# vymv/PupilOptixLab

Hardware: AMD Instinct MI355X
Metric: Mrays/sec + ms/frame, 1M-tri scene @1920x1080 8spp; 1/2/4/8-GPU scaling (higher is better)
Workload: dtype f32; 1 GPU; config4: 1,000,014-primitive sphere field (1,000,014 tris), 1920x1080, 8 spp, max_depth 4; rays_traced_plain_process=18645769168, parallelism=tiles32x1, area_emitters=2, accel=flat, emitter_select=guide, bvh_nodes=213019

## Files before the change

### include/pupil_pt.h

```cpp
#pragma once
#include <stddef.h>
#include <stdint.h>

#ifdef __cplusplus
extern "C" {
#endif

#define PUPIL_OK 0
#define PUPIL_ERR_INVALID -1
#define PUPIL_ERR_HIP -2
#define PUPIL_ERR_OOM -3
#define PUPIL_ERR_IO -4
#define PUPIL_ERR_UNSUPPORTED -5

#define PUPIL_TEX_RGB 0u
#define PUPIL_TEX_BITMAP 1u
#define PUPIL_TEX_CHECKERBOARD 2u

#define PUPIL_MAT_UNKNOWN 0u
#define PUPIL_MAT_DIFFUSE 1u
#define PUPIL_MAT_DIELECTRIC 2u
#define PUPIL_MAT_ROUGH_DIELECTRIC 3u
#define PUPIL_MAT_CONDUCTOR 4u
#define PUPIL_MAT_ROUGH_CONDUCTOR 5u
#define PUPIL_MAT_PLASTIC 6u
#define PUPIL_MAT_ROUGH_PLASTIC 7u
#define PUPIL_MAT_COUNT 8u

#define PUPIL_EMITTER_NONE 0u
#define PUPIL_EMITTER_TRI_AREA 1u
#define PUPIL_EMITTER_SPHERE 2u
#define PUPIL_EMITTER_CONST_ENV 3u
#define PUPIL_EMITTER_ENV_MAP 4u
#define PUPIL_EMITTER_POINT 5u
#define PUPIL_EMITTER_SPOT 6u
#define PUPIL_EMITTER_DIRECTIONAL 7u

#define PUPIL_SHAPE_MESH 0u
#define PUPIL_SHAPE_SPHERE 1u

typedef struct pupil_texture {
    uint32_t type;
    float c0[3];
    float c1[3];
    float transform[16];
    uint32_t width, height;
    uint32_t filter;
    uint32_t pad;
    const float *rgba;
} pupil_texture;

typedef struct pupil_material {
    uint32_t type;
    uint32_t twosided;
    float int_ior, ext_ior;
    uint32_t nonlinear;
    pupil_texture tex[4];
} pupil_material;

typedef struct pupil_shape {
    uint32_t kind;
    uint32_t num_vertices, num_faces;
    const float *positions;
    const float *normals;
    const float *texcoords;
    const uint32_t *indices;
} pupil_shape;

typedef struct pupil_instance {
    uint32_t shape;
    uint32_t material;
    float to_world[12];
    float to_object[12];
    uint32_t flip_normals;
    uint32_t flip_tex_coords;
    int32_t emitter_offset;
    uint32_t pad;
} pupil_instance;

typedef struct pupil_emitter {
    uint32_t type;
    float weight;
    float select_probability;
    float area;
    pupil_texture radiance;
    float pos[3][3];
    float nrm[3][3];
    float tex[3][2];
    float center[3];
    float radius;
    float color[3];
    float to_world[9];
    float to_local[9];
    float scale;
} pupil_emitter;

typedef struct pupil_scene_desc {
    uint32_t width, height;
    uint32_t max_depth;
    uint32_t pad0;
    float sample_to_camera[16];
    float camera_to_world[16];
    uint32_t num_shapes;
    uint32_t num_materials;
    uint32_t num_instances;
    uint32_t num_area_emitters;
    const pupil_shape *shapes;
    const pupil_material *materials;
    const pupil_instance *instances;
    const pupil_emitter *area_emitters;
    const pupil_emitter *env;
} pupil_scene_desc;

typedef struct pupil_pt_frame {
    void *accum;
    void *frame;
    void *albedo;
    void *normal;
    void *test;
    uint32_t compact;
    uint32_t pad;
} pupil_pt_frame;

typedef struct pupil_pt_launch {
    uint32_t random_seed;
    uint32_t sample_cnt;
    uint32_t spp;
    uint32_t max_depth;
    uint32_t accumulate;
    uint32_t tile_size;
    uint32_t tile_rank;
    uint32_t tile_world;
    uint32_t collect_stats;
    uint32_t hints;
} pupil_pt_launch;

#define PUPIL_STATS_COUNTERS 1u
#define PUPIL_STATS_TIMING 2u
#define PUPIL_STATS_TRACE_TIMING 4u
#define PUPIL_HINT_CONTINUE 1u

typedef struct pupil_pt_counters {
    uint64_t primary_rays;
    uint64_t extension_rays;
    uint64_t shadow_rays;
    uint64_t path_samples;
    uint64_t node_visits;
    uint64_t prim_tests;
    uint64_t bvh_nodes;
    uint64_t bvh_prims;
    double build_ms;
    double last_render_ms;
    double trace_ms;
    double trace_bytes;
    uint64_t trace_launches;
    double extend_ms;
    uint64_t extend_launches;
    uint64_t extend_node_visits;
    uint64_t extend_prim_tests;
    double extend_bytes;
    double shade_ms;
    uint64_t two_level;
    uint64_t shadow_rays_reference;
    uint64_t bvh_depth;
    uint64_t unique_node_fetches;
    uint64_t rays_traced_total;
    uint64_t frames_in_flight;
    uint64_t pipeline_slots;
    uint64_t tlas_sah_splits;
    uint64_t queue_handed;
    uint64_t queue_activated;
    uint64_t queue_retired;
    uint64_t queue_listed;
    uint64_t ring_bytes;
    uint64_t ring_budget_bytes;
    uint64_t accel_refits;
    float node_bound[3];
    uint32_t pad_counters;
    uint64_t node_loop_iters;
    uint64_t node_loop_lanes;
    uint64_t leaf_loop_iters;
    uint64_t leaf_loop_lanes;
    uint64_t refills;
    uint64_t refill_lanes;
    uint64_t frame_launches;
    double frame_ms;
    uint64_t terminal_rays_culled;
    uint64_t coop_slots;
    uint64_t hidden_instances;
} pupil_pt_counters;

typedef struct pupil_pt pupil_pt;

const char *pupil_last_error(void);
int pupil_abi_version(void);

int pupil_pt_create(const pupil_scene_desc *scene, int device, pupil_pt **out);
int pupil_pt_set_camera(pupil_pt *pt, const float sample_to_camera[16], const float camera_to_world[16]);
int pupil_pt_update_instance(pupil_pt *pt, uint32_t instance, const float to_world[12], const float to_object[12]);
int pupil_pt_update_instances(pupil_pt *pt, uint32_t n, const uint32_t *ids, const float *to_world,
                              const float *to_object);
int pupil_pt_update_instances_masked(pupil_pt *pt, uint32_t n, const uint32_t *ids,
                                     const float *to_world, const float *to_object,
                                     const uint32_t *visibility_mask);
int pupil_pt_update_instances_device(pupil_pt *pt, uint32_t n, const uint32_t *ids_device,
                                     const void *to_world_device, const void *to_object_device, void *hip_stream);
int pupil_pt_get_instance_transforms(pupil_pt *pt, uint32_t first, uint32_t n, float *to_world, float *to_object);
int pupil_pt_instances_device_info(pupil_pt *pt, uint64_t *updates, uint64_t *instances, uint64_t *skipped,
                                   uint32_t *last_launches, uint32_t *last_syncs, double *last_ms);
int pupil_debug_invert3x4(const float m[12], float out[12]);
int pupil_debug_update_counts(pupil_pt *pt, uint32_t *launches, uint32_t *syncs);
#define PUPIL_VERTS_DEVICE 1u
#define PUPIL_VERTS_REBUILD 2u
int pupil_pt_update_shape_vertices(pupil_pt *pt, uint32_t shape, const float *positions, const float *normals,
                                   uint32_t flags, void *hip_stream);
int pupil_pt_snapshot_shape_vertices(pupil_pt *pt, uint32_t shape);
int pupil_pt_clear_vertex_snapshots(pupil_pt *pt);
int pupil_pt_update_emitters(pupil_pt *pt, const pupil_scene_desc *scene);
int pupil_pt_enable_device_emitters(pupil_pt *pt, const pupil_scene_desc *scene);
int pupil_pt_refresh_emitters(pupil_pt *pt);
int pupil_pt_device_emitters_info(pupil_pt *pt, uint32_t *enabled, uint64_t *refreshes, double *last_ms);
int pupil_pt_update_materials(pupil_pt *pt, uint32_t n, const uint32_t *ids, const pupil_material *materials);
int pupil_pt_update_texture_device(pupil_pt *pt, uint32_t material, uint32_t slot, const void *rgba_device,
                                   uint32_t width, uint32_t height, void *hip_stream);
int pupil_pt_material_info(pupil_pt *pt, uint64_t *updates, double *last_ms);
int pupil_pt_update_env_device(pupil_pt *pt, const void *rgba_device, uint32_t width, uint32_t height,
                               void *hip_stream);
int pupil_pt_update_env_params(pupil_pt *pt, float scale, const float to_world[9], const float to_local[9]);
int pupil_pt_env_info(pupil_pt *pt, uint64_t *updates, double *last_ms);
int pupil_pt_render(pupil_pt *pt, const pupil_pt_frame *out, const pupil_pt_launch *launch, void *hip_stream);
int pupil_pt_stats(pupil_pt *pt, pupil_pt_counters *out);
int pupil_pt_local_pixels(uint32_t width, uint32_t height, uint32_t tile_size, uint32_t tile_rank,
                          uint32_t tile_world, uint32_t *out_pixels, uint32_t *inout_count);
void pupil_pt_destroy(pupil_pt *pt);
int pupil_pt_motion_vectors(pupil_pt *pt, const float prev_sample_to_camera[16],
                            const float prev_camera_to_world[16], const float *prev_to_world,
                            void *out_flow , uint32_t compact,
                            uint32_t tile_size, uint32_t tile_rank, uint32_t tile_world,
                            void *hip_stream);

typedef struct pupil_ray_hits {
    void *hit;
    void *instance;
    void *primitive;
    void *material;
    void *position;
    void *normal;
    void *texcoord;
} pupil_ray_hits;
enum { PUPIL_QUERY_ANY_HIT = 1 };
int pupil_pt_query_rays(pupil_pt *pt, uint32_t n, const void *rays_device , uint32_t flags,
                        const pupil_ray_hits *out, void *hip_stream);
int pupil_pt_query_camera(pupil_pt *pt, float jitter_x, float jitter_y, uint32_t compact, uint32_t tile_size,
                          uint32_t tile_rank, uint32_t tile_world, void *rays_out_device, const pupil_ray_hits *out,
                          void *hip_stream);
int pupil_pt_query_info(pupil_pt *pt, uint64_t *queries, uint64_t *rays, uint64_t *scratch_grows, double *last_ms);

typedef struct pupil_ray_radiance {
    void *radiance;
    void *albedo;
    void *normal;
} pupil_ray_radiance;
int pupil_pt_radiance_rays(pupil_pt *pt, uint32_t n, const void *rays_device ,
                           const uint32_t *stream_ids_device ,
                           const pupil_pt_launch *launch, const pupil_ray_radiance *out, void *hip_stream);
int pupil_pt_radiance_info(pupil_pt *pt, uint64_t *calls, uint64_t *rays, uint64_t *extension_rays,
                           uint64_t *shadow_rays, uint64_t *scratch_grows, double *last_ms);

int pupil_pt_trace_rays(pupil_pt *pt, uint32_t n, const float *rays, float *out, int any_hit);
int pupil_pt_export_bvh4(pupil_pt *pt, uint32_t *num_nodes, void *nodes, uint32_t *num_records, float *records,
                         int32_t *root_link);
int pupil_debug_math(int device, uint32_t n, const float *x, const float *y2, float *out);
int pupil_debug_select_emitter(pupil_pt *pt, uint32_t n, const float *p, int32_t *out);
int pupil_debug_read_emitters(pupil_pt *pt, uint32_t first, uint32_t n, float *out);
int pupil_debug_emitter_sample(pupil_pt *pt, uint32_t emitter, uint32_t n, const float *xi, const float *pos_nrm,
                               float *out);
int pupil_debug_read_emitter_guide(pupil_pt *pt, uint32_t *bits, uint32_t *guide, uint32_t *inout_count);
int pupil_debug_env(pupil_pt *pt, uint32_t n, const float *xi_or_dir, const float *pos_nrm, uint32_t mode, float *out);
int pupil_debug_read_env_tables(pupil_pt *pt, uint32_t *width, uint32_t *height, float *col_cdf, float *row_cdf,
                                float *row_weight, float *normalization);
int pupil_debug_tex_sample(pupil_pt *pt, uint32_t material, uint32_t slot, uint32_t n, const float *uv, float *out);
int pupil_debug_read_material(pupil_pt *pt, uint32_t material, uint32_t *type, float out[3]);
int pupil_debug_fill_tlas_reserve(pupil_pt *pt, float value);
int pupil_debug_bvh_reinsert(int device, uint32_t n, const float *boxes, uint32_t rounds, double *cost,
                             uint32_t *kept, uint32_t *rejected);
int pupil_debug_partition(int device, uint32_t n, uint32_t capacity, const uint8_t *keys, uint32_t nbins,
                          uint32_t mode, uint32_t shift_or_tag, uint32_t bin_mask, const uint64_t *cum_in,
                          uint32_t *out, uint32_t *counts, uint32_t *starts, uint32_t *total, uint32_t *log,
                          uint64_t *cum_out, uint64_t *snap, uint32_t *info);

enum { PUPIL_IMAGE_AUTO = 0, PUPIL_IMAGE_EXR = 1, PUPIL_IMAGE_HDR = 2, PUPIL_IMAGE_PFM = 3 };
int pupil_image_save(const char *path, uint32_t width, uint32_t height, const float *rgba, uint32_t format);

int pupil_image_load(const char *path, uint32_t *width, uint32_t *height, float *rgba);

enum {
    PUPIL_DENOISE_USE_ALBEDO = 1,
    PUPIL_DENOISE_USE_NORMAL = 1 << 1,
    PUPIL_DENOISE_APPLY_TO_AOV = 1 << 2,
    PUPIL_DENOISE_USE_TEMPORAL = 1 << 3,
    PUPIL_DENOISE_USE_UPSCALE_2X = 1 << 4,
    PUPIL_DENOISE_TILED = 1 << 5
};
typedef struct pupil_denoise_data {
    const void *input;
    void *output;
    const void *prev_output;
    const void *albedo;
    const void *normal;
    const void *motion_vector;
} pupil_denoise_data;
typedef struct pupil_denoiser pupil_denoiser;
int pupil_denoiser_create(int device, uint32_t mode, pupil_denoiser **out);
int pupil_denoiser_setup(pupil_denoiser *d, uint32_t mode, uint32_t width, uint32_t height, float sigma_color);
int pupil_denoiser_execute(pupil_denoiser *d, const pupil_denoise_data *data, void *hip_stream);
int pupil_denoiser_reset_history(pupil_denoiser *d);
void pupil_denoiser_destroy(pupil_denoiser *d);

typedef struct pupil_world pupil_world;

int pupil_world_create(pupil_world **out);
int pupil_world_load_xml(pupil_world *w, const char *path);
int pupil_world_set_film(pupil_world *w, uint32_t width, uint32_t height, uint32_t max_depth);
int pupil_world_set_sensor(pupil_world *w, float fov, char fov_axis, float near_clip, float far_clip,
                           const float to_world[16]);
int pupil_world_add_mesh(pupil_world *w, uint32_t num_vertices, uint32_t num_faces, const float *positions,
                         const float *normals, const float *texcoords, const uint32_t *indices, uint32_t *out_shape);
int pupil_world_add_builtin_shape(pupil_world *w, const char *name , uint32_t *out_shape);
int pupil_world_add_material(pupil_world *w, const pupil_material *m, uint32_t *out_material);
int pupil_world_add_instance(pupil_world *w, uint32_t shape, uint32_t material, const float to_world[16],
                             uint32_t flip_normals, uint32_t flip_tex_coords, uint32_t is_emitter,
                             const pupil_texture *radiance, uint32_t *out_instance);
int pupil_world_add_const_env(pupil_world *w, const float radiance[3]);
int pupil_world_add_delta_emitter(pupil_world *w, const pupil_emitter *e, uint32_t *out_light);
int pupil_world_set_delta_emitter(pupil_world *w, uint32_t light, const pupil_emitter *e);
int pupil_world_get_delta_emitter(pupil_world *w, uint32_t light, pupil_emitter *out);
int pupil_world_invert3x3(const float m[9], float out[9]);
int pupil_world_set_instance_transform(pupil_world *w, uint32_t instance, const float to_world[16]);
int pupil_world_set_instance_visibility(pupil_world *w, uint32_t instance, uint32_t visibility_mask);
int pupil_world_get_instance_visibility(pupil_world *w, uint32_t instance, uint32_t *visibility_mask);
int pupil_world_set_mesh_vertices(pupil_world *w, uint32_t shape, const float *positions, const float *normals);
int pupil_world_set_material(pupil_world *w, uint32_t material, const pupil_material *m);
int pupil_world_get_desc(pupil_world *w, pupil_scene_desc *desc);
void pupil_world_destroy(pupil_world *w);

#ifdef __cplusplus
}
#endif
```

### pupiloptixlab_amd/abi.py

```python
from __future__ import annotations

import ctypes as C
import os

TEX_RGB, TEX_BITMAP, TEX_CHECKERBOARD = 0, 1, 2
MAT_UNKNOWN, MAT_DIFFUSE, MAT_DIELECTRIC, MAT_ROUGH_DIELECTRIC = 0, 1, 2, 3
MAT_CONDUCTOR, MAT_ROUGH_CONDUCTOR, MAT_PLASTIC, MAT_ROUGH_PLASTIC = 4, 5, 6, 7
EMITTER_NONE, EMITTER_TRI_AREA, EMITTER_SPHERE, EMITTER_CONST_ENV, EMITTER_ENV_MAP = 0, 1, 2, 3, 4
EMITTER_POINT, EMITTER_SPOT, EMITTER_DIRECTIONAL = 5, 6, 7
SHAPE_MESH, SHAPE_SPHERE = 0, 1

PUPIL_OK = OK = 0
ERR_INVALID, ERR_HIP, ERR_OOM, ERR_IO, ERR_UNSUPPORTED = -1, -2, -3, -4, -5
VERTS_DEVICE, VERTS_REBUILD = 1, 2
IMAGE_AUTO, IMAGE_EXR, IMAGE_HDR, IMAGE_PFM = 0, 1, 2, 3
ERR_NAMES = {-1: "PUPIL_ERR_INVALID", -2: "PUPIL_ERR_HIP", -3: "PUPIL_ERR_OOM", -4: "PUPIL_ERR_IO",
             -5: "PUPIL_ERR_UNSUPPORTED"}

f32p = C.POINTER(C.c_float)
u32p = C.POINTER(C.c_uint32)


class Texture(C.Structure):
    _fields_ = [("type", C.c_uint32), ("c0", C.c_float * 3), ("c1", C.c_float * 3),
                ("transform", C.c_float * 16), ("width", C.c_uint32), ("height", C.c_uint32),
                ("filter", C.c_uint32), ("pad", C.c_uint32), ("rgba", f32p)]


class Material(C.Structure):
    _fields_ = [("type", C.c_uint32), ("twosided", C.c_uint32), ("int_ior", C.c_float),
                ("ext_ior", C.c_float), ("nonlinear", C.c_uint32), ("tex", Texture * 4)]


class Shape(C.Structure):
    _fields_ = [("kind", C.c_uint32), ("num_vertices", C.c_uint32), ("num_faces", C.c_uint32),
                ("positions", f32p), ("normals", f32p), ("texcoords", f32p), ("indices", u32p)]


class Instance(C.Structure):
    _fields_ = [("shape", C.c_uint32), ("material", C.c_uint32), ("to_world", C.c_float * 12),
                ("to_object", C.c_float * 12), ("flip_normals", C.c_uint32),
                ("flip_tex_coords", C.c_uint32), ("emitter_offset", C.c_int32), ("pad", C.c_uint32)]


class Emitter(C.Structure):
    _fields_ = [("type", C.c_uint32), ("weight", C.c_float), ("select_probability", C.c_float),
                ("area", C.c_float), ("radiance", Texture), ("pos", (C.c_float * 3) * 3),
                ("nrm", (C.c_float * 3) * 3), ("tex", (C.c_float * 2) * 3), ("center", C.c_float * 3),
                ("radius", C.c_float), ("color", C.c_float * 3), ("to_world", C.c_float * 9),
                ("to_local", C.c_float * 9), ("scale", C.c_float)]


class SceneDesc(C.Structure):
    _fields_ = [("width", C.c_uint32), ("height", C.c_uint32), ("max_depth", C.c_uint32),
                ("pad0", C.c_uint32), ("sample_to_camera", C.c_float * 16),
                ("camera_to_world", C.c_float * 16), ("num_shapes", C.c_uint32),
                ("num_materials", C.c_uint32), ("num_instances", C.c_uint32),
                ("num_area_emitters", C.c_uint32), ("shapes", C.POINTER(Shape)),
                ("materials", C.POINTER(Material)), ("instances", C.POINTER(Instance)),
                ("area_emitters", C.POINTER(Emitter)), ("env", C.POINTER(Emitter))]


class Frame(C.Structure):
    _fields_ = [("accum", C.c_void_p), ("frame", C.c_void_p), ("albedo", C.c_void_p),
                ("normal", C.c_void_p), ("test", C.c_void_p), ("compact", C.c_uint32),
                ("pad", C.c_uint32)]


class Launch(C.Structure):
    _fields_ = [("random_seed", C.c_uint32), ("sample_cnt", C.c_uint32), ("spp", C.c_uint32),
                ("max_depth", C.c_uint32), ("accumulate", C.c_uint32), ("tile_size", C.c_uint32),
                ("tile_rank", C.c_uint32), ("tile_world", C.c_uint32), ("collect_stats", C.c_uint32),
                ("hints", C.c_uint32)]


class Counters(C.Structure):
    _fields_ = [("primary_rays", C.c_uint64), ("extension_rays", C.c_uint64),
                ("shadow_rays", C.c_uint64), ("path_samples", C.c_uint64),
                ("node_visits", C.c_uint64), ("prim_tests", C.c_uint64), ("bvh_nodes", C.c_uint64),
                ("bvh_prims", C.c_uint64), ("build_ms", C.c_double), ("last_render_ms", C.c_double),
                ("trace_ms", C.c_double), ("trace_bytes", C.c_double), ("trace_launches", C.c_uint64),
                ("extend_ms", C.c_double), ("extend_launches", C.c_uint64), ("extend_node_visits", C.c_uint64),
                ("extend_prim_tests", C.c_uint64), ("extend_bytes", C.c_double), ("shade_ms", C.c_double),
                ("two_level", C.c_uint64), ("shadow_rays_reference", C.c_uint64),
                ("bvh_depth", C.c_uint64), ("unique_node_fetches", C.c_uint64),
                ("rays_traced_total", C.c_uint64), ("frames_in_flight", C.c_uint64),
                ("pipeline_slots", C.c_uint64), ("tlas_sah_splits", C.c_uint64),
                ("queue_handed", C.c_uint64), ("queue_activated", C.c_uint64), ("queue_retired", C.c_uint64),
                ("queue_listed", C.c_uint64), ("ring_bytes", C.c_uint64), ("ring_budget_bytes", C.c_uint64),
                ("accel_refits", C.c_uint64), ("node_bound", C.c_float * 3), ("pad_counters", C.c_uint32),
                ("node_loop_iters", C.c_uint64), ("node_loop_lanes", C.c_uint64), ("leaf_loop_iters", C.c_uint64),
                ("leaf_loop_lanes", C.c_uint64), ("refills", C.c_uint64), ("refill_lanes", C.c_uint64),
                ("frame_launches", C.c_uint64),
                ("frame_ms", C.c_double),
                ("terminal_rays_culled", C.c_uint64), ("coop_slots", C.c_uint64),
                ("hidden_instances", C.c_uint64)]

    def as_dict(self):
        d = {name: getattr(self, name) for name, _ in self._fields_ if name != "pad_counters"}
        d["node_bound"] = [float(x) for x in self.node_bound]
        return d


DENOISE_USE_ALBEDO, DENOISE_USE_NORMAL, DENOISE_APPLY_TO_AOV = 1, 2, 4
DENOISE_USE_TEMPORAL, DENOISE_USE_UPSCALE_2X, DENOISE_TILED = 8, 16, 32


class DenoiseData(C.Structure):
    _fields_ = [("input", C.c_void_p), ("output", C.c_void_p), ("prev_output", C.c_void_p),
                ("albedo", C.c_void_p), ("normal", C.c_void_p), ("motion_vector", C.c_void_p)]


QUERY_ANY_HIT = 1


class RayHits(C.Structure):
    _fields_ = [("hit", C.c_void_p), ("instance", C.c_void_p), ("primitive", C.c_void_p),
                ("material", C.c_void_p), ("position", C.c_void_p), ("normal", C.c_void_p),
                ("texcoord", C.c_void_p)]


class RayRadiance(C.Structure):
    _fields_ = [("radiance", C.c_void_p), ("albedo", C.c_void_p), ("normal", C.c_void_p)]


SIGNATURES = {
    "pupil_last_error": (C.c_char_p, []),
    "pupil_abi_version": (C.c_int, []),
    "pupil_pt_create": (C.c_int, [C.POINTER(SceneDesc), C.c_int, C.POINTER(C.c_void_p)]),
    "pupil_pt_set_camera": (C.c_int, [C.c_void_p, f32p, f32p]),
    "pupil_pt_update_instance": (C.c_int, [C.c_void_p, C.c_uint32, f32p, f32p]),
    "pupil_pt_update_instances": (C.c_int, [C.c_void_p, C.c_uint32, u32p, f32p, f32p]),
    "pupil_pt_update_instances_masked": (C.c_int, [C.c_void_p, C.c_uint32, u32p, f32p, f32p, u32p]),
    "pupil_pt_update_instances_device": (C.c_int, [C.c_void_p, C.c_uint32, C.c_void_p, C.c_void_p, C.c_void_p,
                                                    C.c_void_p]),
    "pupil_pt_get_instance_transforms": (C.c_int, [C.c_void_p, C.c_uint32, C.c_uint32, f32p, f32p]),
    "pupil_pt_instances_device_info": (C.c_int, [C.c_void_p, C.POINTER(C.c_uint64), C.POINTER(C.c_uint64),
                                                  C.POINTER(C.c_uint64), u32p, u32p, C.POINTER(C.c_double)]),
    "pupil_debug_invert3x4": (C.c_int, [f32p, f32p]),
    "pupil_debug_update_counts": (C.c_int, [C.c_void_p, u32p, u32p]),
    "pupil_pt_update_shape_vertices": (C.c_int, [C.c_void_p, C.c_uint32, C.c_void_p, C.c_void_p, C.c_uint32,
                                                  C.c_void_p]),
    "pupil_pt_snapshot_shape_vertices": (C.c_int, [C.c_void_p, C.c_uint32]),
    "pupil_pt_clear_vertex_snapshots": (C.c_int, [C.c_void_p]),
    "pupil_pt_update_emitters": (C.c_int, [C.c_void_p, C.POINTER(SceneDesc)]),
    "pupil_pt_enable_device_emitters": (C.c_int, [C.c_void_p, C.POINTER(SceneDesc)]),
    "pupil_pt_refresh_emitters": (C.c_int, [C.c_void_p]),
    "pupil_pt_device_emitters_info": (C.c_int, [C.c_void_p, u32p, C.POINTER(C.c_uint64), C.POINTER(C.c_double)]),
    "pupil_pt_update_materials": (C.c_int, [C.c_void_p, C.c_uint32, u32p, C.POINTER(Material)]),
    "pupil_pt_update_texture_device": (C.c_int, [C.c_void_p, C.c_uint32, C.c_uint32, C.c_void_p, C.c_uint32,
                                                  C.c_uint32, C.c_void_p]),
    "pupil_pt_material_info": (C.c_int, [C.c_void_p, C.POINTER(C.c_uint64), C.POINTER(C.c_double)]),
    "pupil_pt_update_env_device": (C.c_int, [C.c_void_p, C.c_void_p, C.c_uint32, C.c_uint32, C.c_void_p]),
    "pupil_pt_update_env_params": (C.c_int, [C.c_void_p, C.c_float, f32p, f32p]),
    "pupil_pt_env_info": (C.c_int, [C.c_void_p, C.POINTER(C.c_uint64), C.POINTER(C.c_double)]),
    "pupil_debug_read_env_tables": (C.c_int, [C.c_void_p, u32p, u32p, f32p, f32p, f32p, f32p]),
    "pupil_world_invert3x3": (C.c_int, [f32p, f32p]),
    "pupil_debug_read_material": (C.c_int, [C.c_void_p, C.c_uint32, u32p, f32p]),
    "pupil_debug_read_emitters": (C.c_int, [C.c_void_p, C.c_uint32, C.c_uint32, f32p]),
    "pupil_debug_read_emitter_guide": (C.c_int, [C.c_void_p, u32p, u32p, u32p]),
    "pupil_debug_fill_tlas_reserve": (C.c_int, [C.c_void_p, C.c_float]),
    "pupil_pt_render": (C.c_int, [C.c_void_p, C.POINTER(Frame), C.POINTER(Launch), C.c_void_p]),
    "pupil_pt_stats": (C.c_int, [C.c_void_p, C.POINTER(Counters)]),
    "pupil_pt_local_pixels": (C.c_int, [C.c_uint32, C.c_uint32, C.c_uint32, C.c_uint32, C.c_uint32,
                                         u32p, u32p]),
    "pupil_pt_destroy": (None, [C.c_void_p]),
    "pupil_pt_motion_vectors": (C.c_int, [C.c_void_p, f32p, f32p, f32p, C.c_void_p, C.c_uint32, C.c_uint32,
                                           C.c_uint32, C.c_uint32, C.c_void_p]),
    "pupil_pt_query_rays": (C.c_int, [C.c_void_p, C.c_uint32, C.c_void_p, C.c_uint32, C.POINTER(RayHits), C.c_void_p]),
    "pupil_pt_query_camera": (C.c_int, [C.c_void_p, C.c_float, C.c_float, C.c_uint32, C.c_uint32, C.c_uint32,
                                         C.c_uint32, C.c_void_p, C.POINTER(RayHits), C.c_void_p]),
    "pupil_pt_query_info": (C.c_int, [C.c_void_p, C.POINTER(C.c_uint64), C.POINTER(C.c_uint64),
                                       C.POINTER(C.c_uint64), C.POINTER(C.c_double)]),
    "pupil_pt_radiance_rays": (C.c_int, [C.c_void_p, C.c_uint32, C.c_void_p, C.c_void_p, C.POINTER(Launch),
                                          C.POINTER(RayRadiance), C.c_void_p]),
    "pupil_pt_radiance_info": (C.c_int, [C.c_void_p, C.POINTER(C.c_uint64), C.POINTER(C.c_uint64),
                                          C.POINTER(C.c_uint64), C.POINTER(C.c_uint64), C.POINTER(C.c_uint64),
                                          C.POINTER(C.c_double)]),
    "pupil_pt_trace_rays": (C.c_int, [C.c_void_p, C.c_uint32, f32p, f32p, C.c_int]),
    "pupil_pt_export_bvh4": (C.c_int, [C.c_void_p, u32p, C.c_void_p, u32p, f32p, C.POINTER(C.c_int32)]),
    "pupil_debug_math": (C.c_int, [C.c_int, C.c_uint32, f32p, f32p, f32p]),
    "pupil_debug_bvh_reinsert": (C.c_int, [C.c_int, C.c_uint32, f32p, C.c_uint32, C.POINTER(C.c_double), u32p, u32p]),
    "pupil_debug_partition": (C.c_int, [C.c_int, C.c_uint32, C.c_uint32, C.POINTER(C.c_uint8), C.c_uint32, C.c_uint32,
                                         C.c_uint32, C.c_uint32, C.POINTER(C.c_uint64), u32p, u32p, u32p, u32p, u32p,
                                         C.POINTER(C.c_uint64), C.POINTER(C.c_uint64), u32p]),
    "pupil_image_save": (C.c_int, [C.c_char_p, C.c_uint32, C.c_uint32, f32p, C.c_uint32]),
    "pupil_debug_select_emitter": (C.c_int, [C.c_void_p, C.c_uint32, f32p, C.POINTER(C.c_int32)]),
    "pupil_debug_env": (C.c_int, [C.c_void_p, C.c_uint32, f32p, f32p, C.c_uint32, f32p]),
    "pupil_debug_emitter_sample": (C.c_int, [C.c_void_p, C.c_uint32, C.c_uint32, f32p, f32p, f32p]),
    "pupil_debug_tex_sample": (C.c_int, [C.c_void_p, C.c_uint32, C.c_uint32, C.c_uint32, f32p, f32p]),
    "pupil_image_load": (C.c_int, [C.c_char_p, C.POINTER(C.c_uint32), C.POINTER(C.c_uint32), f32p]),
    "pupil_world_create": (C.c_int, [C.POINTER(C.c_void_p)]),
    "pupil_world_load_xml": (C.c_int, [C.c_void_p, C.c_char_p]),
    "pupil_world_set_film": (C.c_int, [C.c_void_p, C.c_uint32, C.c_uint32, C.c_uint32]),
    "pupil_world_set_sensor": (C.c_int, [C.c_void_p, C.c_float, C.c_char, C.c_float, C.c_float, f32p]),
    "pupil_world_add_mesh": (C.c_int, [C.c_void_p, C.c_uint32, C.c_uint32, f32p, f32p, f32p, u32p, u32p]),
    "pupil_world_add_builtin_shape": (C.c_int, [C.c_void_p, C.c_char_p, u32p]),
    "pupil_world_add_material": (C.c_int, [C.c_void_p, C.POINTER(Material), u32p]),
    "pupil_world_add_instance": (C.c_int, [C.c_void_p, C.c_uint32, C.c_uint32, f32p, C.c_uint32,
                                           C.c_uint32, C.c_uint32, C.POINTER(Texture), u32p]),
    "pupil_world_add_const_env": (C.c_int, [C.c_void_p, f32p]),
    "pupil_world_add_delta_emitter": (C.c_int, [C.c_void_p, C.POINTER(Emitter), u32p]),
    "pupil_world_set_delta_emitter": (C.c_int, [C.c_void_p, C.c_uint32, C.POINTER(Emitter)]),
    "pupil_world_get_delta_emitter": (C.c_int, [C.c_void_p, C.c_uint32, C.POINTER(Emitter)]),
    "pupil_world_set_instance_transform": (C.c_int, [C.c_void_p, C.c_uint32, f32p]),
    "pupil_world_set_instance_visibility": (C.c_int, [C.c_void_p, C.c_uint32, C.c_uint32]),
    "pupil_world_get_instance_visibility": (C.c_int, [C.c_void_p, C.c_uint32, u32p]),
    "pupil_world_set_mesh_vertices": (C.c_int, [C.c_void_p, C.c_uint32, f32p, f32p]),
    "pupil_world_set_material": (C.c_int, [C.c_void_p, C.c_uint32, C.POINTER(Material)]),
    "pupil_world_get_desc": (C.c_int, [C.c_void_p, C.POINTER(SceneDesc)]),
    "pupil_world_destroy": (None, [C.c_void_p]),
    "pupil_denoiser_create": (C.c_int, [C.c_int, C.c_uint32, C.POINTER(C.c_void_p)]),
    "pupil_denoiser_setup": (C.c_int, [C.c_void_p, C.c_uint32, C.c_uint32, C.c_uint32, C.c_float]),
    "pupil_denoiser_execute": (C.c_int, [C.c_void_p, C.POINTER(DenoiseData), C.c_void_p]),
    "pupil_denoiser_reset_history": (C.c_int, [C.c_void_p]),
    "pupil_denoiser_destroy": (None, [C.c_void_p]),
}

LIB_DIR = os.path.join(os.path.dirname(os.path.abspath(__file__)), "lib")
LIB_PATH = os.path.join(LIB_DIR, "libpupil_pt.so")


class PupilError(RuntimeError):
    def __init__(self, code: int, message: str):
        super().__init__(f"{ERR_NAMES.get(code, code)}: {message}")
        self.code = code


_LIB = None


def load_library(path: str | None = None):
    global _LIB
    if _LIB is not None and path is None:
        return _LIB
    try:
        import torch
    except Exception:
        pass
    p = path or os.environ.get("PUPIL_LIB") or LIB_PATH
    if not os.path.exists(p):
        raise FileNotFoundError(f"{p} not built: run `python -c 'import __graft_entry__ as g; g.build()'`")
    lib = C.CDLL(p)
    for name, (res, args) in SIGNATURES.items():
        if p != LIB_PATH and not hasattr(lib, name):
            continue
        fn = getattr(lib, name)
        fn.restype = res
        fn.argtypes = args
    if path is None:
        _LIB = lib
    return lib


def check(code: int, lib=None):
    if code != PUPIL_OK:
        lib = lib or load_library()
        msg = lib.pupil_last_error()
        raise PupilError(code, msg.decode() if msg else "")
    return code
```

### pupiloptixlab_amd/csrc/engine.hip

```cpp
#include <hip/hip_runtime.h>

#include <algorithm>
#include <chrono>
#include <cmath>
#include <cstddef>
#include <cstdio>
#include <cstdlib>
#include <cstring>
#include <string>
#include <vector>

#include "host/emitter_weight.h"
#include "host/pipe_schedule.h"
#include "host/scoped_buffer.h"
#include "pt_accel.h"

namespace {

thread_local std::string g_last_error;

constexpr uint32_t kMaxPairs = 4096;

using namespace pupil;

// ... 525 lines not shown
    bool trace_only = false;
    uint32_t pair = 0;
    bool open = false;
    const TraceStats *tsp() const { return stats ? &ts_dev : nullptr; }
    uint32_t pair_cap = 0;
    void ev0(uint8_t kind) {
        open = timing && !(trace_only && kind == 2) && pair < pair_cap;
        if (!open) return;
        pt->pair_kind[pair] = kind;
        (void)hipEventRecord(pt->trace_events[2 * pair], s);
    }
    void ev1() {
        if (!open) return;
        (void)hipEventRecord(pt->trace_events[2 * pair + 1], s);
        pair++;
        open = false;
    }
    void tail_slot() {
        if (tail && pt->tail_launches < kMaxDepth + 1)
            ts_dev.wave_times = pt->tail_buf + (size_t)pt->tail_launches++ * pt->tail_waves * 4;
        else
            ts_dev.wave_times = nullptr;
    }
    PathState view(uint32_t h, size_t paths, size_t extra = 0) const {
        PathState v = pt->ps;
        const size_t o = (size_t)h * paths + extra;
        v.ray_o += o, v.ray_d += o, v.hit += o, v.thr += o, v.rad += o, v.misc += o;
        v.sh_d += o, v.sh_c += o, v.mbin += o, v.sflags += o;
        return v;
    }
};

int render_pipelined(RenderCtx &cx, const FrameParams &fp, const pupil_pt_launch *launch) {
    pupil_pt *pt = cx.pt;
    hipStream_t s = cx.s;
    PipeState &st = pt->pipe;
    const PipeKnobs &kn = pt->knobs;
    const uint32_t nl = fp.num_local;
    const PipeRender r{fp.spp, launch->random_seed, fp.max_depth, (launch->hints & PUPIL_HINT_CONTINUE) != 0, cx.stats,
                       fp.num_paths, nl, {cx.key[0], cx.key[1], cx.key[2], cx.key[3], cx.key[4]}};
    PipePlan plan = st.plan(kn, r);
    bool grew = false;
    if (plan.ring_paths() > pt->cap) {
        grew = true;
        int rc = ensure_state(pt, plan.ring_paths());
        while (rc == PUPIL_ERR_OOM && plan.shrink()) rc = ensure_state(pt, plan.ring_paths());
        if (rc) return rc;
    }
    if (plan.aov_floats() > pt->aov_cap) {
        grew = true;
        if (pt->aov_scratch) (void)hipFree(pt->aov_scratch);
        pt->aov_scratch = nullptr;
        pt->aov_cap = 0;
        HIP_TRY(hipMalloc((void **)&pt->aov_scratch, sizeof(float) * plan.aov_floats()));
        pt->aov_cap = plan.aov_floats();
    }
    const PathState ring = pt->ps;
    const PipeCommit commit = st.commit(plan, grew);
    for (const PipeRange &d : commit.dropped) {
        if (d.off + d.len > pt->cap) continue;
        HIP_TRY(hipMemsetAsync(ring.sflags + d.off, 0, d.len, s));
        if (!pt->shade_list) HIP_TRY(hipMemsetAsync(ring.mbin + d.off, 0xFF, d.len, s));
    }
    if (commit.reset && pt->ring_fresh) {
        HIP_TRY(hipMemsetAsync(ring.sflags, 0, pt->cap, s));
        if (!pt->shade_list) HIP_TRY(hipMemsetAsync(ring.mbin, 0xFF, pt->cap, s));
        pt->ring_fresh = false;
    }
    Queues &q = pt->q;
    const uint32_t interleave0 = pt->primary_interleave;
    if (st.one_launch_frame(kn) && frame_kernel_supported(pt->sc)) {
        HIP_TRY(hipMemcpyAsync(pt->ray_cum + 2, pt->ray_cum, 2 * sizeof(unsigned long long), hipMemcpyDeviceToDevice, s));
        pt->snap_taken = true;
        FrameParams fs = fp;
        fs.group = 1;
        cx.ev0(3);
        launch_frame(pt->sc, fs, ring, pt->q.work + kWorkFrame, pt->ray_cum, pt->ovf, pt->ovf_threads,
                     interleave0 && fp.spp > 1 ? fp.spp : 0u, s);
        cx.ev1();
        launch_accumulate(fp, ring, nullptr, true, s);
        st.one_launch_frame_done();
        pt->last_iters = fp.max_depth;
        pt->last_primary = st.started;
        pt->primary_cum += st.started;
        pt->frame_launches++;
        return PUPIL_OK;
    }
    auto scratch = [&](uint32_t index) { return pt->aov_scratch + (size_t)index * 7 * nl; };
    pt->snap_taken = false;
    auto trace = [&](const PipeTrace &t) -> int {
        const uint32_t interleave = interleave0 && t.samples > 1 ? t.samples : 0u;
        if (t.inject) {
            FrameParams fg = fp;
            fg.seed0 = t.nf.seed;
            fg.num_paths = t.nfp;
            launch_generate(pt->sc, fg, cx.view(t.nf.slot, st.cap), s, !pt->fresh());
        }
        if (t.had) {
            launch_partition(ring.sflags, t.ring_extent, 2, kPartFlags, t.read_tag, q.nxsh, q.hist, q.counts + kCntNext,
                             q.counts + kStartNext, nullptr, nullptr, s, pt->ray_cum,
                             pt->snap_taken ? nullptr : pt->ray_cum + 2);
            pt->snap_taken = true;
            if (t.check_exit) {
                uint32_t c[2] = {1, 1};
                HIP_TRY(hipMemcpyAsync(c, q.counts + kCntNext, sizeof(c), hipMemcpyDeviceToHost, s));
                HIP_TRY(hipStreamSynchronize(s));
                if (c[0] == 0 && c[1] == 0) return 1;
            }
            cx.ev0(1);
            cx.tail_slot();
            if (t.inject)
                launch_trace_mixed(pt->sc, ring, q, pt->ovf, pt->ovf_threads, cx.tsp(), s, t.nfp, 0u, t.base, interleave, nl);
            else
                launch_trace_mixed(pt->sc, ring, q, pt->ovf, pt->ovf_threads, cx.tsp(), s);
            cx.ev1();
        } else {
            cx.ev0(0);
            cx.tail_slot();
            launch_extend(pt->sc, cx.view(t.nf.slot, st.cap), q, nullptr, nullptr, t.nfp, pt->ovf, pt->ovf_threads,
                          cx.tsp(), s, interleave, nl);
            cx.ev1();
        }
        return 0;
    };
    auto shade = [&](const PipeShade &h) -> int {
        if (!pt->shade_list)
            launch_partition(ring.mbin, h.ring_extent, kPartMaxBins, kPartExclusive, 0u, q.bins, q.hist, q.counts,
                             q.counts + kStartBins, q.counts + kScratch, nullptr, s, nullptr, nullptr, pt->bin_mask);
        FrameParams fs = fp;
        fs.group = st.G;
        if (h.aov_scratch) {
            fs.albedo = scratch(h.aov_index);
            fs.normal = fs.albedo + 3 * (size_t)nl;
            fs.test = fs.albedo + 6 * (size_t)nl;
            fs.aov_local = 1;
            fs.aov_frame_stride = (uint32_t)(7 * nl);
        }
        if (h.clear_flags) HIP_TRY(hipMemsetAsync(ring.sflags, 0, h.ring_extent, s));
        constexpr ShadeList kLists[] = {kShadeAll, kShadeNext, kShadeNextRange};
        const ShadeList list = pt->shade_list ? kLists[(int)h.list] : kShadeBins;
        cx.ev0(2);
        launch_shade(pt->sc, fs, ring, q, h.write_tag, s, list, h.range_base, h.range_n, h.max_count, pt->fresh(),
                     h.range_seed);
        cx.ev1();
        return 0;
    };
    if (st.half_pending)
        if (const int rc = shade(st.shade_half())) return rc;
    const uint32_t L = st.iterations();
    for (uint32_t it = 0; it < L; it++) {
        const int rc = trace(st.trace_half(kn, it, L));
        if (rc == 1) break;
        if (rc) return rc;
        if (const int rs = shade(st.shade_half())) return rs;
    }
    const PipeFinish fin = st.finish(kn, L);
    launch_accumulate(fp, cx.view(fin.slot, st.cap, fin.offset), fin.aov_scratch ? scratch(fin.aov_index) : nullptr, true, s);
    if (fin.trace_ahead) {
        const int rc = trace(st.trace_ahead(kn));
        if (rc < 0) return rc;
        st.half_ran(rc == 0);
    }
    pt->last_iters = L;
    pt->last_primary = st.started;
    pt->primary_cum += st.started;
    return PUPIL_OK;
}


int upload_shapes(pupil_pt *pt, const pupil_scene_desc *scene) {
    std::vector<ShapeDev> &shapes = pt->shapes;
    shapes.assign(scene->num_shapes, ShapeDev{});
    for (uint32_t s = 0; s < scene->num_shapes; s++) {
        const pupil_shape &sh = scene->shapes[s];
        shapes[s].kind = sh.kind;
        shapes[s].num_vertices = sh.num_vertices;
        shapes[s].num_faces = sh.num_faces;
        if (sh.kind == PUPIL_SHAPE_MESH) {
            if (!sh.positions || !sh.indices || sh.num_faces == 0)
                return fail(PUPIL_ERR_INVALID, "mesh without positions/indices");
            for (size_t i = 0; i < 3 * (size_t)sh.num_faces; i++)
                if (sh.indices[i] >= sh.num_vertices) return fail(PUPIL_ERR_INVALID, "index out of range");
            if (pt->upload(&shapes[s].pos, sh.positions, 3 * (size_t)sh.num_vertices) ||
                (sh.normals && pt->upload(&shapes[s].nrm, sh.normals, 3 * (size_t)sh.num_vertices)) ||
                (sh.texcoords && pt->upload(&shapes[s].tex, sh.texcoords, 2 * (size_t)sh.num_vertices)) ||
                pt->upload(&shapes[s].idx, sh.indices, 3 * (size_t)sh.num_faces))
                return fail(PUPIL_ERR_OOM, "mesh upload failed");
        } else if (sh.kind != PUPIL_SHAPE_SPHERE) {
            return fail(PUPIL_ERR_INVALID, "unknown shape kind");
        }
    }
    return PUPIL_OK;
}

int convert_material(const pupil_material &src, DevMaterial &d) {
    std::memset(&d, 0, sizeof(d));
    d.type = src.type <= 7u ? src.type : 0u;
    d.twosided = src.twosided;
    d.nonlinear = src.nonlinear;
    if (d.type == PUPIL_MAT_DIELECTRIC || d.type == PUPIL_MAT_ROUGH_DIELECTRIC || d.type == PUPIL_MAT_PLASTIC ||
        d.type == PUPIL_MAT_ROUGH_PLASTIC)
        d.eta = src.int_ior / src.ext_ior;
    for (int k = 0; k < 4; k++)
        if (const int rc = texture_desc(src.tex[k], d.tex[k])) return rc;
    if (d.type == PUPIL_MAT_PLASTIC || d.type == PUPIL_MAT_ROUGH_PLASTIC) {
        const pupil_texture &dt = d.type == PUPIL_MAT_PLASTIC ? src.tex[0] : src.tex[1];
        const pupil_texture &stx = d.type == PUPIL_MAT_PLASTIC ? src.tex[1] : src.tex[2];
        d.specular_sampling_weight = specular_sampling_weight(pixel_average(dt), pixel_average(stx));
        d.int_fdr = diffuse_reflectance(1.f / d.eta);
    }
    return PUPIL_OK;
}

int convert_materials(pupil_pt *pt, const pupil_scene_desc *scene, std::vector<DevMaterial> &mats) {
    mats.resize(scene->num_materials);
    for (uint32_t m = 0; m < scene->num_materials; m++) {
        const pupil_material &src = scene->materials[m];
        DevMaterial &d = mats[m];
        if (const int rc = convert_material(src, d)) return rc;
        for (int k = 0; k < 4; k++)
            if (src.tex[k].type == PUPIL_TEX_BITMAP) {
                float4 *texels = nullptr;
                HIP_TRY(pt->upload(&texels, reinterpret_cast<const float4 *>(src.tex[k].rgba),
                                   (size_t)src.tex[k].width * src.tex[k].height));
                d.tex[k].data = texels;
            }
    }
    if (mats.empty()) {
        DevMaterial d;
        std::memset(&d, 0, sizeof(d));
        mats.push_back(d);
    }
    return PUPIL_OK;
}

int upload_tables(pupil_pt *pt, const pupil_scene_desc *scene, const std::vector<DevMaterial> &mats) {
    std::vector<DevInstance> &insts = pt->h_insts;
    insts.resize(scene->num_instances);
    std::vector<uint32_t> prim_inst;
    uint32_t true_areas = 0;
    if (scene->area_emitters)
        for (uint32_t e = 0; e < scene->num_area_emitters; e++) {
            const uint32_t t = scene->area_emitters[e].type;
            true_areas += t >= PUPIL_EMITTER_POINT && t <= PUPIL_EMITTER_DIRECTIONAL ? 0u : 1u;
        }
    for (uint32_t i = 0; i < scene->num_instances; i++) {
        const pupil_instance &src = scene->instances[i];
        if (src.shape >= scene->num_shapes) return fail(PUPIL_ERR_INVALID, "instance shape out of range");
        if (src.material >= mats.size()) return fail(PUPIL_ERR_INVALID, "instance material out of range");
        const pupil_shape &sh = scene->shapes[src.shape];
        DevInstance &d = insts[i];
        std::memset(&d, 0, sizeof(d));
        std::memcpy(d.to_world, src.to_world, sizeof(d.to_world));
        std::memcpy(d.to_object, src.to_object, sizeof(d.to_object));
        d.kind = sh.kind;
        d.material = src.material;
        d.prim_offset = (uint32_t)prim_inst.size();
        d.emitter_offset = src.emitter_offset;
        d.flip_normals = src.flip_normals;
        d.flip_tex_coords = src.flip_tex_coords;
        d.bin = material_bin(mats[src.material].type);
        d.blas_root = kTraverseDone;
        d.positions = pt->shapes[src.shape].pos;
        d.normals = pt->shapes[src.shape].nrm;
        d.texcoords = pt->shapes[src.shape].tex;
        d.indices = pt->shapes[src.shape].idx;
        const uint32_t nprim = sh.kind == PUPIL_SHAPE_SPHERE ? 1u : sh.num_faces;
        if (src.emitter_offset >= 0 && (size_t)src.emitter_offset + nprim > true_areas)
            return fail(PUPIL_ERR_INVALID, "emitter offset out of range");
        prim_inst.insert(prim_inst.end(), nprim, i);
    }
    pt->num_prims = (uint32_t)prim_inst.size();
    if (prim_inst.size() >= (1ull << 31)) return fail(PUPIL_ERR_UNSUPPORTED, "more than 2^31 primitives");
    std::vector<uint32_t> inst_first(insts.size() + 1);
    for (size_t i = 0; i < insts.size(); i++) inst_first[i] = insts[i].prim_offset;
    inst_first[insts.size()] = (uint32_t)prim_inst.size();
    uint32_t guide_shift = 0;
    while ((prim_inst.size() >> guide_shift) > 8192u) guide_shift++;
    std::vector<uint32_t> inst_guide;
    if (!prim_inst.empty()) {
        const size_t nb = ((prim_inst.size() - 1) >> guide_shift) + 1;
        inst_guide.resize(nb + 1);
        for (size_t k = 0; k <= nb; k++)
            inst_guide[k] = prim_inst[std::min(k << guide_shift, prim_inst.size() - 1)];
    } else {
        inst_guide.assign(2, 0u);
    }
    uint32_t *d_inst_first = nullptr, *d_inst_guide = nullptr;
    if (pt->upload(&pt->d_insts, insts.data(), insts.size()) || pt->upload(&pt->d_mats, mats.data(), mats.size()) ||
        pt->upload(&pt->d_prim_inst, prim_inst.data(), prim_inst.size()) ||
        pt->upload(&d_inst_first, inst_first.data(), inst_first.size()) ||
        pt->upload(&d_inst_guide, inst_guide.data(), inst_guide.size()))
        return fail(PUPIL_ERR_OOM, "scene upload failed");
    pt->num_mats = (uint32_t)mats.size();
    pt->h_mats = mats;
    DeviceScene &sc = pt->sc;
    sc.num_prims = pt->num_prims;
    sc.prim_inst = pt->d_prim_inst;
    sc.inst_first = d_inst_first;
    sc.inst_guide = d_inst_guide;
    sc.inst_guide_shift = guide_shift;
    sc.instances = pt->d_insts;
    sc.materials = pt->d_mats;
    return PUPIL_OK;
}

void derive_bins(pupil_pt *pt) {
    DeviceScene &sc = pt->sc;
    const bool was_list = pt->shade_list;
    const uint32_t was_single = sc.single_bin;
    uint32_t bins = 0;
    for (const DevInstance &d : pt->h_insts) bins |= 1u << d.bin;
    pt->shade_list = (bins & (bins - 1u)) == 0u;
    if (const char *sl = std::getenv("PUPIL_SHADE_LIST")) {
        if (std::strcmp(sl, "bins") == 0) pt->shade_list = false;
        if (std::strcmp(sl, "list") == 0) pt->shade_list = true;
    }
    sc.single_bin = pt->shade_list && bins && (bins & (bins - 1u)) == 0u ? (uint32_t)__builtin_ctz(bins) : 0u;
    pt->bin_mask = bins | 1u;
    if (pt->shade_list != was_list || sc.single_bin != was_single) pt->ring_fresh = true;
}

void read_knobs(pupil_pt *pt) {
    DeviceScene &sc = pt->sc;
    int cus = 256;
    (void)hipDeviceGetAttribute(&cus, hipDeviceAttributeMultiprocessorCount, pt->device);
    sc.num_cus = (uint32_t)std::max(1, cus);
    sc.trace_refill = 16;
    if (const char *r = std::getenv("PUPIL_REFILL")) sc.trace_refill = (uint32_t)std::min(64, std::max(1, std::atoi(r)));
    if (const char *po = std::getenv("PUPIL_PRIMARY_ORDER")) pt->primary_interleave = std::strcmp(po, "path") != 0;
    derive_bins(pt);
    if (const char *fr = std::getenv("PUPIL_FRESH_SHADE")) pt->fresh_shade = std::atoi(fr) != 0;
    if (const char *tc = std::getenv("PUPIL_TERMINAL_CULL")) pt->cull_on = std::atoi(tc) != 0;
    if (const char *tk = std::getenv("PUPIL_TERMINAL_CULL_K"))
        pt->cull_k = (uint32_t)std::min((int)kCullSetMax, std::max(1, std::atoi(tk)));
    if (const char *a = std::getenv("PUPIL_AHEAD")) pt->knobs.ahead_mode = std::min(2, std::max(0, std::atoi(a)));
    if (const char *k = std::getenv("PUPIL_PIPE")) pt->knobs.limit = (uint32_t)std::min(63, std::max(0, std::atoi(k)));
    {
        size_t free_b = 0, total_b = 0;
        if (hipMemGetInfo(&free_b, &total_b) != hipSuccess) free_b = 0;
        pt->knobs.budget = 0.25 * (double)free_b;
    }
    if (const char *g = std::getenv("PUPIL_PIPE_GB")) pt->knobs.budget = std::max(0.0, std::atof(g)) * 1e9;
    if (const char *g = std::getenv("PUPIL_PIPE_PATHS")) pt->knobs.paths = std::max(1.0, std::atof(g));
    if (const char *g = std::getenv("PUPIL_PIPE_GROUP_PATHS")) pt->knobs.group_paths = std::max(1.0, std::atof(g));
    if (const char *g = std::getenv("PUPIL_PIPE_GROUP_MAX")) pt->knobs.group_max = (uint32_t)std::min(64, std::max(1, std::atoi(g)));
    if (const char *g = std::getenv("PUPIL_PIPE_GROUP_ALL")) pt->knobs.group_all = std::atoi(g) != 0;
    if (const char *g = std::getenv("PUPIL_PIPE_SPLIT")) pt->knobs.split = std::atoi(g) != 0;
    if (const char *g = std::getenv("PUPIL_PIPE_RAMP")) pt->knobs.ramp = (uint32_t)std::max(0, std::atoi(g));
    if (const char *g = std::getenv("PUPIL_FRAME_PATHS")) pt->knobs.frame_paths = std::max(0.0, std::atof(g));
    if (const char *g = std::getenv("PUPIL_RADIANCE_CHUNK"))
        pt->rad_chunk = (size_t)std::min(2147483647.0, std::max(64.0, std::atof(g)));
    sc.trace_node_min = 8;
    if (const char *r = std::getenv("PUPIL_NODE_MIN")) sc.trace_node_min = (uint32_t)std::min(64, std::max(1, std::atoi(r)));
}

int alloc_workspace(pupil_pt *pt) {
    pt->ovf_threads = trace_grid_blocks() * (uint32_t)kTraceBlock;
    if (pt->alloc(&pt->ovf, (size_t)pt->ovf_threads * kStackOvf) || pt->alloc(&pt->trace_counters, 32) ||
        pt->alloc(&pt->ray_cum, 4) || pt->alloc(&pt->q.counts, kCountSlots) || pt->alloc(&pt->q.work, kWorkSlots) ||
        pt->alloc(&pt->d_cull, 1 + kCullSetMax) || pt->alloc(&pt->cull_cum, 2 * kCullShards * kCullStride) ||
        pt->alloc(&pt->rad_cum, pupil_pt::kRadTotals + 2))
        return fail(PUPIL_ERR_OOM, "workspace allocation failed");
    if (hipMemset(pt->q.work, 0, kWorkSlots * sizeof(uint32_t)) != hipSuccess ||
        hipMemset(pt->rad_cum, 0, (pupil_pt::kRadTotals + 2) * sizeof(unsigned long long)) != hipSuccess ||
        hipMemset(pt->cull_cum, 0, 2 * kCullShards * kCullStride * sizeof(unsigned long long)) != hipSuccess ||
        hipMemset(pt->ray_cum, 0, 4 * sizeof(unsigned long long)) != hipSuccess)
        return fail(PUPIL_ERR_HIP, "workspace clear failed");
    if (hipEventCreate(&pt->ev_begin) != hipSuccess || hipEventCreate(&pt->ev_end) != hipSuccess ||
        hipEventCreateWithFlags(&pt->ev_sync, hipEventDisableTiming) != hipSuccess ||
        hipEventCreateWithFlags(&pt->ev_verts, hipEventDisableTiming) != hipSuccess)
        return fail(PUPIL_ERR_HIP, "event creation failed");
    return PUPIL_OK;
}

int derive_cull_set(pupil_pt *pt, bool records_changed = true) {
    DeviceScene &sc = pt->sc;
    sc.cull_set = pt->d_cull + 1;
    sc.cull_n = 0;
    if (records_changed) pt->cull_scanned = 0;
    if (records_changed) pt->query_slot_valid = false;
    if (!pt->cull_on || sc.has_env || !sc.prims || (sc.two_level && !sc.tl_world)) return PUPIL_OK;
    uint64_t emissive = 0;
    for (size_t i = 0; i < pt->h_insts.size(); i++) {
        const DevInstance &d = pt->h_insts[i];
        if (d.emitter_offset < 0) continue;
        emissive += d.kind == PUPIL_SHAPE_MESH ? pt->shapes[pt->accel.inst_shape[i]].num_faces : 1u;
    }
    if (emissive == 0 || emissive > pt->cull_k) return PUPIL_OK;
    if (pt->cull_scanned == emissive) {
        sc.cull_n = pt->cull_scanned;
        return PUPIL_OK;
    }
    uint32_t found[1 + kCullSetMax] = {};
    HIP_TRY(hipMemsetAsync(pt->d_cull, 0, sizeof(found), pt->own_stream));
    launch_cull_scan(sc.prims, pt->accel.world_record_slots(), pt->d_insts, (uint32_t)pt->h_insts.size(), pt->d_cull,
                     kCullSetMax, pt->own_stream);
    HIP_TRY(hipGetLastError());
    HIP_TRY(hipMemcpyAsync(found, pt->d_cull, sizeof(found), hipMemcpyDeviceToHost, pt->own_stream));
    HIP_TRY(hipStreamSynchronize(pt->own_stream));
    pt->accel.counts.launches++, pt->accel.counts.syncs++;
    if (found[0] != emissive) return PUPIL_OK;
    std::sort(found + 1, found + 1 + found[0]);
    HIP_TRY(hipMemcpyAsync(pt->d_cull, found, sizeof(found), hipMemcpyHostToDevice, pt->own_stream));
    HIP_TRY(hipStreamSynchronize(pt->own_stream));
    pt->accel.counts.syncs++;
    sc.cull_n = pt->cull_scanned = found[0];
    return PUPIL_OK;
}

int device_emitter_tables(const pupil_pt *pt, const pupil_scene_desc *scene, std::vector<uint32_t> &emit_inst,
                          std::vector<float> &inst_weight) {
    const uint32_t ni = (uint32_t)pt->h_insts.size(), ne = pt->num_true_areas;
    if (scene->num_instances != ni) return fail(PUPIL_ERR_INVALID, "the scene's instance count is not the engine's");
    if (scene->num_area_emitters != pt->sc.num_areas)
        return fail(PUPIL_ERR_INVALID, "the scene's area emitter count is not the engine's");
    if ((ni && !scene->instances) || (pt->sc.num_areas && !scene->area_emitters))
        return fail(PUPIL_ERR_INVALID, "missing scene array");
    for (uint32_t e = 0; e < pt->sc.num_areas; e++) {
        const uint32_t t = scene->area_emitters[e].type;
        const bool delta = t >= PUPIL_EMITTER_POINT && t <= PUPIL_EMITTER_DIRECTIONAL;
        if (delta != (e >= ne) || (delta && t != pt->emit_types[e]))
            return fail(PUPIL_ERR_INVALID, "the scene's delta lights are not the engine's");
    }
    emit_inst.assign(ne, 0u);
    inst_weight.assign(ni, 0.f);
    uint32_t next = 0;
    for (uint32_t i = 0; i < ni; i++) {
        const DevInstance &d = pt->h_insts[i];
        if (scene->instances[i].emitter_offset != d.emitter_offset)
            return fail(PUPIL_ERR_INVALID, "an instance's emitter_offset is not the engine's");
        if (d.emitter_offset < 0) continue;
        const uint32_t range = d.kind == PUPIL_SHAPE_MESH ? pt->shapes[pt->accel.inst_shape[i]].num_faces : 1u;
        if ((uint32_t)d.emitter_offset != next || range > ne - next)
            return fail(PUPIL_ERR_INVALID, "an emissive instance's emitter range is not its face count");
        inst_weight[i] = Pupil::world::GetWeight(scene->area_emitters[next].radiance);
        for (uint32_t k = 0; k < range; k++) emit_inst[next + k] = i;
        next += range;
    }
    if (next != ne) return fail(PUPIL_ERR_INVALID, "the emitter ranges do not cover the emitter table");
    return PUPIL_OK;
}

int device_emitter_setup(pupil_pt *pt, const pupil_scene_desc *scene) {
    std::vector<uint32_t> emit_inst;
    std::vector<float> inst_weight;
    if (const int rc = device_emitter_tables(pt, scene, emit_inst, inst_weight)) return rc;
    const uint32_t ne = pt->sc.num_areas;
    if (!pt->d_emit_inst || pt->dev_emit_count != ne) {
        for (void *p : {(void *)pt->d_emit_inst, (void *)pt->d_emit_weight, (void *)pt->d_emit_select}) pt->release(p);
        pt->d_emit_inst = nullptr;
        pt->d_emit_weight = pt->d_emit_select = nullptr;
        if (pt->alloc(&pt->d_emit_inst, ne) || pt->alloc(&pt->d_emit_weight, ne) || pt->alloc(&pt->d_emit_select, ne))
            return fail(PUPIL_ERR_OOM, "emitter bookkeeping allocation failed");
        pt->dev_emit_count = ne;
    }
    if (!pt->d_inst_weight && (pt->alloc(&pt->d_inst_weight, inst_weight.size()) || pt->alloc(&pt->d_emit_sum, 1)))
        return fail(PUPIL_ERR_OOM, "emitter bookkeeping allocation failed");
    if (!emit_inst.empty())
        HIP_TRY(hipMemcpy(pt->d_emit_inst, emit_inst.data(), sizeof(uint32_t) * emit_inst.size(), hipMemcpyHostToDevice));
    HIP_TRY(hipMemcpy(pt->d_inst_weight, inst_weight.data(), sizeof(float) * inst_weight.size(), hipMemcpyHostToDevice));
    return PUPIL_OK;
}

int rebuild_emitters(pupil_pt *pt) {
    const auto t0 = std::chrono::steady_clock::now();
    EmitterJob job{};
    job.areas = pt->d_areas;
    job.cdf = pt->d_cdf;
    job.guide = pt->d_guide;
    job.guide_bits = pt->sc.guide_bits;
    job.count = pt->num_true_areas;
    job.total = pt->sc.num_areas;
    job.emitter_num = pt->sc.num_areas + (pt->sc.has_env ? 1u : 0u);
    job.instances = pt->d_insts;
    job.emit_inst = pt->d_emit_inst;
    job.inst_weight = pt->d_inst_weight;
    job.weight = pt->d_emit_weight;
    job.select = pt->d_emit_select;
    job.sum = pt->d_emit_sum;
    launch_emitter_rebuild(job, pt->own_stream);
    HIP_TRY(hipGetLastError());
    HIP_TRY(hipStreamSynchronize(pt->own_stream));
    pt->accel.counts.launches += job.count ? (job.guide ? 5u : 4u) : 0u;
    pt->accel.counts.syncs++;
    pt->emit_refreshes++;
    pt->emit_ms = std::chrono::duration<double, std::milli>(std::chrono::steady_clock::now() - t0).count();
    return derive_cull_set(pt, false);
}

int keep_device_emitters(pupil_pt *pt, const pupil_scene_desc *scene) {
    if (!pt->dev_emit) return PUPIL_OK;
    if (device_emitter_setup(pt, scene) != PUPIL_OK) {
        pt->dev_emit = false;
        g_last_error = "device-side emitter table switched off: " + g_last_error;
    }
    return PUPIL_OK;
}

}

extern "C" {

const char *pupil_last_error(void) { return g_last_error.c_str(); }
int pupil_abi_version(void) { return 7; }

int pupil_pt_local_pixels(uint32_t width, uint32_t height, uint32_t tile_size, uint32_t tile_rank, uint32_t tile_world,
                          uint32_t *out_pixels, uint32_t *inout_count) {
    if (!inout_count || width == 0 || height == 0) return fail(PUPIL_ERR_INVALID, "bad arguments");
    if (tile_world > 1 && (tile_size == 0 || tile_rank >= tile_world)) return fail(PUPIL_ERR_INVALID, "bad tiling");
    const uint32_t n = local_pixels(width, height, tile_size, tile_rank, tile_world, nullptr);
    if (out_pixels) {
        if (*inout_count < n) return fail(PUPIL_ERR_INVALID, "output too small");
        local_pixels(width, height, tile_size, tile_rank, tile_world, out_pixels);
    }
    *inout_count = n;
    return PUPIL_OK;
}

int pupil_pt_create(const pupil_scene_desc *scene, int device, pupil_pt **out) {
    if (!scene || !out) return fail(PUPIL_ERR_INVALID, "null argument");
    *out = nullptr;
    if (scene->width == 0 || scene->height == 0) return fail(PUPIL_ERR_INVALID, "empty film");
    if (scene->num_instances == 0) return fail(PUPIL_ERR_INVALID, "scene has no instances");
    if (scene->env && scene->env->type == PUPIL_EMITTER_ENV_MAP &&
        !env_map_size_ok(scene->env->radiance.width, scene->env->radiance.height))
        return fail(PUPIL_ERR_INVALID, "env map smaller than 2 x 2 texels");
    int ndev = 0;
    if (hipGetDeviceCount(&ndev) != hipSuccess || ndev == 0) return fail(PUPIL_ERR_HIP, "no HIP device");
    if (device < 0 || device >= ndev) return fail(PUPIL_ERR_INVALID, "bad device index");
    HIP_TRY(hipSetDevice(device));
    auto pt = new pupil_pt();
    pt->device = device;
    pt->width = scene->width;
    pt->height = scene->height;
    pt->max_depth = scene->max_depth ? scene->max_depth : 1;
    std::memcpy(pt->sc.camera.s2c, scene->sample_to_camera, sizeof(pt->sc.camera.s2c));
    std::memcpy(pt->sc.camera.c2w, scene->camera_to_world, sizeof(pt->sc.camera.c2w));
    std::vector<DevMaterial> mats;
    int rc = hipStreamCreateWithFlags(&pt->own_stream, hipStreamNonBlocking) == hipSuccess
                 ? PUPIL_OK
                 : fail(PUPIL_ERR_HIP, "stream creation failed");
    if (!rc) rc = upload_shapes(pt, scene);
    if (!rc) rc = convert_materials(pt, scene, mats);
    if (!rc) rc = upload_tables(pt, scene, mats);
    if (!rc) rc = upload_emitters(pt, scene);
    if (!rc)
        rc = pt->accel.build({pt->own_stream, pt->num_prims, pt->d_prim_inst, pt->d_insts, pt->d_mats, &pt->h_insts,
                              &pt->sc, &pt->totals},
                             scene, pt->shapes);
    if (!rc) read_knobs(pt);
    if (!rc) rc = alloc_workspace(pt);
    if (!rc) rc = pt->accel.publish();
    if (!rc) rc = derive_cull_set(pt);
    if (rc) {
        delete pt;
        return rc;
    }
    pt->totals.bvh_prims = pt->num_prims;
    pt->totals.build_ms = pt->accel.ms;
    *out = pt;
    return PUPIL_OK;
}

int pupil_pt_set_camera(pupil_pt *pt, const float sample_to_camera[16], const float camera_to_world[16]) {
    if (!pt || !sample_to_camera || !camera_to_world) return fail(PUPIL_ERR_INVALID, "null argument");
    if (std::memcmp(pt->sc.camera.s2c, sample_to_camera, sizeof(pt->sc.camera.s2c)) != 0 ||
        std::memcmp(pt->sc.camera.c2w, camera_to_world, sizeof(pt->sc.camera.c2w)) != 0)
        pt->pipe.invalidate();
    std::memcpy(pt->sc.camera.s2c, sample_to_camera, sizeof(pt->sc.camera.s2c));
    std::memcpy(pt->sc.camera.c2w, camera_to_world, sizeof(pt->sc.camera.c2w));
    return PUPIL_OK;
}

int pupil_pt_update_instances_masked(pupil_pt *pt, uint32_t n, const uint32_t *ids, const float *to_world,
                                     const float *to_object, const uint32_t *visibility_mask) {
    if (!pt || (n && (!ids || (!to_world && !visibility_mask) || !to_world != !to_object)))
        return fail(PUPIL_ERR_INVALID, "null argument");
    for (uint32_t k = 0; k < n; k++)
        if (ids[k] >= pt->h_insts.size()) return fail(PUPIL_ERR_INVALID, "instance index out of range");
    if (n == 0) return PUPIL_OK;
    HIP_TRY(hipSetDevice(pt->device));
    HIP_TRY(order_after_renders(pt));
    pt->pipe.invalidate();
    pt->accel.counts = SceneAccel::Counts{};
    std::vector<uint32_t> changed;
    bool emitters_moved = false;
    for (uint32_t k = 0; k < n; k++) {
        const uint32_t id = ids[k];
        DevInstance &d = pt->h_insts[id];
        if (to_world) {
            emitters_moved = emitters_moved || d.emitter_offset >= 0;
            std::memcpy(d.to_world, to_world + 12 * (size_t)k, sizeof(d.to_world));
            std::memcpy(d.to_object, to_object + 12 * (size_t)k, sizeof(d.to_object));
            if (pt->accel.two_level) refresh_instance_margins(d);
        }
        if (visibility_mask) d.hidden = (visibility_mask[k] & 0xFFu) == 0u ? 1u : 0u;
        if (std::find(changed.begin(), changed.end(), id) == changed.end()) changed.push_back(id);
    }
    std::vector<DevInstance> staged;
    staged.reserve(changed.size());
    for (uint32_t id : changed) {
        staged.push_back(device_instance(pt->h_insts[id]));
        HIP_TRY(hipMemcpyAsync(pt->d_insts + id, &staged.back(), sizeof(DevInstance), hipMemcpyHostToDevice,
                               pt->own_stream));
    }
    pt->accel.refits++;
    if (const int rc = pt->accel.update_instances(changed)) return rc;
    pt->totals.build_ms = pt->accel.ms;
    if (const int rc = derive_cull_set(pt)) return rc;
    if (pt->dev_emit && emitters_moved) return rebuild_emitters(pt);
    return PUPIL_OK;
}

int pupil_pt_update_shape_vertices(pupil_pt *pt, uint32_t shape, const float *positions, const float *normals,
                                   uint32_t flags, void *hip_stream) {
    if (!pt || !positions) return fail(PUPIL_ERR_INVALID, "null argument");
    if (shape >= pt->shapes.size()) return fail(PUPIL_ERR_INVALID, "shape index out of range");
    const ShapeDev &sd = pt->shapes[shape];
    if (sd.kind != PUPIL_SHAPE_MESH) return fail(PUPIL_ERR_INVALID, "shape is not a mesh");
    if (normals && !sd.nrm) return fail(PUPIL_ERR_INVALID, "the shape was created without normals");
    if (flags & ~(PUPIL_VERTS_DEVICE | PUPIL_VERTS_REBUILD)) return fail(PUPIL_ERR_INVALID, "unknown flags");
    const bool device = (flags & PUPIL_VERTS_DEVICE) != 0u, rebuild = (flags & PUPIL_VERTS_REBUILD) != 0u;
    std::vector<uint32_t> changed;
    bool emissive = false;
    for (uint32_t i = 0; i < (uint32_t)pt->h_insts.size(); i++)
        if (pt->accel.inst_shape[i] == shape && pt->h_insts[i].kind == PUPIL_SHAPE_MESH) {
            changed.push_back(i);
            emissive = emissive || pt->h_insts[i].emitter_offset >= 0;
        }
    if (device && emissive && !pt->dev_emit)
        return fail(PUPIL_ERR_UNSUPPORTED, "device vertices of an emissive shape: the emitter table needs the host path");
    HIP_TRY(hipSetDevice(pt->device));
    const auto t0 = std::chrono::steady_clock::now();
    HIP_TRY(order_after_renders(pt));
    pt->pipe.invalidate();
    const size_t bytes = sizeof(float) * 3 * (size_t)sd.num_vertices;
    if (device) {
        HIP_TRY(hipEventRecord(pt->ev_verts, (hipStream_t)hip_stream));
        HIP_TRY(hipStreamWaitEvent(pt->own_stream, pt->ev_verts, 0));
    }
    const hipMemcpyKind kind = device ? hipMemcpyDeviceToDevice : hipMemcpyHostToDevice;
    HIP_TRY(hipMemcpyAsync(sd.pos, positions, bytes, kind, pt->own_stream));
    if (normals) HIP_TRY(hipMemcpyAsync(sd.nrm, normals, bytes, kind, pt->own_stream));
    if (changed.empty()) {
        HIP_TRY(hipStreamSynchronize(pt->own_stream));
    } else {
        if (const int rc = pt->accel.update_shape(shape, changed, rebuild)) return rc;
        pt->totals.build_ms = std::chrono::duration<double, std::milli>(std::chrono::steady_clock::now() - t0).count();
    }
    pt->accel.refits++;
    if (const int rc = derive_cull_set(pt)) return rc;
    if (pt->dev_emit && emissive) return rebuild_emitters(pt);
    return PUPIL_OK;
}
// ... 870 lines not shown
        const uint32_t rec_slots = slots ? pt->accel.world_record_slots() : 1u;
        if (slots && !pt->query_slot_valid) {
            launch_query_prim_slots(pt->sc.prims, rec_slots, pt->num_prims, pt->query_slot, s);
            pt->query_slot_valid = true;
        }
        const QueryJob job{rays,
                           hits,
                           n,
                           rec_slots,
                           slots ? pt->query_slot : nullptr,
                           (int32_t *)out->instance,
                           (int32_t *)out->primitive,
                           (int32_t *)out->material,
                           (float *)out->position,
                           (float *)out->normal,
                           (float2 *)out->texcoord,
                           scatter,
                           scatter ? (float4 *)out->hit : nullptr};
        launch_query_resolve(pt->sc, job, s);
    }
    HIP_TRY(hipEventRecord(pt->ev_q1, s));
    HIP_TRY(hipGetLastError());
    pt->queries++;
    pt->query_rays += n;
    pt->last_stream = s;
    pt->rendered = true;
    return PUPIL_OK;
}

}
}

int pupil_pt_query_rays(pupil_pt *pt, uint32_t n, const void *rays_device, uint32_t flags, const pupil_ray_hits *out,
                        void *hip_stream) {
    if (!pt) return fail(PUPIL_ERR_INVALID, "null argument");
    if (const int rc = check_query_outputs(out, flags)) return rc;
    if (n >= (1u << 31)) return fail(PUPIL_ERR_INVALID, "too many rays in one query");
    if (n == 0) return PUPIL_OK;
    if (!rays_device) return fail(PUPIL_ERR_INVALID, "null argument");
    if ((uintptr_t)rays_device & 15u) return fail(PUPIL_ERR_INVALID, "misaligned ray list (16 B)");
    HIP_TRY(hipSetDevice(pt->device));
    return run_query(pt, n, (const float4 *)rays_device, flags, out, (hipStream_t)hip_stream, nullptr, [] {});
}

int pupil_pt_query_camera(pupil_pt *pt, float jitter_x, float jitter_y, uint32_t compact, uint32_t tile_size,
                          uint32_t tile_rank, uint32_t tile_world, void *rays_out_device, const pupil_ray_hits *out,
                          void *hip_stream) {
    if (!pt) return fail(PUPIL_ERR_INVALID, "null argument");
    if (const int rc = check_query_outputs(out, 0u)) return rc;
    if ((uintptr_t)rays_out_device & 15u) return fail(PUPIL_ERR_INVALID, "misaligned ray list (16 B)");
    const uint32_t world = tile_world ? tile_world : 1u;
    const uint32_t ts = tile_size ? tile_size : 32u;
    if (tile_rank >= world) return fail(PUPIL_ERR_INVALID, "tile_rank >= tile_world");
    HIP_TRY(hipSetDevice(pt->device));
    hipStream_t s = (hipStream_t)hip_stream;
    const uint32_t key[5] = {pt->width, pt->height, ts, tile_rank, world};
    const uint32_t *map = nullptr;
    uint32_t num_local = 0;
    if (const int rc = local_pixel_map(pt, key, &map, &num_local)) return rc;
    if (num_local == 0) return PUPIL_OK;
    const uint32_t *scatter = compact ? nullptr : map;
    float4 *rays = (float4 *)rays_out_device;
    if (!rays) {
        if (!pt->flow_rays) HIP_TRY(pt->alloc(&pt->flow_rays, 2 * (size_t)pt->width * pt->height));
        rays = pt->flow_rays;
    }
    return run_query(pt, num_local, rays, 0u, out, s, scatter, [&] {
        launch_flow_rays(pt->sc, pt->width, pt->height, map, num_local, jitter_x, jitter_y, rays, s);
    });
}

int pupil_pt_query_info(pupil_pt *pt, uint64_t *queries, uint64_t *rays, uint64_t *scratch_grows, double *last_ms) {
    if (!pt) return fail(PUPIL_ERR_INVALID, "null argument");
    if (queries) *queries = pt->queries;
    if (rays) *rays = pt->query_rays;
    if (scratch_grows) *scratch_grows = pt->query_grows;
    if (last_ms) {
        *last_ms = 0.0;
        if (pt->queries) {
            HIP_TRY(hipSetDevice(pt->device));
            HIP_TRY(hipEventSynchronize(pt->ev_q1));
            float ms = 0.f;
            HIP_TRY(hipEventElapsedTime(&ms, pt->ev_q0, pt->ev_q1));
            *last_ms = ms;
        }
    }
    return PUPIL_OK;
}

extern "C++" {
namespace {

int ensure_radiance_state(pupil_pt *pt, size_t need, hipStream_t s) {
    if (need <= pt->rad_cap) return PUPIL_OK;
    if (pt->rad_block && pt->rendered) HIP_TRY(hipStreamSynchronize(pt->last_stream));
    const size_t cap = std::min(pt->rad_chunk, std::max(need, 2 * pt->rad_cap));
    auto up = [](size_t bytes) { return (bytes + 255u) & ~(size_t)255u; };
    const size_t rec = up(16 * cap), byte = up(cap);
    const size_t hist = up(sizeof(uint32_t) * partition_hist_entries((uint32_t)cap));
    const size_t total = 8 * rec + 2 * byte + up(4 * cap) + up(8 * cap) + up(4 * cap) + hist + up(4 * kCountSlots);
    if (pt->rad_block) (void)hipFree(pt->rad_block);
    pt->rad_block = nullptr;
    pt->rad_cap = 0;
    HIP_TRY(hipMalloc(&pt->rad_block, total));
    char *b = (char *)pt->rad_block;
    auto take = [&b](size_t bytes) {
        char *p = b;
        b += bytes;
        return (void *)p;
    };
    PathState &ps = pt->rad_ps;
    ps.ray_o = (float4 *)take(rec);
    ps.ray_d = (float4 *)take(rec);
    ps.hit = (float4 *)take(rec);
    ps.thr = (float4 *)take(rec);
    ps.rad = (float4 *)take(rec);
    ps.misc = (uint4 *)take(rec);
    ps.sh_d = (float4 *)take(rec);
    ps.sh_c = (float4 *)take(rec);
    ps.mbin = (uint8_t *)take(byte);
    ps.sflags = (uint8_t *)take(byte);
    Queues &q = pt->rad_q;
    q.bins = (uint32_t *)take(up(4 * cap));
    q.nxsh = (uint32_t *)take(up(8 * cap));
    pt->rad_ids = (uint32_t *)take(up(4 * cap));
    q.hist = (uint32_t *)take(hist);
    q.counts = (uint32_t *)take(up(4 * kCountSlots));
    q.work = pt->q.work + kWorkRadiance;
    q.capacity = (uint32_t)cap;
    pt->rad_cap = cap;
    pt->rad_grows++;
    launch_identity_ids(pt->rad_ids, (uint32_t)cap, s);
    return PUPIL_OK;
}

int radiance_chunk(pupil_pt *pt, hipStream_t s, const float4 *rays, const uint32_t *stream_ids,
                   const pupil_pt_launch *launch, const pupil_ray_radiance *out, uint32_t depth, uint32_t r0,
                   uint32_t nr, uint32_t s0, uint32_t ns) {
    const PathState &ps = pt->rad_ps;
    const Queues &q = pt->rad_q;
    const uint32_t np = nr * ns;
    HIP_TRY(hipMemsetAsync(ps.sflags, 0, np, s));
    if (!pt->shade_list) HIP_TRY(hipMemsetAsync(ps.mbin, 0xFF, np, s));
    launch_generate_rays(RayGenJob{rays, stream_ids, r0, nr, np, launch->random_seed + s0}, ps, s);
    FrameParams fp{};
    fp.num_local = nr;
    fp.num_paths = np;
    fp.spp = ns;
    fp.seed0 = launch->random_seed + s0;
    fp.cnt0 = launch->sample_cnt + (launch->accumulate ? s0 : 0u);
    fp.accumulate = launch->accumulate;
    fp.max_depth = depth;
    fp.compact = 1;
    fp.aov_local = 1;
    fp.group = 1;
    fp.accum = (float4 *)out->radiance + r0;
    fp.albedo = out->albedo ? (float *)out->albedo + 3 * (size_t)r0 : nullptr;
    fp.normal = out->normal ? (float *)out->normal + 3 * (size_t)r0 : nullptr;
    fp.cull_cum = pt->sc.cull_n ? pt->rad_cum : nullptr;
    for (uint32_t b = 0; b < depth; b++) {
        if (b == 0) {
            launch_extend(pt->sc, ps, q, pt->rad_ids, nullptr, np, pt->ovf, pt->ovf_threads, nullptr, s);
        } else {
            launch_partition(ps.sflags, np, 2, kPartFlags, sflag_tag(depth, b - 1), q.nxsh, q.hist, q.counts + kCntNext,
                             q.counts + kStartNext, nullptr, nullptr, s, pt->rad_cum + pupil_pt::kRadTotals, nullptr);
            if (depth > 64 && b % 16 == 0) {
                uint32_t c[2] = {1, 1};
                HIP_TRY(hipMemcpyAsync(c, q.counts + kCntNext, sizeof(c), hipMemcpyDeviceToHost, s));
                HIP_TRY(hipStreamSynchronize(s));
                if (c[0] == 0 && c[1] == 0) break;
            }
            launch_trace_mixed(pt->sc, ps, q, pt->ovf, pt->ovf_threads, nullptr, s);
        }
        if (!pt->shade_list)
            launch_partition(ps.mbin, np, kPartMaxBins, kPartExclusive, 0u, q.bins, q.hist, q.counts,
                             q.counts + kStartBins, q.counts + kScratch, nullptr, s, nullptr, nullptr, pt->bin_mask);
        if (depth > 63) HIP_TRY(hipMemsetAsync(ps.sflags, 0, np, s));
        const ShadeList list = !pt->shade_list ? kShadeBins : (b == 0 ? kShadeAll : kShadeNext);
        launch_shade(pt->sc, fp, ps, q, sflag_tag(depth, b), s, list, 0u, b == 0 ? np : 0u, np);
    }
    launch_accumulate(fp, ps, nullptr, false, s);
    return PUPIL_OK;
}

}
}

int pupil_pt_radiance_rays(pupil_pt *pt, uint32_t n, const void *rays_device, const uint32_t *stream_ids_device,
                           const pupil_pt_launch *launch, const pupil_ray_radiance *out, void *hip_stream) {
    if (!pt || !launch || !out || !out->radiance) return fail(PUPIL_ERR_INVALID, "null argument");
    if (launch->spp == 0) return fail(PUPIL_ERR_INVALID, "spp = 0");
    if (n >= (1u << 31)) return fail(PUPIL_ERR_INVALID, "too many rays in one call");
    if (((uintptr_t)rays_device & 15u) || ((uintptr_t)out->radiance & 15u) || ((uintptr_t)stream_ids_device & 3u) ||
        ((uintptr_t)out->albedo & 3u) || ((uintptr_t)out->normal & 3u))
        return fail(PUPIL_ERR_INVALID, "misaligned pointer (rays, radiance: 16 B, the others: 4 B)");
    if (n == 0) return PUPIL_OK;
    if (!rays_device) return fail(PUPIL_ERR_INVALID, "null argument");
    HIP_TRY(hipSetDevice(pt->device));
    hipStream_t s = (hipStream_t)hip_stream;
    const uint32_t depth = std::max(1u, launch->max_depth ? launch->max_depth : pt->max_depth);
    const uint32_t sb = (uint32_t)std::min<size_t>(launch->spp, pt->rad_chunk);
    const uint32_t per = (uint32_t)std::min<size_t>(n, pt->rad_chunk / sb);
    if (!pt->ev_r0) {
        HIP_TRY(hipEventCreate(&pt->ev_r0));
        HIP_TRY(hipEventCreate(&pt->ev_r1));
    }
    if (const int rc = ensure_radiance_state(pt, (size_t)sb * per, s)) return rc;
    if (pt->rendered && s != pt->last_stream) {
        HIP_TRY(hipEventRecord(pt->ev_sync, pt->last_stream));
        HIP_TRY(hipStreamWaitEvent(s, pt->ev_sync, 0));
    }
    HIP_TRY(hipEventRecord(pt->ev_r0, s));
    pt->last_stream = s;
    pt->rendered = true;
    for (uint32_t s0 = 0; s0 < launch->spp; s0 += sb)
        for (uint32_t r0 = 0; r0 < n; r0 += per)
            if (const int rc = radiance_chunk(pt, s, (const float4 *)rays_device, stream_ids_device, launch, out, depth,
                                              r0, std::min(per, n - r0), s0, std::min(sb, launch->spp - s0)))
                return rc;
    HIP_TRY(hipEventRecord(pt->ev_r1, s));
    HIP_TRY(hipGetLastError());
    pt->rad_calls++;
    pt->rad_rays += n;
    return PUPIL_OK;
}

int pupil_pt_radiance_info(pupil_pt *pt, uint64_t *calls, uint64_t *rays, uint64_t *extension_rays,
                           uint64_t *shadow_rays, uint64_t *scratch_grows, double *last_ms) {
    if (!pt) return fail(PUPIL_ERR_INVALID, "null argument");
    if (calls) *calls = pt->rad_calls;
    if (rays) *rays = pt->rad_rays;
    if (scratch_grows) *scratch_grows = pt->rad_grows;
    if (extension_rays) *extension_rays = 0;
    if (shadow_rays) *shadow_rays = 0;
    if (last_ms) *last_ms = 0.0;
    if (!pt->rad_calls || !(extension_rays || shadow_rays || last_ms)) return PUPIL_OK;
    HIP_TRY(hipSetDevice(pt->device));
    HIP_TRY(hipEventSynchronize(pt->ev_r1));
    if (extension_rays || shadow_rays) {
        std::vector<unsigned long long> cum(pupil_pt::kRadTotals + 2);
        HIP_TRY(hipMemcpy(cum.data(), pt->rad_cum, sizeof(unsigned long long) * cum.size(), hipMemcpyDeviceToHost));
        unsigned long long culled = 0;
        for (uint32_t k = 0; k < kCullShards; k++) culled += cum[k * kCullStride];
        if (extension_rays) *extension_rays = cum[pupil_pt::kRadTotals] + culled;
        if (shadow_rays) *shadow_rays = cum[pupil_pt::kRadTotals + 1];
    }
    if (last_ms) {
        float ms = 0.f;
        HIP_TRY(hipEventElapsedTime(&ms, pt->ev_r0, pt->ev_r1));
        *last_ms = ms;
    }
    return PUPIL_OK;
}

int pupil_debug_select_emitter(pupil_pt *pt, uint32_t n, const float *p, int32_t *out) {
    if (!pt || !p || !out) return fail(PUPIL_ERR_INVALID, "null argument");
    if (n == 0) return PUPIL_OK;
    HIP_TRY(hipSetDevice(pt->device));
    HIP_TRY(hipDeviceSynchronize());
    float *dp = nullptr;
    int *dout = nullptr;
    HIP_TRY(hipMalloc((void **)&dp, sizeof(float) * n));
    hipError_t err = hipMalloc((void **)&dout, sizeof(int) * n);
    if (err == hipSuccess) err = hipMemcpy(dp, p, sizeof(float) * n, hipMemcpyHostToDevice);
    if (err == hipSuccess) {
        launch_debug_select(pt->sc, dp, dout, n, pt->own_stream);
        err = hipStreamSynchronize(pt->own_stream);
    }
    if (err == hipSuccess) err = hipMemcpy(out, dout, sizeof(int) * n, hipMemcpyDeviceToHost);
    (void)hipFree(dp);
    if (dout) (void)hipFree(dout);
    HIP_TRY(err);
    return PUPIL_OK;
}

int pupil_debug_read_emitters(pupil_pt *pt, uint32_t first, uint32_t n, float *out) {
    if (!pt || (n && !out)) return fail(PUPIL_ERR_INVALID, "null argument");
    if (first > pt->sc.num_areas || n > pt->sc.num_areas - first) return fail(PUPIL_ERR_INVALID, "emitter range out of bounds");
    if (n == 0) return PUPIL_OK;
    HIP_TRY(hipSetDevice(pt->device));
    HIP_TRY(order_after_renders(pt));
    HIP_TRY(hipStreamSynchronize(pt->own_stream));
    std::vector<DevEmitter> areas(n);
    std::vector<float> cdf(n);
    HIP_TRY(hipMemcpy(areas.data(), pt->d_areas + first, sizeof(DevEmitter) * n, hipMemcpyDeviceToHost));
    HIP_TRY(hipMemcpy(cdf.data(), pt->d_cdf + first, sizeof(float) * n, hipMemcpyDeviceToHost));
    for (uint32_t e = 0; e < n; e++) {
        const DevEmitter &d = areas[e];
        float *o = out + 24 * (size_t)e;
        o[0] = d.select_probability;
        o[1] = d.area;
        o[2] = cdf[e];
        std::memcpy(o + 3, &d.type, sizeof(float));
        for (int v = 0; v < 3; v++) {
            o[4 + 3 * v] = d.pos[v].x, o[5 + 3 * v] = d.pos[v].y, o[6 + 3 * v] = d.pos[v].z;
            o[13 + 3 * v] = d.nrm[v].x, o[14 + 3 * v] = d.nrm[v].y, o[15 + 3 * v] = d.nrm[v].z;
        }
        if (d.type >= PUPIL_EMITTER_POINT) {
            o[4] = d.center.x, o[5] = d.center.y, o[6] = d.center.z;
            o[7] = d.color.x, o[8] = d.color.y, o[9] = d.color.z;
            o[10] = d.pos[0].x, o[11] = d.pos[0].y, o[12] = 0.f;
        }
        o[22] = o[23] = 0.f;
    }
    return PUPIL_OK;
}

int pupil_debug_read_emitter_guide(pupil_pt *pt, uint32_t *bits, uint32_t *guide, uint32_t *inout_count) {
    if (!pt || !inout_count) return fail(PUPIL_ERR_INVALID, "null argument");
    const uint32_t count = pt->d_guide ? (1u << pt->sc.guide_bits) + 1u : 0u;
    if (bits) *bits = pt->sc.guide_bits;
    if (guide && count) {
        if (*inout_count < count) return fail(PUPIL_ERR_INVALID, "output too small");
        HIP_TRY(hipSetDevice(pt->device));
        HIP_TRY(order_after_renders(pt));
        HIP_TRY(hipStreamSynchronize(pt->own_stream));
        HIP_TRY(hipMemcpy(guide, pt->d_guide, sizeof(uint32_t) * count, hipMemcpyDeviceToHost));
    }
    *inout_count = count;
    return PUPIL_OK;
}

extern "C++" {
namespace {
template <typename Launch>
int debug_probe(pupil_pt *pt, uint32_t n, const float *in, uint32_t in_w, float *out, uint32_t out_w, Launch launch) {
    HIP_TRY(hipSetDevice(pt->device));
    HIP_TRY(order_after_renders(pt));
    float *din = nullptr, *dout = nullptr;
    HIP_TRY(hipMalloc((void **)&din, sizeof(float) * in_w * n));
    hipError_t err = hipMalloc((void **)&dout, sizeof(float) * out_w * n);
    if (err == hipSuccess) err = hipMemcpy(din, in, sizeof(float) * in_w * n, hipMemcpyHostToDevice);
    if (err == hipSuccess) {
        launch(din, dout);
        err = hipGetLastError();
        if (err == hipSuccess) err = hipStreamSynchronize(pt->own_stream);
    }
    if (err == hipSuccess) err = hipMemcpy(out, dout, sizeof(float) * out_w * n, hipMemcpyDeviceToHost);
    (void)hipFree(din);
    if (dout) (void)hipFree(dout);
    HIP_TRY(err);
    return PUPIL_OK;
}
}
}

int pupil_debug_env(pupil_pt *pt, uint32_t n, const float *xi_or_dir, const float *pos_nrm, uint32_t mode, float *out) {
    if (!pt || !xi_or_dir || !pos_nrm || !out) return fail(PUPIL_ERR_INVALID, "null argument");
    if (mode > 1u) return fail(PUPIL_ERR_INVALID, "unknown mode");
    if (!pt->sc.has_env || !pt->d_env) return fail(PUPIL_ERR_INVALID, "the scene has no env emitter");
    if (n == 0) return PUPIL_OK;
    if (mode == 0u)
        for (uint32_t i = 0; i < n; i++)
            if (!(xi_or_dir[3 * i] >= 0.f && xi_or_dir[3 * i] <= 1.f && xi_or_dir[3 * i + 1] >= 0.f && xi_or_dir[3 * i + 1] <= 1.f))
                return fail(PUPIL_ERR_INVALID, "xi outside [0, 1]");
    return debug_probe(pt, n, xi_or_dir, 3, out, 8, [&](const float *din, float *dout) {
        launch_debug_env(pt->sc, din, pos_nrm, mode, dout, n, pt->own_stream);
    });
}

int pupil_debug_emitter_sample(pupil_pt *pt, uint32_t emitter, uint32_t n, const float *xi, const float *pos_nrm,
                               float *out) {
    if (!pt || !xi || !pos_nrm || !out) return fail(PUPIL_ERR_INVALID, "null argument");
    if (emitter > pt->sc.num_areas) return fail(PUPIL_ERR_INVALID, "emitter index beyond the env's");
    const bool env = emitter == pt->sc.num_areas;
    if (env && (!pt->sc.has_env || !pt->d_env)) return fail(PUPIL_ERR_INVALID, "the scene has no env emitter");
    if (n == 0) return PUPIL_OK;
    for (uint32_t i = 0; i < n; i++)
        if (!(xi[3 * i] >= 0.f && xi[3 * i] <= 1.f && xi[3 * i + 1] >= 0.f && xi[3 * i + 1] <= 1.f))
            return fail(PUPIL_ERR_INVALID, "xi outside [0, 1]");
    const DevEmitter *e = env ? pt->d_env : pt->d_areas + emitter;
    return debug_probe(pt, n, xi, 3, out, 8, [&](const float *din, float *dout) {
        launch_debug_emitter_sample(e, din, pos_nrm, dout, n, pt->own_stream);
    });
}

int pupil_debug_read_env_tables(pupil_pt *pt, uint32_t *width, uint32_t *height, float *col_cdf, float *row_cdf,
                                float *row_weight, float *normalization) {
    if (!pt || !width || !height) return fail(PUPIL_ERR_INVALID, "null argument");
    if (const int rc = env_map_held(pt)) return rc;
    const DevEmitter &e = pt->h_env;
    const size_t w = e.map_w, h = e.map_h;
    *width = e.map_w;
    *height = e.map_h;
    if (!col_cdf && !row_cdf && !row_weight && !normalization) return PUPIL_OK;
    HIP_TRY(hipSetDevice(pt->device));
    HIP_TRY(order_after_renders(pt));
    HIP_TRY(hipStreamSynchronize(pt->own_stream));
    if (col_cdf) HIP_TRY(hipMemcpy(col_cdf, e.col_cdf, sizeof(float) * (w + 1) * h, hipMemcpyDeviceToHost));
    if (row_cdf) HIP_TRY(hipMemcpy(row_cdf, e.row_cdf, sizeof(float) * (h + 1), hipMemcpyDeviceToHost));
    if (row_weight) HIP_TRY(hipMemcpy(row_weight, e.row_weight, sizeof(float) * h, hipMemcpyDeviceToHost));
    if (normalization)
        HIP_TRY(hipMemcpy(normalization, &pt->d_env->normalization, sizeof(float), hipMemcpyDeviceToHost));
    return PUPIL_OK;
}

int pupil_debug_tex_sample(pupil_pt *pt, uint32_t material, uint32_t slot, uint32_t n, const float *uv, float *out) {
    if (!pt || !uv || !out) return fail(PUPIL_ERR_INVALID, "null argument");
    if (material >= pt->num_mats || slot >= 4u) return fail(PUPIL_ERR_INVALID, "no such material texture");
    if (n == 0) return PUPIL_OK;
    return debug_probe(pt, n, uv, 2, out, 3, [&](const float *din, float *dout) {
        launch_debug_tex(pt->sc, material, slot, din, dout, n, pt->own_stream);
    });
}

int pupil_debug_read_material(pupil_pt *pt, uint32_t material, uint32_t *type, float out[3]) {
    if (!pt || !type || !out) return fail(PUPIL_ERR_INVALID, "null argument");
    if (material >= pt->num_mats) return fail(PUPIL_ERR_INVALID, "material index out of range");
    HIP_TRY(hipSetDevice(pt->device));
    HIP_TRY(order_after_renders(pt));
    HIP_TRY(hipStreamSynchronize(pt->own_stream));
    DevMaterial d;
    HIP_TRY(hipMemcpy(&d, pt->d_mats + material, sizeof(d), hipMemcpyDeviceToHost));
    *type = d.type;
    out[0] = d.eta;
    out[1] = d.int_fdr;
    out[2] = d.specular_sampling_weight;
    return PUPIL_OK;
}

int pupil_debug_fill_tlas_reserve(pupil_pt *pt, float value) {
    if (!pt) return fail(PUPIL_ERR_INVALID, "null argument");
    if (!pt->accel.two_level) return fail(PUPIL_ERR_UNSUPPORTED, "the flattened BVH has no TLAS reserve");
    HIP_TRY(hipSetDevice(pt->device));
    HIP_TRY(order_after_renders(pt));
    const uint64_t lo = pt->accel.tl.tlas_nodes, hi = std::min<uint64_t>(pt->accel.tl.tlas_cap, pt->accel.nodes4_count());
    if (hi > lo) {
        std::vector<float> junk((hi - lo) * (sizeof(Bvh4Node) / sizeof(float)), value);
        HIP_TRY(hipMemcpyAsync((void *)(pt->sc.nodes4 + lo), junk.data(), sizeof(float) * junk.size(),
                               hipMemcpyHostToDevice, pt->own_stream));
        HIP_TRY(hipStreamSynchronize(pt->own_stream));
    }
    if (const int rc = pt->accel.publish()) return rc;
    return derive_cull_set(pt);
}

int pupil_debug_bvh_reinsert(int device, uint32_t n, const float *boxes, uint32_t rounds, double *cost,
                             uint32_t *kept, uint32_t *rejected) {
    if (!boxes || !cost) return fail(PUPIL_ERR_INVALID, "null argument");
    if (n < 2 || rounds > 64u) return fail(PUPIL_ERR_INVALID, "needs n >= 2 boxes and at most 64 rounds");
    HIP_TRY(hipSetDevice(device));
    std::vector<Bvh4Node> nodes;
    std::vector<uint32_t> order;
    ReinsertLog log;
    if (build_bvh4_over_boxes(boxes, n, nodes, order, nullptr, nullptr, (int)rounds, &log) != 0)
        return fail(PUPIL_ERR_HIP, "the box BVH build failed");
    if (log.costs.empty()) return fail(PUPIL_ERR_HIP, "out of device memory for the reinsertion pass");
    for (uint32_t r = 0; r <= rounds; r++) cost[r] = log.costs[std::min<size_t>(r, log.costs.size() - 1)];
    if (kept) *kept = (uint32_t)log.kept;
    if (rejected) *rejected = (uint32_t)log.rejected;
    return PUPIL_OK;
}

int pupil_debug_partition(int device, uint32_t n, uint32_t capacity, const uint8_t *keys, uint32_t nbins,
                          uint32_t mode, uint32_t shift_or_tag, uint32_t bin_mask, const uint64_t *cum_in,
                          uint32_t *out, uint32_t *counts, uint32_t *starts, uint32_t *total, uint32_t *log,
                          uint64_t *cum_out, uint64_t *snap, uint32_t *info) {
    if ((!keys && n > 0) || !out || !counts || !starts) return fail(PUPIL_ERR_INVALID, "null argument");
    if (nbins < 1u || nbins > (uint32_t)kPartMaxBins) return fail(PUPIL_ERR_INVALID, "nbins must be in 1..9");
    if (mode > 1u) return fail(PUPIL_ERR_INVALID, "mode must be 0 (exclusive) or 1 (flags)");
    if (mode == 1u && nbins != 2u) return fail(PUPIL_ERR_INVALID, "the flags mode has two bins");
    if (n > capacity) return fail(PUPIL_ERR_INVALID, "n exceeds the capacity");
    if (capacity > (1u << 28)) return fail(PUPIL_ERR_INVALID, "the capacity exceeds 2^28 paths");
    if (!cum_in && (cum_out || snap)) return fail(PUPIL_ERR_INVALID, "cum_out and snap need cum_in");
    HIP_TRY(hipSetDevice(device));
    constexpr uint32_t kFill = 0xA5A5A5A5u, kGuard = 64;
    const size_t per = mode == 1u ? 2 : 1;
    const size_t hist_n = partition_hist_entries(capacity), out_n = per * capacity;
    uint32_t rounds = 0, blocks = 0;
    partition_geometry(n, &rounds, &blocks);
    if ((size_t)nbins * blocks > hist_n) return fail(PUPIL_ERR_INVALID, "the histogram would not fit its scratch");
    constexpr uint32_t kCounts = 0, kStarts = kPartMaxBins, kLog = 2 * kPartMaxBins, kTotal = 3 * kPartMaxBins;
    constexpr uint32_t kSmall = 3 * kPartMaxBins + 1;
    ScratchBuf<uint8_t> d_keys;
    ScratchBuf<uint32_t> d_hist, d_out, d_small;
    ScratchBuf<unsigned long long> d_cum;
    HIP_TRY(d_keys.alloc(n));
    HIP_TRY(d_hist.alloc(hist_n + kGuard));
    HIP_TRY(d_out.alloc(out_n + kGuard));
    HIP_TRY(d_small.alloc(kSmall));
    HIP_TRY(d_cum.alloc(2 * kPartMaxBins));
    HIP_TRY(hipMemsetD32((hipDeviceptr_t)d_hist.get(), (int)kFill, hist_n + kGuard));
    HIP_TRY(hipMemsetD32((hipDeviceptr_t)d_out.get(), (int)kFill, out_n + kGuard));
    HIP_TRY(hipMemsetD32((hipDeviceptr_t)d_small.get(), (int)kFill, kSmall));
    HIP_TRY(hipMemsetD32((hipDeviceptr_t)d_cum.get(), (int)kFill, 2 * 2 * kPartMaxBins));
    if (n) HIP_TRY(hipMemcpy(d_keys.get(), keys, n, hipMemcpyHostToDevice));
    if (cum_in) HIP_TRY(hipMemcpy(d_cum.get(), cum_in, sizeof(uint64_t) * nbins, hipMemcpyHostToDevice));
    HIP_TRY(hipDeviceSynchronize());
    launch_partition(d_keys.get(), n, nbins, mode == 1u ? kPartFlags : kPartExclusive, shift_or_tag, d_out.get(),
                     d_hist.get(), d_small.get() + kCounts, d_small.get() + kStarts, d_small.get() + kTotal,
                     d_small.get() + kLog, nullptr, cum_in ? d_cum.get() : nullptr,
                     cum_in && snap ? d_cum.get() + kPartMaxBins : nullptr, bin_mask);
    HIP_TRY(hipGetLastError());
    HIP_TRY(hipDeviceSynchronize());
    std::vector<uint32_t> h_hist(hist_n + kGuard), h_out(out_n + kGuard);
    uint32_t h_small[kSmall];
    HIP_TRY(hipMemcpy(h_hist.data(), d_hist.get(), sizeof(uint32_t) * h_hist.size(), hipMemcpyDeviceToHost));
    HIP_TRY(hipMemcpy(h_out.data(), d_out.get(), sizeof(uint32_t) * h_out.size(), hipMemcpyDeviceToHost));
    HIP_TRY(hipMemcpy(h_small, d_small.get(), sizeof(h_small), hipMemcpyDeviceToHost));
    if (cum_out) HIP_TRY(hipMemcpy(cum_out, d_cum.get(), sizeof(uint64_t) * nbins, hipMemcpyDeviceToHost));
    if (snap) HIP_TRY(hipMemcpy(snap, d_cum.get() + kPartMaxBins, sizeof(uint64_t) * nbins, hipMemcpyDeviceToHost));
    std::copy(h_out.begin(), h_out.begin() + per * n, out);
    std::copy(h_small + kCounts, h_small + kCounts + nbins, counts);
    std::copy(h_small + kStarts, h_small + kStarts + nbins, starts);
    if (log) std::copy(h_small + kLog, h_small + kLog + nbins, log);
    if (total) *total = h_small[kTotal];
    if (info) {
        const auto untouched = [](const std::vector<uint32_t> &v, size_t from) {
            return std::all_of(v.begin() + from, v.end(), [](uint32_t w) { return w == kFill; });
        };
        info[0] = rounds;
        info[1] = blocks;
        info[2] = (uint32_t)hist_n;
        info[3] = untouched(h_hist, (size_t)nbins * blocks) && untouched(h_out, per * n) ? 1u : 0u;
    }
    return PUPIL_OK;
}

int pupil_debug_math(int device, uint32_t n, const float *x, const float *y2, float *out) {
    if (!x || !y2 || !out) return fail(PUPIL_ERR_INVALID, "null argument");
    HIP_TRY(hipSetDevice(device));
    float *dx = nullptr, *dy = nullptr, *dout = nullptr;
    HIP_TRY(hipMalloc((void **)&dx, sizeof(float) * (n ? n : 1)));
    HIP_TRY(hipMalloc((void **)&dy, sizeof(float) * (n ? n : 1)));
    HIP_TRY(hipMalloc((void **)&dout, sizeof(float) * 6 * (n ? n : 1)));
    HIP_TRY(hipMemcpy(dx, x, sizeof(float) * n, hipMemcpyHostToDevice));
    HIP_TRY(hipMemcpy(dy, y2, sizeof(float) * n, hipMemcpyHostToDevice));
    launch_debug_math(dx, dy, dout, n, nullptr);
    HIP_TRY(hipDeviceSynchronize());
    HIP_TRY(hipMemcpy(out, dout, sizeof(float) * 6 * n, hipMemcpyDeviceToHost));
    (void)hipFree(dx);
    (void)hipFree(dy);
    (void)hipFree(dout);
    return PUPIL_OK;
}

}
```

### pupiloptixlab_amd/csrc/pt_kernels.h

```cpp
#pragma once

#include <vector>

#include <hip/hip_runtime.h>

#include "pt_scene.h"

namespace pupil {

constexpr int kTraceBlock = 128;
constexpr int kTraceWavesPerSimd = 7;
constexpr int kTraceWavesPerSimdTL = 5;
constexpr int kStackOvf = 160;
constexpr int kRing = 16;
constexpr int kTraceStackEntries = kRing + kStackOvf;
constexpr int kShadeBlock = 256;
constexpr uint32_t kMaxDepth = 128;
constexpr uint32_t kNumQueues = 9;
constexpr uint32_t kMissIndex = 0xFFFFFFFFu;

struct PathState {
    float4 *ray_o;
    float4 *ray_d;
    float4 *hit;
    float4 *thr;
    float4 *rad;
    uint4 *misc;
    float4 *sh_d;
    float4 *sh_c;
    uint8_t *mbin;
    uint8_t *sflags;
};

__host__ __device__ inline uint32_t sflag_tag(uint32_t max_depth, uint32_t bounce) {
    return max_depth <= 63u ? bounce % 63u + 1u : 0u;
}

constexpr int kPartMaxBins = 9;
constexpr uint32_t kCntNext = 9, kCntShadow = 10;
constexpr uint32_t kWorkShards = 8, kWorkStride = 32, kWorkKind = (2 * kWorkShards + 1) * kWorkStride;
constexpr uint32_t kWorkExtend = 0, kWorkRays = 2 * kWorkKind, kWorkFrame = 3 * kWorkKind;
constexpr uint32_t kWorkFlow = 4 * kWorkKind;
constexpr uint32_t kWorkQuery = 5 * kWorkKind;
constexpr uint32_t kWorkRadiance = 6 * kWorkKind;
constexpr uint32_t kWorkSlots = 7 * kWorkKind;
constexpr uint32_t kStartBins = 16;
constexpr uint32_t kStartNext = 25, kStartShadow = 26;
constexpr uint32_t kScratch = 27;
constexpr uint32_t kCountSlots = 32;

constexpr uint32_t kCullSetMax = 32;
constexpr uint32_t kCullShards = 64, kCullStride = 16;

struct Queues {
    uint32_t *bins;
    uint32_t *nxsh;
    uint32_t *counts;
    uint32_t *hist;
    uint32_t *work;
    uint32_t capacity;
};

enum PartMode : int {
    kPartExclusive = 0,
    kPartFlags = 1,
};

struct FrameParams {
    uint32_t width, height;
    uint32_t num_local;
    uint32_t num_paths;
    uint32_t spp;
    uint32_t seed0;
    uint32_t cnt0;
    uint32_t accumulate;
    uint32_t max_depth;
    uint32_t compact;
    const uint32_t *pixel_map;
    float4 *accum;
    float4 *frame;
    float *albedo;
    float *normal;
    float *test;
    unsigned long long *nee_count;
    unsigned long long *cull_cum;
    uint32_t aov_local;
    uint32_t group;
    uint32_t aov_frame_stride;
};

__device__ __forceinline__ float4 ld_ps(const float4 *a) {
    typedef float v4f __attribute__((ext_vector_type(4)));
    const v4f v = __builtin_nontemporal_load(reinterpret_cast<const v4f *>(a));
    return make_float4(v.x, v.y, v.z, v.w);
}
__device__ __forceinline__ uint4 ld_ps(const uint4 *a) {
    typedef unsigned v4u __attribute__((ext_vector_type(4)));
    const v4u v = __builtin_nontemporal_load(reinterpret_cast<const v4u *>(a));
    return make_uint4(v.x, v.y, v.z, v.w);
}
__device__ __forceinline__ void st_ps(float4 *a, float4 v) {
    typedef float v4f __attribute__((ext_vector_type(4)));
    v4f w = {v.x, v.y, v.z, v.w};
    __builtin_nontemporal_store(w, reinterpret_cast<v4f *>(a));
}
__device__ __forceinline__ void st_ps(uint4 *a, uint4 v) {
    typedef unsigned v4u __attribute__((ext_vector_type(4)));
    v4u w = {v.x, v.y, v.z, v.w};
    __builtin_nontemporal_store(w, reinterpret_cast<v4u *>(a));
}

#ifndef PUPIL_INST_GUIDE
#define PUPIL_INST_GUIDE 1
#endif
__device__ __forceinline__ uint32_t inst_of_prim(const DeviceScene &sc, uint32_t idx) {
    if (!PUPIL_INST_GUIDE) return sc.prim_inst[idx];
    const uint32_t k = idx >> sc.inst_guide_shift;
    uint32_t lo = sc.inst_guide[k], hi = sc.inst_guide[k + 1];
    while (lo < hi) {
        const uint32_t mid = (lo + hi + 1u) >> 1;
        if (sc.inst_first[mid] <= idx) lo = mid;
        else hi = mid - 1u;
    }
    return lo;
}

struct TraceStats {
    unsigned long long *counters;
    unsigned long long *wave_times = nullptr;
};

void launch_generate(const DeviceScene &sc, const FrameParams &fp, const PathState &ps, hipStream_t s, bool full);
void launch_extend(const DeviceScene &sc, const PathState &ps, const Queues &q, const uint32_t *queue,
                   const uint32_t *queue_count, uint32_t static_count, int *ovf, uint32_t ovf_threads,
                   const TraceStats *stats, hipStream_t s, uint32_t interleave_spp = 0, uint32_t num_local = 0);
enum ShadeList : int { kShadeBins = 0, kShadeAll = 1, kShadeNext = 2, kShadeNextRange = 3 };
void launch_shade(const DeviceScene &sc, const FrameParams &fp, const PathState &ps, const Queues &q, uint32_t tag,
                  hipStream_t s, ShadeList list, uint32_t range_base, uint32_t range_n, uint32_t max_count,
                  bool fresh_range = false, uint32_t fresh_seed0 = 0);
void launch_trace_mixed(const DeviceScene &sc, const PathState &ps, const Queues &q, int *ovf, uint32_t ovf_threads,
                        const TraceStats *stats, hipStream_t s, uint32_t ahead_count = 0, uint32_t list_base = 0,
                        uint32_t ahead_base = 0, uint32_t ahead_spp = 0, uint32_t ahead_local = 0);
bool frame_kernel_supported(const DeviceScene &sc);
void launch_frame(const DeviceScene &sc, const FrameParams &fp, const PathState &ps, uint32_t *work,
                  unsigned long long *ray_cum, int *ovf, uint32_t ovf_threads, uint32_t interleave_spp, hipStream_t s);
void launch_node_bound(const Bvh4Node *nodes, uint64_t n, uint32_t *out, hipStream_t s, bool clear = true);
void launch_accumulate(const FrameParams &fp, const PathState &ps, const float *aov_src, bool clear_flags,
                       hipStream_t s);
uint32_t trace_grid_blocks();
void launch_trace_debug(const DeviceScene &sc, const float *rays, float *out, uint32_t n, int any, int *ovf,
                        uint32_t ovf_threads, uint32_t *work, hipStream_t s, const TraceStats *stats = nullptr);
struct FlowJob {
    float world_to_sample[16];
    const float *prev_to_world;
    const uint32_t *pixel_map;
    uint32_t width, height;
    uint32_t n;
    uint32_t compact;
};
void launch_flow_rays(const DeviceScene &sc, uint32_t width, uint32_t height, const uint32_t *pixel_map, uint32_t n,
                      float jitter_x, float jitter_y, float4 *rays, hipStream_t s);
void launch_flow_project(const DeviceScene &sc, const FlowJob &job, const float4 *rays, const float4 *hits,
                         float2 *flow, hipStream_t s, const float *const *prev_verts = nullptr);
struct QueryJob {
    const float4 *rays;
    const float4 *hits;
    uint32_t n;
    uint32_t slots;
    const uint32_t *prim_slot;
    int32_t *instance, *primitive, *material;
    float *position, *normal;
    float2 *texcoord;
    const uint32_t *out_index;
    float4 *hit_out;
};
void launch_query_prim_slots(const float4 *recs, uint32_t slots, uint32_t num_prims, uint32_t *prim_slot,
                             hipStream_t s);
void launch_query_resolve(const DeviceScene &sc, const QueryJob &job, hipStream_t s);
struct RayGenJob {
    const float4 *rays;
    const uint32_t *stream_ids;
    uint32_t ray_base;
    uint32_t num_local;
    uint32_t num_paths;
    uint32_t seed0;
};
void launch_generate_rays(const RayGenJob &job, const PathState &ps, hipStream_t s);
void launch_identity_ids(uint32_t *ids, uint32_t n, hipStream_t s);
struct EmitterJob {
    DevEmitter *areas;
    float *cdf;
    uint32_t *guide;
    uint32_t guide_bits;
    uint32_t count;
    uint32_t total;
    uint32_t emitter_num;
    const DevInstance *instances;
    const uint32_t *emit_inst;
    const float *inst_weight;
    float *weight, *select;
    float *sum;
};
void launch_emitter_rebuild(const EmitterJob &job, hipStream_t s);
void launch_cull_scan(const float4 *recs, uint32_t slots, const DevInstance *instances, uint32_t num_instances,
                      uint32_t *out, uint32_t cap, hipStream_t s);
PT_HD vec3 texture_const_average(uint32_t type, const float *c0, const float *c1) {
    if (type == PUPIL_TEX_RGB) return v3(c0[0], c0[1], c0[2]);
    if (type == PUPIL_TEX_CHECKERBOARD) {
        const float r = c0[0] + c1[0];
        const float g = c0[1] + c1[1];
        const float b = c0[2] + c1[2];
        return v3(r, g, b) * 0.5f;
    }
    return v3(0.f);
}
PT_HD vec3 bitmap_average(vec3 sum, uint32_t width, uint32_t height) {
    return sum / (1.f * (float)height * (float)width);
}
PT_HD float specular_sampling_weight(vec3 diffuse_average, vec3 specular_average) {
    const float diffuse_luminance = luminance(diffuse_average);
    const float specular_luminance = luminance(specular_average);
    return specular_luminance / (specular_luminance + diffuse_luminance);
}
void launch_specular_weight(DevMaterial *mat, hipStream_t s);
void launch_record_bins(float4 *recs, uint32_t slots, const DevInstance *instances, uint32_t num_instances,
                        hipStream_t s);
constexpr uint32_t kEnvStage = 1024;
struct EnvTablesJob {
    const float4 *texels;
    uint32_t w, h;
    float *col_cdf, *row_cdf;
    const float *row_weight;
    float *col_sum;
    DevEmitter *env;
};
void launch_env_tables(const EnvTablesJob &job, hipStream_t s);
constexpr uint32_t kMoveStageFloats = 32;
constexpr uint32_t kMoveStageBox = 26;
struct MoveInstancesJob {
    DevInstance *instances;
    uint32_t num_instances, n;
    const uint32_t *ids;
    const float *to_world, *to_object;
    uint32_t margins, fallback;
    float *stage;
    uint32_t *list;
    uint8_t *moved;
    uint32_t *skipped;
};
void launch_move_instances(const MoveInstancesJob &job, hipStream_t s);
void launch_debug_math(const float *x, const float *y2, float *out, uint32_t n, hipStream_t s);
void launch_debug_select(const DeviceScene &sc, const float *p, int *out, uint32_t n, hipStream_t s);
void launch_debug_env(const DeviceScene &sc, const float *in, const float *pos_nrm, uint32_t mode, float *out, uint32_t n,
                      hipStream_t s);
void launch_debug_emitter_sample(const DevEmitter *e, const float *in, const float *pos_nrm, float *out, uint32_t n,
                                 hipStream_t s);
void launch_debug_tex(const DeviceScene &sc, uint32_t material, uint32_t slot, const float *uv, float *out, uint32_t n,
                      hipStream_t s);

uint32_t partition_hist_entries(uint32_t n);
void partition_geometry(uint32_t n, uint32_t *rounds, uint32_t *blocks);
void launch_partition(const uint8_t *keys, uint32_t n, uint32_t nbins, PartMode mode, uint32_t shift, uint32_t *out,
                      uint32_t *hist, uint32_t *counts_out, uint32_t *starts_out, uint32_t *total_out, uint32_t *log_out,
                      hipStream_t s, unsigned long long *cum_out = nullptr, unsigned long long *snap_out = nullptr,
                      uint32_t bin_mask = 0u);

struct BvhBuildInput {
    uint32_t num_prims;
    const uint32_t *prim_inst;
    const DevInstance *instances;
    const DevMaterial *materials;
    uint32_t object_space;
};
struct BvhBuildOutput {
    Bvh4Node *nodes4;
    float4 *prims;
    float4 *attrs;
    uint32_t root_link4;
    uint32_t num_nodes4;
    uint32_t depth4;
    uint32_t num_records = 0;
    std::vector<uint32_t> level_start;
};
int build_lbvh(const BvhBuildInput &in, BvhBuildOutput &out, uint32_t leaf_size, hipStream_t s, double *build_ms,
               bool force_lbvh = false);
int build_bvh_bounded(const BvhBuildInput &in, BvhBuildOutput &out, uint32_t leaf_size, hipStream_t s,
                      double *build_ms, uint32_t reserve);
void free_lbvh(BvhBuildOutput &out);
int refit_bvh4(const BvhBuildInput &in, BvhBuildOutput &out, const uint8_t *moved, float *nbox, hipStream_t s,
               double *ms, bool records_only = false);
void launch_refit_levels(Bvh4Node *nodes, const std::vector<uint32_t> &level_start, uint32_t node_base,
                         const float4 *recs, float *nbox, hipStream_t s);
void launch_refresh_attrs(const BvhBuildInput &in, const BvhBuildOutput &out, const uint8_t *moved, hipStream_t s);
void launch_refresh_attrs_shape(float4 *attrs, uint32_t n, const float *positions, const float *normals,
                                const uint32_t *indices, hipStream_t s);
struct ReinsertLog {
    std::vector<double> costs;
    int kept = 0;
    int rejected = 0;
};
int build_bvh4_over_boxes(const float *h_boxes, uint32_t n, std::vector<Bvh4Node> &nodes,
                          std::vector<uint32_t> &order, uint32_t *depth, hipStream_t s, int rounds = -1,
                          ReinsertLog *log = nullptr);

}
```

### pupiloptixlab_amd/csrc/pt_kernels.hip

```cpp
#include "pt_kernels.h"
#include "pt_shade.h"
#include "pt_shading.h"
#include "pt_trace.h"
#include "pt_traverse.h"

#include <cstdlib>
#include <algorithm>

namespace pupil {

namespace {

using namespace tr;

__global__ __launch_bounds__(kShadeBlock) void k_generate(DeviceScene sc, FrameParams fp, PathState ps, uint32_t full) {
    const uint32_t p = blockIdx.x * blockDim.x + threadIdx.x;
    if (p >= fp.num_paths) return;
    vec3 dir;
    const uint32_t rng = fresh_path(sc, fp, p, fp.seed0, dir);
    st_ps(ps.ray_d + p, make_float4(dir.x, dir.y, dir.z, 0.f));
    if (!full) return;
    st_ps(ps.ray_o + p, f4(camera_origin(sc.camera), 0.f));
    st_ps(ps.thr + p, make_float4(1.f, 1.f, 1.f, 0.f));
    st_ps(ps.rad + p, make_float4(0.f, 0.f, 0.f, 0.f));
    st_ps(ps.misc + p, make_uint4(rng, 0u, 0u, 0u));
}

template <int LIST>
__global__ __launch_bounds__(kShadeBlock) __attribute__((amdgpu_waves_per_eu(4))) void k_shade_all(DeviceScene sc, FrameParams fp, PathState ps, Queues q,
                                                           uint32_t tag, uint32_t range_base, uint32_t range_n,
                                                           uint32_t fresh_range, uint32_t fresh_seed0) {
    const uint32_t n_list = LIST == kShadeNext || LIST == kShadeNextRange ? q.counts[kCntNext] : 0u;
    const uint32_t count = LIST == kShadeBins ? q.counts[kScratch]
                                              : n_list + (LIST == kShadeAll || LIST == kShadeNextRange ? range_n : 0u);
    uint32_t start[kPartMaxBins];
#pragma unroll
    for (int b = 0; b < kPartMaxBins; b++) start[b] = LIST == kShadeBins ? q.counts[kStartBins + b] : 0u;
    const uint32_t stride = gridDim.x * blockDim.x;
    for (uint32_t i = blockIdx.x * blockDim.x + threadIdx.x; i < count; i += stride) {
        const uint32_t p = LIST == kShadeBins ? q.bins[i] : (i < n_list ? q.nxsh[i] : range_base + (i - n_list));
        uint32_t bin = 0;
        if (LIST == kShadeBins) {
#pragma unroll
            for (int b = 1; b < kPartMaxBins; b++) bin = i >= start[b] ? (uint32_t)b : bin;
        } else if (sc.single_bin) {
            bin = __float_as_uint(ld_ps(ps.hit + p).w) == kMissIndex ? 0u : sc.single_bin;
        } else {
            bin = ps.mbin[p];
        }
        const bool fresh = LIST != kShadeBins && fresh_range && i >= n_list;
        const uint32_t fresh_p = p - range_base;
        uint32_t flags = 0;
        switch (bin) {
        case 0: shade_miss(sc, fp, ps, p, fresh, fresh_p, fresh_seed0); break;
        case PUPIL_MAT_DIFFUSE: flags = shade_hit<PUPIL_MAT_DIFFUSE>(sc, fp, ps, p, fresh, fresh_p, fresh_seed0); break;
        case PUPIL_MAT_DIELECTRIC: flags = shade_hit<PUPIL_MAT_DIELECTRIC>(sc, fp, ps, p, fresh, fresh_p, fresh_seed0); break;
        case PUPIL_MAT_ROUGH_DIELECTRIC:
            flags = shade_hit<PUPIL_MAT_ROUGH_DIELECTRIC>(sc, fp, ps, p, fresh, fresh_p, fresh_seed0);
            break;
        case PUPIL_MAT_CONDUCTOR: flags = shade_hit<PUPIL_MAT_CONDUCTOR>(sc, fp, ps, p, fresh, fresh_p, fresh_seed0); break;
        case PUPIL_MAT_ROUGH_CONDUCTOR:
            flags = shade_hit<PUPIL_MAT_ROUGH_CONDUCTOR>(sc, fp, ps, p, fresh, fresh_p, fresh_seed0);
            break;
        case PUPIL_MAT_PLASTIC: flags = shade_hit<PUPIL_MAT_PLASTIC>(sc, fp, ps, p, fresh, fresh_p, fresh_seed0); break;
        case PUPIL_MAT_ROUGH_PLASTIC: flags = shade_hit<PUPIL_MAT_ROUGH_PLASTIC>(sc, fp, ps, p, fresh, fresh_p, fresh_seed0); break;
        default: flags = shade_hit<0u>(sc, fp, ps, p, fresh, fresh_p, fresh_seed0); break;
        }
        if (fp.nee_count) {
            const unsigned long long m = __ballot((flags & 4u) != 0u);
            if (m && __lane_id() == __ffsll((unsigned long long)__builtin_amdgcn_read_exec()) - 1)
                atomicAdd(fp.nee_count, (unsigned long long)__popcll(m));
        }
        count_culled(fp, flags);
        ps.sflags[p] = (uint8_t)((flags & 3u) | tag << 2);
        if (LIST == kShadeBins) ps.mbin[p] = 0xFFu;
    }
}

constexpr int shade_one_waves(uint32_t mat) { return mat == PUPIL_MAT_DIFFUSE ? 5 : 4; }
template <int LIST, uint32_t MAT>
__global__ __launch_bounds__(kShadeBlock) __attribute__((amdgpu_waves_per_eu(shade_one_waves(MAT)))) void k_shade_one(
    DeviceScene sc, FrameParams fp, PathState ps, Queues q, uint32_t tag, uint32_t range_base, uint32_t range_n,
    uint32_t fresh_range, uint32_t fresh_seed0) {
    static_assert(LIST != kShadeBins, "single-material shading walks a list");
    const uint32_t n_list = LIST == kShadeNext || LIST == kShadeNextRange ? q.counts[kCntNext] : 0u;
    const uint32_t count = n_list + (LIST == kShadeAll || LIST == kShadeNextRange ? range_n : 0u);
    const uint32_t stride = gridDim.x * blockDim.x;
    for (uint32_t i = blockIdx.x * blockDim.x + threadIdx.x; i < count; i += stride) {
        const uint32_t p = i < n_list ? q.nxsh[i] : range_base + (i - n_list);
        const bool miss = __float_as_uint(ld_ps(ps.hit + p).w) == kMissIndex;
        const bool fresh = fresh_range && i >= n_list;
        const uint32_t fresh_p = p - range_base;
        uint32_t flags = 0;
        if (miss) shade_miss(sc, fp, ps, p, fresh, fresh_p, fresh_seed0);
        else flags = shade_hit<MAT>(sc, fp, ps, p, fresh, fresh_p, fresh_seed0);
        if (fp.nee_count) {
            const unsigned long long m = __ballot((flags & 4u) != 0u);
            if (m && __lane_id() == __ffsll((unsigned long long)__builtin_amdgcn_read_exec()) - 1)
                atomicAdd(fp.nee_count, (unsigned long long)__popcll(m));
        }
        count_culled(fp, flags);
        ps.sflags[p] = (uint8_t)((flags & 3u) | tag << 2);
    }
}

__global__ __launch_bounds__(kShadeBlock) void k_accumulate(FrameParams fp, PathState ps, const float *aov_src,
                                                             uint32_t clear_flags) {
    const uint32_t l = blockIdx.x * blockDim.x + threadIdx.x;
    if (l >= fp.num_local) return;
    const uint32_t out = fp.compact ? l : global_pixel(fp, l);
    if (aov_src) {
        const uint32_t n = fp.num_local;
        if (fp.albedo)
            for (int k = 0; k < 3; k++) fp.albedo[3 * out + k] = aov_src[3 * l + k];
        if (fp.normal)
            for (int k = 0; k < 3; k++) fp.normal[3 * out + k] = aov_src[3 * n + 3 * l + k];
        if (fp.test) fp.test[out] = aov_src[6 * n + l];
    }
    vec3 acc = f3(fp.accum[out]);
    constexpr uint32_t kBatch = 8;
    for (uint32_t s0 = 0; s0 < fp.spp; s0 += kBatch) {
        float4 rad[kBatch];
#pragma unroll
        for (uint32_t j = 0; j < kBatch; j++)
            if (s0 + j < fp.spp) rad[j] = ps.rad[(size_t)(s0 + j) * fp.num_local + l];
#pragma unroll
        for (uint32_t j = 0; j < kBatch; j++) {
            const uint32_t s = s0 + j;
            if (s >= fp.spp) break;
            if (clear_flags) ps.sflags[(size_t)s * fp.num_local + l] = 0u;
            vec3 L = f3(rad[j]);
            const uint32_t cnt = fp.cnt0 + (fp.accumulate ? s : 0u);
            if (fp.accumulate && cnt > 0) {
                const float t = 1.f / ((float)cnt + 1.f);
                L = lerp(acc, L, t);
            }
            acc = L;
        }
    }
    fp.accum[out] = f4(acc, 1.f);
    if (fp.frame) fp.frame[out] = f4(acc, 1.f);
}


__global__ void k_debug_math(const float *x, const float *y2, float *out, uint32_t n) {
    const uint32_t i = blockIdx.x * blockDim.x + threadIdx.x;
    if (i >= n) return;
    const float a = x[i], b = y2[i];
    float s, c;
    dm_sincos(a, s, c);
    out[6 * i + 0] = s;
    out[6 * i + 1] = c;
    out[6 * i + 2] = dm_acos(fminf(fmaxf(a, -1.f), 1.f));
    out[6 * i + 3] = dm_atan2(a, b);
    out[6 * i + 4] = sqrtf(fabs_(a));
    out[6 * i + 5] = 1.0f / a;
}

}


__global__ void k_debug_select(DeviceScene sc, const float *p, int *out, uint32_t n) {
    const uint32_t i = blockIdx.x * blockDim.x + threadIdx.x;
    if (i >= n) return;
    float prob;
    const DevEmitter *e = select_emitter(sc, p[i], prob);
    out[i] = !e ? -2 : (e == sc.env && sc.has_env ? -1 : (int)(e - sc.areas));
}

__global__ void k_debug_env(DeviceScene sc, const float *in, vec3 pos, vec3 nrm, uint32_t mode, float *out, uint32_t n) {
    const uint32_t i = blockIdx.x * blockDim.x + threadIdx.x;
    if (i >= n) return;
    const DevEmitter &e = *sc.env;
    float *o = out + 8 * (size_t)i;
    if (mode == 0u) {
        LocalGeo g;
        g.position = pos;
        g.normal = nrm;
        g.texcoord = v2(0.f, 0.f);
        const EmitterSample r = emitter_sample_direct(e, g, v2(in[3 * i], in[3 * i + 1]));
        o[0] = r.wi.x, o[1] = r.wi.y, o[2] = r.wi.z;
        o[3] = r.pdf;
        o[4] = r.distance;
        o[5] = r.radiance.x, o[6] = r.radiance.y, o[7] = r.radiance.z;
    } else {
        vec3 radiance;
        float pdf;
        env_eval(e, pos, v3(in[3 * i], in[3 * i + 1], in[3 * i + 2]), radiance, pdf);
        o[0] = radiance.x, o[1] = radiance.y, o[2] = radiance.z;
        o[3] = pdf;
        o[4] = o[5] = o[6] = o[7] = 0.f;
    }
}

__global__ void k_debug_emitter_sample(const DevEmitter *e, const float *in, vec3 pos, vec3 nrm, float *out, uint32_t n) {
    const uint32_t i = blockIdx.x * blockDim.x + threadIdx.x;
    if (i >= n) return;
    LocalGeo g;
    g.position = pos;
    g.normal = nrm;
    g.texcoord = v2(0.f, 0.f);
    const EmitterSample r = emitter_sample_direct(*e, g, v2(in[3 * i], in[3 * i + 1]));
    float *o = out + 8 * (size_t)i;
    o[0] = r.wi.x, o[1] = r.wi.y, o[2] = r.wi.z;
    o[3] = r.pdf;
    o[4] = r.distance;
    o[5] = r.radiance.x, o[6] = r.radiance.y, o[7] = r.radiance.z;
}

void launch_debug_emitter_sample(const DevEmitter *e, const float *in, const float *pos_nrm, float *out, uint32_t n,
                                 hipStream_t s) {
    hipLaunchKernelGGL(k_debug_emitter_sample, dim3((n + 255) / 256), dim3(256), 0, s, e, in,
                       v3(pos_nrm[0], pos_nrm[1], pos_nrm[2]), v3(pos_nrm[3], pos_nrm[4], pos_nrm[5]), out, n);
}

__global__ void k_debug_tex(const DevMaterial *mat, uint32_t slot, const float *uv, float *out, uint32_t n) {
    const uint32_t i = blockIdx.x * blockDim.x + threadIdx.x;
    if (i >= n) return;
    const vec3 c = tex_sample(mat->tex[slot], v2(uv[2 * i], uv[2 * i + 1]));
    out[3 * i] = c.x, out[3 * i + 1] = c.y, out[3 * i + 2] = c.z;
}

void launch_debug_env(const DeviceScene &sc, const float *in, const float *pos_nrm, uint32_t mode, float *out, uint32_t n,
                      hipStream_t s) {
    hipLaunchKernelGGL(k_debug_env, dim3((n + 255) / 256), dim3(256), 0, s, sc, in, v3(pos_nrm[0], pos_nrm[1], pos_nrm[2]),
                       v3(pos_nrm[3], pos_nrm[4], pos_nrm[5]), mode, out, n);
}

void launch_debug_tex(const DeviceScene &sc, uint32_t material, uint32_t slot, const float *uv, float *out, uint32_t n,
                      hipStream_t s) {
    hipLaunchKernelGGL(k_debug_tex, dim3((n + 255) / 256), dim3(256), 0, s, sc.materials + material, slot, uv, out, n);
}

void launch_debug_select(const DeviceScene &sc, const float *p, int *out, uint32_t n, hipStream_t s) {
    hipLaunchKernelGGL(k_debug_select, dim3((n + 255) / 256), dim3(256), 0, s, sc, p, out, n);
}

void launch_debug_math(const float *x, const float *y2, float *out, uint32_t n, hipStream_t s) {
    hipLaunchKernelGGL(k_debug_math, dim3((n + 255) / 256), dim3(256), 0, s, x, y2, out, n);
}


void launch_generate(const DeviceScene &sc, const FrameParams &fp, const PathState &ps, hipStream_t s, bool full) {
    const uint32_t blocks = (fp.num_paths + kShadeBlock - 1) / kShadeBlock;
    hipLaunchKernelGGL(k_generate, dim3(blocks), dim3(kShadeBlock), 0, s, sc, fp, ps, full ? 1u : 0u);
}


static uint32_t shade_blocks(uint32_t num_paths) {
    static const int forced = [] {
        const char *e = std::getenv("PUPIL_SHADE_BLOCKS");
        return e ? std::min(1 << 20, std::max(64, std::atoi(e))) : 0;
    }();
    if (forced) return (uint32_t)forced;
    return std::max(64u, std::min(1u << 20, (num_paths + kShadeBlock - 1) / kShadeBlock));
}

void launch_shade(const DeviceScene &sc, const FrameParams &fp, const PathState &ps, const Queues &q, uint32_t tag,
                  hipStream_t s, ShadeList list, uint32_t range_base, uint32_t range_n, uint32_t max_count,
                  bool fresh_range, uint32_t fresh_seed0) {
    const dim3 g(shade_blocks(max_count)), b(kShadeBlock);
    const uint32_t fr = fresh_range && list != kShadeBins ? 1u : 0u;
#define SHADE(L) \
    hipLaunchKernelGGL(k_shade_all<L>, g, b, 0, s, sc, fp, ps, q, tag, range_base, range_n, fr, fresh_seed0)
#define SHADE1(L, M) \
    hipLaunchKernelGGL((k_shade_one<L, M>), g, b, 0, s, sc, fp, ps, q, tag, range_base, range_n, fr, fresh_seed0)
#define SHADE1_ALL(L)                                                       \
    switch (sc.single_bin) {                                                \
    case PUPIL_MAT_DIFFUSE: SHADE1(L, PUPIL_MAT_DIFFUSE); break;             \
    case PUPIL_MAT_DIELECTRIC: SHADE1(L, PUPIL_MAT_DIELECTRIC); break;       \
    case PUPIL_MAT_ROUGH_DIELECTRIC: SHADE1(L, PUPIL_MAT_ROUGH_DIELECTRIC); break; \
    case PUPIL_MAT_CONDUCTOR: SHADE1(L, PUPIL_MAT_CONDUCTOR); break;         \
    case PUPIL_MAT_ROUGH_CONDUCTOR: SHADE1(L, PUPIL_MAT_ROUGH_CONDUCTOR); break; \
    case PUPIL_MAT_PLASTIC: SHADE1(L, PUPIL_MAT_PLASTIC); break;             \
    case PUPIL_MAT_ROUGH_PLASTIC: SHADE1(L, PUPIL_MAT_ROUGH_PLASTIC); break; \
    default: SHADE1(L, 0u); break;                                          \
    }
    static const bool one = [] {
        const char *e = std::getenv("PUPIL_SHADE_ONE");
        return !e || std::atoi(e) != 0;
    }();
    if (one && sc.single_bin && list != kShadeBins) {
        switch (list) {
        case kShadeAll: SHADE1_ALL(kShadeAll); break;
        case kShadeNext: SHADE1_ALL(kShadeNext); break;
        default: SHADE1_ALL(kShadeNextRange); break;
        }
        return;
    }
    switch (list) {
    case kShadeAll: SHADE(kShadeAll); break;
    case kShadeNext: SHADE(kShadeNext); break;
    case kShadeNextRange: SHADE(kShadeNextRange); break;
    default: SHADE(kShadeBins); break;
    }
#undef SHADE
#undef SHADE1
#undef SHADE1_ALL
}


void launch_accumulate(const FrameParams &fp, const PathState &ps, const float *aov_src, bool clear_flags,
                       hipStream_t s) {
    const uint32_t blocks = (fp.num_local + kShadeBlock - 1) / kShadeBlock;
    hipLaunchKernelGGL(k_accumulate, dim3(blocks), dim3(kShadeBlock), 0, s, fp, ps, aov_src, clear_flags ? 1u : 0u);
}

}
```

### pupiloptixlab_amd/csrc/pt_scene.h

```cpp
#pragma once

#include "../../include/pupil_pt.h"
#include "accel_limits.h"
#include "pt_math.h"

namespace pupil {

struct DevTexture {
    uint32_t type;
    uint32_t width, height;
    uint32_t filter;
    float c0[3];
    float c1[3];
    float r0[4];
    float r1[4];
    const float4 *data;
};

struct DevMaterial {
    uint32_t type;
    uint32_t twosided;
    uint32_t nonlinear;
    float eta;
    float int_fdr;
    float specular_sampling_weight;
    float pad[2];
    DevTexture tex[4];
};

struct DevEmitter {
    uint32_t type;
    float select_probability;
    float area;
    float radius;
    DevTexture radiance;
    vec3 pos[3];
    vec3 nrm[3];
    vec2 tex[3];
    vec3 center;
    vec3 color;
    float scale;
    float normalization;
    uint32_t map_w, map_h;
    float to_world[9];
    float to_local[9];
    const float *row_cdf;
    const float *col_cdf;
    const float *row_weight;
};

struct DevInstance {
    float to_world[12];
    float to_object[12];
    uint32_t kind;
    uint32_t material;
    uint32_t prim_offset;
    int32_t emitter_offset;
    uint32_t flip_normals;
    uint32_t flip_tex_coords;
    const float *positions;
    const float *normals;
    const float *texcoords;
    const uint32_t *indices;
    int32_t blas_root;
    uint32_t attr_base;
    uint32_t bin;
    float margin[2];
    float wlo[3], whi[3];
    int32_t wrec_delta;
    uint32_t rec_base;
    uint32_t obj_nbase, obj_ncount, wnode_base;
    float vmax;
    uint32_t hidden;
};
static_assert(sizeof(DevInstance) == 224, "DevInstance stride");

inline DevInstance device_instance(const DevInstance &d) {
    DevInstance o = d;
    if (d.hidden && d.kind == PUPIL_SHAPE_SPHERE)
        for (float &x : o.to_object) x = __builtin_nanf("");
    return o;
}

struct alignas(64) Bvh4Node {
    float ox, oy, oz;
    float sx;
    int32_t child[4];
    uint32_t qlo_x, qlo_y, qlo_z;
    uint32_t qhi_x, qhi_y, qhi_z;
    float sy, sz;
};
constexpr int kEmptyLink = 0x7FFFFFFF;
constexpr uint32_t kTopNodes = 16;
constexpr uint64_t kMaxNodes4 = 1ull << 26;
constexpr int kTraverseDone = 0x76543210;
constexpr int kReturnLink = 0x7654321F;


constexpr uint32_t kPrimSphereBit = 0x80000000u;
constexpr uint32_t kRecF4 = 4;
constexpr uint32_t kRecHole = 0xFFFFFFFFu;
PT_HD uint32_t leaf_slots(uint32_t count) { return (count + 1u) & ~1u; }
constexpr uint32_t kAttrStride = 8;

struct Camera {
    float s2c[16];
    float c2w[16];
};

struct DeviceScene {
    const Bvh4Node *nodes4;
    const float4 *prims;
    const float4 *attrs;
    uint32_t num_prims;
    uint32_t root_link4;
    uint32_t trace_refill;
    uint32_t num_cus;
    uint32_t trace_node_min;
    uint32_t top_nodes;
    float node_bound[3];
    uint32_t single_bin;
    uint32_t tl_world;
    uint32_t two_level;
    const float4 *wprims;
    const uint32_t *prim_inst;
    const uint32_t *inst_first;
    const uint32_t *inst_guide;
    uint32_t inst_guide_shift;
    const DevInstance *instances;
    const DevMaterial *materials;
    const DevEmitter *areas;
    const float *area_cdf;
    const uint32_t *area_guide;
    uint32_t guide_bits;
    uint32_t num_areas;
    uint32_t has_env;
    const DevEmitter *env;
    const uint32_t *cull_set;
    uint32_t cull_n;
    Camera camera;
};

}
```

### pupiloptixlab_amd/csrc/pt_shade.h

```cpp
#pragma once

#include "pt_kernels.h"
#include "pt_shading.h"
#include "pt_trace.h"
#include "pt_traverse.h"

namespace pupil {
namespace {

using namespace tr;

__device__ __forceinline__ uint32_t camera_path(const Camera &cam, uint32_t width, uint32_t height,
                                                const uint32_t *pixel_map, uint32_t num_local, uint32_t seed0,
                                                uint32_t p, uint32_t &pixel, vec3 &dir) {
    const uint32_t s = p / num_local;
    const uint32_t l = p - s * num_local;
    pixel = pixel_map ? pixel_map[l] : l;
    uint32_t rng = rng_init(pixel, seed0 + s);
    const float jx = rng_next(rng);
    const float jy = rng_next(rng);
    const uint32_t y = pixel / width;
    const uint32_t x = pixel - y * width;
    const vec4 film = v4(((float)x + jx) / (float)width, ((float)y + jy) / (float)height, 0.f, 1.f);
    const float *m = cam.s2c;
    vec4 d = v4(dot(v4(m[0], m[1], m[2], m[3]), film), dot(v4(m[4], m[5], m[6], m[7]), film),
                dot(v4(m[8], m[9], m[10], m[11]), film), dot(v4(m[12], m[13], m[14], m[15]), film));
    const float inv_w = 1.0f / d.w;
    d = v4(d.x * inv_w, d.y * inv_w, d.z * inv_w, d.w * inv_w);
    d.w = 0.f;
    d = normalize(d);
    const float *c = cam.c2w;
    dir = normalize(v3(dot(v4(c[0], c[1], c[2], c[3]), d), dot(v4(c[4], c[5], c[6], c[7]), d),
                       dot(v4(c[8], c[9], c[10], c[11]), d)));
    return rng;
}


__device__ __forceinline__ uint32_t global_pixel(const FrameParams &fp, uint32_t l) {
    return fp.pixel_map ? fp.pixel_map[l] : l;
}

__device__ __forceinline__ uint32_t fresh_path(const DeviceScene &sc, const FrameParams &fp, uint32_t p, uint32_t seed0,
                                               vec3 &dir) {
    uint32_t pixel;
    return camera_path(sc.camera, fp.width, fp.height, fp.pixel_map, fp.num_local, seed0, p, pixel, dir);
}
__device__ __forceinline__ uint32_t fresh_rng_of(const FrameParams &fp, uint32_t p, uint32_t seed0) {
    const uint32_t s = p / fp.num_local;
    const uint32_t l = p - s * fp.num_local;
    uint32_t rng = rng_init(fp.pixel_map ? fp.pixel_map[l] : l, seed0 + s);
    (void)rng_next(rng);
    (void)rng_next(rng);
    return rng;
}

struct HitGeo {
    LocalGeo g;
    int emitter;
    uint32_t inst;
};

__device__ __forceinline__ HitGeo reconstruct(const DeviceScene &sc, float4 h, const float4 *ro_rec, bool fresh,
                                             vec3 rd, vec2 stale_uv) {
    HitGeo out;
    const uint32_t idx = __float_as_uint(h.w);
    uint32_t inst_id, gprim;
    bool sphere;
    const float4 *rec;
    float4 ra[7];
    if (sc.two_level) {
        gprim = idx;
        inst_id = inst_of_prim(sc, idx);
        const DevInstance &ti = sc.instances[inst_id];
        sphere = ti.kind == PUPIL_SHAPE_SPHERE;
        rec = sc.attrs + (size_t)kAttrStride * (sphere ? 0u : ti.attr_base + (idx - ti.prim_offset));
        for (int k = 0; k < 7; k++) ra[k] = rec[k];
    } else {
        rec = sc.attrs + (size_t)kAttrStride * idx;
        for (int k = 0; k < 7; k++) ra[k] = rec[k];
        asm volatile("" ::"v"(ra[0].x), "v"(ra[0].y), "v"(ra[0].z), "v"(ra[0].w), "v"(ra[1].x), "v"(ra[1].y),
                     "v"(ra[1].z), "v"(ra[1].w), "v"(ra[2].x), "v"(ra[2].y), "v"(ra[2].z), "v"(ra[2].w), "v"(ra[3].x),
                     "v"(ra[3].y));
        asm volatile("" ::"v"(ra[3].z), "v"(ra[3].w), "v"(ra[4].x), "v"(ra[4].y), "v"(ra[4].z), "v"(ra[4].w),
                     "v"(ra[5].x), "v"(ra[5].y), "v"(ra[5].z), "v"(ra[5].w), "v"(ra[6].x), "v"(ra[6].y));
        const uint32_t ref = __float_as_uint(ra[0].w);
        gprim = ref & ~kPrimSphereBit;
        sphere = (ref & kPrimSphereBit) != 0u;
        inst_id = __float_as_uint(ra[1].w);
    }
    const DevInstance &in = sc.instances[inst_id];
    out.inst = inst_id;
    LocalGeo &g = out.g;
    g.texcoord = stale_uv;
    uint32_t local = 0;
    if (sphere) {
        const vec3 ro = fresh ? camera_origin(sc.camera) : f3(ld_ps(ro_rec));
        g.position = ro + h.x * rd;
        const vec3 local_pos = xform_point(in.to_object, g.position);
        g.texcoord = sphere_texcoord(normalize(local_pos - v3(0.f)));
        g.normal = normalize(xform_normal(in.to_object, local_pos - v3(0.f)));
        if (in.flip_normals) g.normal = g.normal * -1.f;
    } else {
        local = gprim - in.prim_offset;
        const float4 a = ra[0];
        const float4 b = ra[1];
        const float4 c = ra[2];
        const vec3 p0 = v3(a.x, a.y, a.z);
        const vec3 p1 = v3(b.x, b.y, b.z);
        const vec3 p2 = v3(c.x, c.y, c.z);
        const float u = h.y, v = h.z;
        const float w = 1.f - u - v;
        g.position = w * p0 + u * p1 + v * p2;
        g.position = xform_point(in.to_world, g.position);
        vec3 n;
        if (in.normals) {
            const float4 d = ra[3], e = ra[4];
            const vec3 n0 = v3(c.w, d.x, d.y);
            const vec3 n1 = v3(d.z, d.w, e.x);
            const vec3 n2 = v3(e.y, e.z, e.w);
            n = w * n0 + u * n1 + v * n2;
        } else {
            n = cross(p1 - p0, p2 - p0);
        }
        g.normal = normalize(xform_normal(in.to_object, n));
        if (in.flip_normals) g.normal = g.normal * -1.f;
        if (in.texcoords) {
            const float4 t01 = ra[5], t2 = ra[6];
            const vec2 t0 = v2(t01.x, t01.y);
            const vec2 t1 = v2(t01.z, t01.w);
            const vec2 tt2 = v2(t2.x, t2.y);
            g.texcoord = w * t0 + u * t1 + v * tt2;
            if (in.flip_tex_coords) g.texcoord.y = 1.f - g.texcoord.y;
        }
    }
    out.emitter = in.emitter_offset >= 0 ? in.emitter_offset + (int)local : -1;
    return out;
}

__device__ __forceinline__ const DevEmitter *select_emitter(const DeviceScene &sc, float p, float &sel_prob) {
    uint32_t lo = 0, hi = sc.num_areas;
    if (sc.area_guide) {
        const uint32_t m = 1u << sc.guide_bits;
        const uint32_t k = min((uint32_t)(p * (float)m), m - 1u);
        lo = sc.area_guide[k];
        hi = sc.area_guide[k + 1];
    }
    while (lo < hi) {
        const uint32_t mid = (lo + hi) >> 1;
        if (p <= sc.area_cdf[mid]) hi = mid;
        else lo = mid + 1;
    }
    const DevEmitter *e = nullptr;
    if (lo < sc.num_areas) e = &sc.areas[lo];
    else if (sc.has_env) e = sc.env;
    else if (sc.num_areas > 0) e = &sc.areas[sc.num_areas - 1];
    sel_prob = e ? e->select_probability : 0.f;
    return e;
}

__device__ __forceinline__ bool last_sample(const FrameParams &fp, uint32_t p, uint32_t &l, uint32_t &frame_off) {
    const uint32_t q = p / fp.num_local;
    l = p - q * fp.num_local;
    const uint32_t s = q / fp.spp;
    frame_off = fp.aov_frame_stride ? (s % fp.group) * fp.aov_frame_stride : 0u;
    return q - s * fp.spp + 1u == fp.spp;
}

__device__ __forceinline__ bool terminal_ray_culled(const DeviceScene &sc, vec3 o, vec3 d) {
    const RayPre r = ray_pre(o, d);
    bool hit = false;
    for (uint32_t k = 0; k < sc.cull_n; k++) {
        const uint32_t i = sc.cull_set[k];
        const float4 a = sc.prims[kRecF4 * i + 0];
        const float4 b = sc.prims[kRecF4 * i + 1];
        const float4 c = sc.prims[kRecF4 * i + 2];
        float t, b1, b2;
        if (__float_as_uint(a.w) & kPrimSphereBit)
            hit = hit || intersect_unit_sphere(sc.instances[__float_as_uint(b.w)].to_object, r.o, d, 0.001f,
                                               kMaxDistance, t);
        else
            hit = hit || intersect_triangle(r, v3(a.x, a.y, a.z), v3(b.x, b.y, b.z), v3(c.x, c.y, c.z), 0.001f,
                                            kMaxDistance, t, b1, b2);
    }
    return !hit;
}

template <uint32_t MAT>
__device__ __forceinline__ uint32_t shade_hit(const DeviceScene &sc, const FrameParams &fp, const PathState &ps,
                                              uint32_t p, bool fresh, uint32_t fresh_p, uint32_t fresh_seed0) {
    bool push_next = false, push_shadow = false, culled = false;
    const float4 h = ld_ps(ps.hit + p);
    const vec3 ray_d = f3(ld_ps(ps.ray_d + p));
    const uint32_t fresh_rng = fresh ? fresh_rng_of(fp, fresh_p, fresh_seed0) : 0u;
    const uint4 misc = fresh ? make_uint4(fresh_rng, 0u, 0u, 0u) : ld_ps(ps.misc + p);
    uint32_t rng = misc.x;
    const uint32_t flags = misc.y;
    const uint32_t bounce = flags & 0xFFFFFFu;
    float4 thr4 = fresh ? make_float4(1.f, 1.f, 1.f, 0.f) : ld_ps(ps.thr + p);
    vec3 T = f3(thr4);
    const float prev_pdf = thr4.w;
    vec3 L_add = v3(0.f);
    const vec2 stale_uv = v2(__uint_as_float(misc.z), __uint_as_float(misc.w));

    HitGeo hg = reconstruct(sc, h, ps.ray_o + p, fresh, ray_d, stale_uv);
    const DevInstance &in = sc.instances[hg.inst];
    const DevMaterial &mat = sc.materials[in.material];
    if (mat.twosided && dot(-ray_d, hg.g.normal) < 0.f) hg.g.normal = -hg.g.normal;
    const LocalGeo &geo = hg.g;
    LocalBsdf bsdf = local_bsdf(mat, geo.texcoord);
    bsdf.type = MAT;

    bool alive = true;
    bool L_changed = fresh;
    if (bounce == 0) {
        if (hg.emitter >= 0) {
            L_add = emitter_radiance(sc.areas[hg.emitter], geo.texcoord);
            L_changed = true;
        }
        const float test = rng_next(rng);
        uint32_t l;
        uint32_t fo;
        if (last_sample(fp, p, l, fo)) {
            const uint32_t out = fp.aov_local ? l : global_pixel(fp, l);
            if (fp.albedo) {
                const vec3 al = bsdf_albedo(bsdf);
                fp.albedo[fo + 3 * out + 0] = al.x;
                fp.albedo[fo + 3 * out + 1] = al.y;
                fp.albedo[fo + 3 * out + 2] = al.z;
            }
            if (fp.normal) {
                fp.normal[fo + 3 * out + 0] = geo.normal.x;
                fp.normal[fo + 3 * out + 1] = geo.normal.y;
                fp.normal[fo + 3 * out + 2] = geo.normal.z;
            }
            if (fp.test) fp.test[fo + out] = test;
        }
    } else if (hg.emitter >= 0) {
        const DevEmitter &e = sc.areas[hg.emitter];
        vec3 Le;
        float pdf_e;
        emitter_eval_area(e, geo, f3(ld_ps(ps.ray_o + p)), Le, pdf_e);
        if (!is_zero(pdf_e)) {
            const float mis = (flags >> 31) ? 1.f : mis_weight(prev_pdf, pdf_e * e.select_probability);
            L_add = T * Le * mis;
            L_changed = true;
        }
    }

    const uint32_t depth = bounce + 1;
    if (depth >= fp.max_depth) alive = false;
    if (alive) {
        const float rr = depth > 2 ? 0.95f : 1.0f;
        if (rng_next(rng) > rr) alive = false;
        else T = T / rr;
    }
    float pdf_b = 0.f, sh_tmax = 0.f;
    uint32_t delta = 0;
    const bool nee = alive;
    if (alive) {
        float sel_prob;
        const DevEmitter *e = select_emitter(sc, rng_next(rng), sel_prob);
        const float x0 = rng_next(rng);
        const float x1 = rng_next(rng);
        const vec3 wo = to_local(-ray_d, geo.normal);
        if (e) {
            const EmitterSample es = emitter_sample_direct(*e, geo, v2(x0, x1));
            BsdfRec er;
            er.wi = to_local(es.wi, geo.normal);
            er.wo = wo;
            er.f = v3(0.f);
            er.pdf = 0.f;
            bsdf_eval_t<MAT>(bsdf, er);
            if (!is_zero(er.f * es.pdf)) {
                const float NoL = dot(geo.normal, es.wi);
                if (NoL > 0.f) {
                    const float mis = es.is_delta ? 1.f : mis_weight(es.pdf, er.pdf);
                    const float pdf_l = es.pdf * sel_prob;
                    const vec3 C = T * es.radiance * er.f * NoL * mis / pdf_l;
                    sh_tmax = es.distance - 0.001f;
                    st_ps(ps.sh_d + p, f4(es.wi, 0.f));
                    st_ps(ps.sh_c + p, f4(C, 0.f));
                    push_shadow = true;
                }
            }
        }
        BsdfRec br;
        br.wo = wo;
        br.wi = v3(0.f);
        br.f = v3(0.f);
        br.pdf = 0.f;
        br.sampled_type = 0;
        bsdf_sample_t<MAT>(bsdf, br, rng);
        if (is_zero(br.f * fabs_(br.wi.z)) || is_zero(br.pdf)) {
            alive = false;
        } else {
            T = T * (br.f * fabs_(br.wi.z) / br.pdf);
            const vec3 nd = to_world(br.wi, geo.normal);
            pdf_b = br.pdf;
            delta = (br.sampled_type & kLobeDelta) ? 1u : 0u;
            if (fp.cull_cum && bounce + 2u >= fp.max_depth && terminal_ray_culled(sc, geo.position, nd)) {
                culled = true;
            } else {
                st_ps(ps.ray_d + p, f4(nd, 0.f));
                push_next = true;
            }
        }
    }
    if (push_shadow || push_next) st_ps(ps.ray_o + p, f4(geo.position, sh_tmax));
    if (push_next) {
        st_ps(ps.thr + p, f4(T, pdf_b));
        st_ps(ps.misc + p, make_uint4(rng, (bounce + 1) | (delta << 31), __float_as_uint(geo.texcoord.x),
                                __float_as_uint(geo.texcoord.y)));
    }
    if (L_changed) {
        const vec3 L = f3(fresh ? make_float4(0.f, 0.f, 0.f, 0.f) : ld_ps(ps.rad + p)) + L_add;
        st_ps(ps.rad + p, f4(L, 0.f));
    }
    return (push_next ? 1u : 0u) | (push_shadow ? 2u : 0u) | (nee ? 4u : 0u) | (culled ? 8u : 0u);
}

__device__ __forceinline__ void count_culled(const FrameParams &fp, uint32_t flags) {
    if (!fp.cull_cum) return;
    const unsigned long long m = __ballot((flags & 8u) != 0u);
    if (m && __lane_id() == __ffsll((unsigned long long)__builtin_amdgcn_read_exec()) - 1)
        atomicAdd(fp.cull_cum + (blockIdx.x % kCullShards) * kCullStride, (unsigned long long)__popcll(m));
}

__device__ __forceinline__ void shade_miss(const DeviceScene &sc, const FrameParams &fp, const PathState &ps,
                                           uint32_t p, bool fresh, uint32_t fresh_p, uint32_t fresh_seed0) {
    const uint32_t fresh_rng = fresh ? fresh_rng_of(fp, fresh_p, fresh_seed0) : 0u;
    const uint4 misc = fresh ? make_uint4(fresh_rng, 0u, 0u, 0u) : ld_ps(ps.misc + p);
    if ((misc.y & 0xFFFFFFu) == 0u) {
        float4 rad4 = fresh ? make_float4(0.f, 0.f, 0.f, 0.f) : ld_ps(ps.rad + p);
        vec3 L = f3(rad4);
        uint32_t rng = misc.x;
        if (sc.has_env) {
            vec3 Le;
            float pdf;
            const vec3 ro = fresh ? camera_origin(sc.camera) : f3(ld_ps(ps.ray_o + p));
            env_eval(*sc.env, ro, f3(ld_ps(ps.ray_d + p)), Le, pdf);
            L = L + Le;
        }
        const float test = rng_next(rng);
        uint32_t l;
        uint32_t fo;
        if (last_sample(fp, p, l, fo)) {
            const uint32_t out = fp.aov_local ? l : global_pixel(fp, l);
            if (fp.albedo) fp.albedo[fo + 3 * out] = fp.albedo[fo + 3 * out + 1] = fp.albedo[fo + 3 * out + 2] = 0.f;
            if (fp.normal) fp.normal[fo + 3 * out] = fp.normal[fo + 3 * out + 1] = fp.normal[fo + 3 * out + 2] = 0.f;
            if (fp.test) fp.test[fo + out] = test;
        }
        st_ps(ps.rad + p, f4(L, 0.f));
    } else if (sc.has_env) {
        const float4 thr4 = ld_ps(ps.thr + p);
        vec3 Le;
        float env_pdf;
        env_eval(*sc.env, f3(ld_ps(ps.ray_o + p)), f3(ld_ps(ps.ray_d + p)), Le, env_pdf);
        const float mis = mis_weight(thr4.w, env_pdf);
        const vec3 env_rad = Le * (f3(thr4) * mis);
        float4 rad4 = ld_ps(ps.rad + p);
        st_ps(ps.rad + p, f4(f3(rad4) + env_rad, 0.f));
    }
}

}
}
```

Measured before the change: 7464 Mrays/s.

## Stage instance, material, emitter and cull tables into LDS in shade kernels

Shade kernels now copy the small per-scene tables (instances, materials, area emitters with CDF and guide, env emitter, terminal-cull records) into shared memory at block start when they fit the fixed capacities, and all lookups go through a table abstraction. This aims to replace scattered global or cached loads in shading with LDS reads. The shade grid is also capped at a maximum block count, with a grid-stride loop covering the rest, so staging is paid by fewer blocks. The cost is a per-block staging copy plus a barrier, and a large static LDS allocation that may reduce occupancy.

```diff
diff --git a/include/pupil_pt.h b/include/pupil_pt.h
--- a/include/pupil_pt.h
+++ b/include/pupil_pt.h
@@ -276,6 +276,7 @@
 int pupil_debug_emitter_sample(pupil_pt *pt, uint32_t emitter, uint32_t n, const float *xi, const float *pos_nrm,
                                float *out);
 int pupil_debug_read_emitter_guide(pupil_pt *pt, uint32_t *bits, uint32_t *guide, uint32_t *inout_count);
+int pupil_debug_shade_tables(pupil_pt *pt, uint32_t caps[4], uint32_t *fit);
 int pupil_debug_env(pupil_pt *pt, uint32_t n, const float *xi_or_dir, const float *pos_nrm, uint32_t mode, float *out);
 int pupil_debug_read_env_tables(pupil_pt *pt, uint32_t *width, uint32_t *height, float *col_cdf, float *row_cdf,
                                 float *row_weight, float *normalization);
diff --git a/pupiloptixlab_amd/abi.py b/pupiloptixlab_amd/abi.py
--- a/pupiloptixlab_amd/abi.py
+++ b/pupiloptixlab_amd/abi.py
@@ -159,6 +159,7 @@
     "pupil_debug_read_material": (C.c_int, [C.c_void_p, C.c_uint32, u32p, f32p]),
     "pupil_debug_read_emitters": (C.c_int, [C.c_void_p, C.c_uint32, C.c_uint32, f32p]),
     "pupil_debug_read_emitter_guide": (C.c_int, [C.c_void_p, u32p, u32p, u32p]),
+    "pupil_debug_shade_tables": (C.c_int, [C.c_void_p, u32p, u32p]),
     "pupil_debug_fill_tlas_reserve": (C.c_int, [C.c_void_p, C.c_float]),
     "pupil_pt_render": (C.c_int, [C.c_void_p, C.POINTER(Frame), C.POINTER(Launch), C.c_void_p]),
     "pupil_pt_stats": (C.c_int, [C.c_void_p, C.POINTER(Counters)]),
diff --git a/pupiloptixlab_amd/csrc/engine.hip b/pupiloptixlab_amd/csrc/engine.hip
--- a/pupiloptixlab_amd/csrc/engine.hip
+++ b/pupiloptixlab_amd/csrc/engine.hip
@@ -851,6 +851,8 @@
     sc.inst_guide_shift = guide_shift;
     sc.instances = pt->d_insts;
     sc.materials = pt->d_mats;
+    sc.num_instances = (uint32_t)insts.size();
+    sc.num_materials = (uint32_t)mats.size();
     return PUPIL_OK;
 }
 
@@ -900,6 +902,9 @@
     if (const char *g = std::getenv("PUPIL_FRAME_PATHS")) pt->knobs.frame_paths = std::max(0.0, std::atof(g));
     if (const char *g = std::getenv("PUPIL_RADIANCE_CHUNK"))
         pt->rad_chunk = (size_t)std::min(2147483647.0, std::max(64.0, std::atof(g)));
+    sc.shade_max_blocks = kShadeMaxBlocks;
+    if (const char *g = std::getenv("PUPIL_SHADE_MAX_BLOCKS"))
+        sc.shade_max_blocks = (uint32_t)std::min(1 << 20, std::max(64, std::atoi(g)));
     sc.trace_node_min = 8;
     if (const char *r = std::getenv("PUPIL_NODE_MIN")) sc.trace_node_min = (uint32_t)std::min(64, std::max(1, std::atoi(r)));
 }
@@ -2376,6 +2381,15 @@
             o[10] = d.pos[0].x, o[11] = d.pos[0].y, o[12] = 0.f;
         }
         o[22] = o[23] = 0.f;
+    }
+    return PUPIL_OK;
+}
+
+int pupil_debug_shade_tables(pupil_pt *pt, uint32_t caps[4], uint32_t *fit) {
+    if (caps) shade_table_caps(caps);
+    if (fit) {
+        if (!pt) return fail(PUPIL_ERR_INVALID, "null argument");
+        *fit = shade_tables_fit(pt->sc);
     }
     return PUPIL_OK;
 }
diff --git a/pupiloptixlab_amd/csrc/pt_kernels.h b/pupiloptixlab_amd/csrc/pt_kernels.h
--- a/pupiloptixlab_amd/csrc/pt_kernels.h
+++ b/pupiloptixlab_amd/csrc/pt_kernels.h
@@ -15,6 +15,7 @@
 constexpr int kRing = 16;
 constexpr int kTraceStackEntries = kRing + kStackOvf;
 constexpr int kShadeBlock = 256;
+constexpr uint32_t kShadeMaxBlocks = 16384;
 constexpr uint32_t kMaxDepth = 128;
 constexpr uint32_t kNumQueues = 9;
 constexpr uint32_t kMissIndex = 0xFFFFFFFFu;
@@ -138,6 +139,8 @@
 void launch_shade(const DeviceScene &sc, const FrameParams &fp, const PathState &ps, const Queues &q, uint32_t tag,
                   hipStream_t s, ShadeList list, uint32_t range_base, uint32_t range_n, uint32_t max_count,
                   bool fresh_range = false, uint32_t fresh_seed0 = 0);
+void shade_table_caps(uint32_t caps[4]);
+uint32_t shade_tables_fit(const DeviceScene &sc);
 void launch_trace_mixed(const DeviceScene &sc, const PathState &ps, const Queues &q, int *ovf, uint32_t ovf_threads,
                         const TraceStats *stats, hipStream_t s, uint32_t ahead_count = 0, uint32_t list_base = 0,
                         uint32_t ahead_base = 0, uint32_t ahead_spp = 0, uint32_t ahead_local = 0);
diff --git a/pupiloptixlab_amd/csrc/pt_kernels.hip b/pupiloptixlab_amd/csrc/pt_kernels.hip
--- a/pupiloptixlab_amd/csrc/pt_kernels.hip
+++ b/pupiloptixlab_amd/csrc/pt_kernels.hip
@@ -26,19 +26,74 @@
     st_ps(ps.misc + p, make_uint4(rng, 0u, 0u, 0u));
 }
 
-template <int LIST>
+__device__ __forceinline__ void stage_copy(uint32_t *dst, const void *src, uint32_t bytes) {
+    const uint32_t n16 = bytes / 16u;
+    for (uint32_t i = threadIdx.x; i < n16; i += kShadeBlock)
+        reinterpret_cast<uint4 *>(dst)[i] = reinterpret_cast<const uint4 *>(src)[i];
+    for (uint32_t i = 4u * n16 + threadIdx.x; i < bytes / 4u; i += kShadeBlock)
+        dst[i] = reinterpret_cast<const uint32_t *>(src)[i];
+}
+
+template <int TAB>
+__device__ __forceinline__ BlockTables stage_tables(const DeviceScene &sc, uint32_t fit, uint32_t *s) {
+    const bool f_inst = TAB == 1 || (fit & 1u), f_mat = TAB == 1 || (fit & 2u), f_area = TAB == 1 || (fit & 4u),
+               f_cull = TAB == 1 || (fit & 8u);
+    uint32_t *s_inst = s + kTabOffInst / 4u, *s_mat = s + kTabOffMat / 4u, *s_area = s + kTabOffArea / 4u,
+             *s_cdf = s + kTabOffCdf / 4u, *s_guide = s + kTabOffGuide / 4u, *s_crec = s + kTabOffCullRec / 4u,
+             *s_cobj = s + kTabOffCullObj / 4u;
+    uint32_t *s_env = s_area + kTabAreas * (uint32_t)(sizeof(DevEmitter) / 4u);
+    if (f_inst) stage_copy(s_inst, sc.instances, sc.num_instances * (uint32_t)sizeof(DevInstance));
+    if (f_mat) stage_copy(s_mat, sc.materials, sc.num_materials * (uint32_t)sizeof(DevMaterial));
+    if (f_area) {
+        stage_copy(s_area, sc.areas, sc.num_areas * (uint32_t)sizeof(DevEmitter));
+        stage_copy(s_cdf, sc.area_cdf, sc.num_areas * 4u);
+        if (sc.area_guide) stage_copy(s_guide, sc.area_guide, ((1u << sc.guide_bits) + 1u) * 4u);
+        if (sc.has_env) stage_copy(s_env, sc.env, (uint32_t)sizeof(DevEmitter));
+    }
+    if (f_cull && threadIdx.x < sc.cull_n) {
+        const uint32_t k = threadIdx.x, i = sc.cull_set[k];
+        const float4 a = sc.prims[kRecF4 * i + 0];
+        reinterpret_cast<float4 *>(s_crec)[3 * k + 0] = a;
+        const float4 b = sc.prims[kRecF4 * i + 1];
+        reinterpret_cast<float4 *>(s_crec)[3 * k + 1] = b;
+        reinterpret_cast<float4 *>(s_crec)[3 * k + 2] = sc.prims[kRecF4 * i + 2];
+        if (__float_as_uint(a.w) & kPrimSphereBit) {
+            const float *t = sc.instances[__float_as_uint(b.w)].to_object;
+            for (int j = 0; j < 12; j++) reinterpret_cast<float *>(s_cobj)[12 * k + j] = t[j];
+        }
+    }
+    __syncthreads();
+    return BlockTables{f_inst ? reinterpret_cast<const DevInstance *>(s_inst) : sc.instances,
+                       f_mat ? reinterpret_cast<const DevMaterial *>(s_mat) : sc.materials,
+                       f_area ? reinterpret_cast<const DevEmitter *>(s_area) : sc.areas,
+                       f_area ? reinterpret_cast<const DevEmitter *>(s_env) : sc.env,
+                       f_area ? reinterpret_cast<const float *>(s_cdf) : sc.area_cdf,
+                       f_area ? reinterpret_cast<const uint32_t *>(s_guide) : sc.area_guide,
+                       f_cull ? reinterpret_cast<const float4 *>(s_crec) : nullptr,
+                       reinterpret_cast<const float *>(s_cobj),
+                       sc};
+}
+
+template <int LIST, int TAB>
 __global__ __launch_bounds__(kShadeBlock) __attribute__((amdgpu_waves_per_eu(4))) void k_shade_all(DeviceScene sc, FrameParams fp, PathState ps, Queues q,
                                                            uint32_t tag, uint32_t range_base, uint32_t range_n,
-                                                           uint32_t fresh_range, uint32_t fresh_seed0) {
+                                                           uint32_t fresh_range, uint32_t fresh_seed0, uint32_t fit) {
+    __shared__ uint4 s_tab[kTabBytes / 16u];
     const uint32_t n_list = LIST == kShadeNext || LIST == kShadeNextRange ? q.counts[kCntNext] : 0u;
     const uint32_t count = LIST == kShadeBins ? q.counts[kScratch]
                                               : n_list + (LIST == kShadeAll || LIST == kShadeNextRange ? range_n : 0u);
     uint32_t start[kPartMaxBins];
 #pragma unroll
     for (int b = 0; b < kPartMaxBins; b++) start[b] = LIST == kShadeBins ? q.counts[kStartBins + b] : 0u;
+    if (blockIdx.x * blockDim.x >= count) return;
+    const BlockTables tb = stage_tables<TAB>(sc, fit, reinterpret_cast<uint32_t *>(s_tab));
     const uint32_t stride = gridDim.x * blockDim.x;
-    for (uint32_t i = blockIdx.x * blockDim.x + threadIdx.x; i < count; i += stride) {
-        const uint32_t p = LIST == kShadeBins ? q.bins[i] : (i < n_list ? q.nxsh[i] : range_base + (i - n_list));
+    auto path_of = [&](uint32_t k) {
+        return LIST == kShadeBins ? q.bins[k] : (k < n_list ? q.nxsh[k] : range_base + (k - n_list));
+    };
+    uint32_t i = blockIdx.x * blockDim.x + threadIdx.x;
+    for (; i < count; i += stride) {
+        const uint32_t p = path_of(i);
         uint32_t bin = 0;
         if (LIST == kShadeBins) {
 #pragma unroll
@@ -52,19 +107,19 @@
         const uint32_t fresh_p = p - range_base;
         uint32_t flags = 0;
         switch (bin) {
-        case 0: shade_miss(sc, fp, ps, p, fresh, fresh_p, fresh_seed0); break;
-        case PUPIL_MAT_DIFFUSE: flags = shade_hit<PUPIL_MAT_DIFFUSE>(sc, fp, ps, p, fresh, fresh_p, fresh_seed0); break;
-        case PUPIL_MAT_DIELECTRIC: flags = shade_hit<PUPIL_MAT_DIELECTRIC>(sc, fp, ps, p, fresh, fresh_p, fresh_seed0); break;
+        case 0: shade_miss(sc, tb, fp, ps, p, fresh, fresh_p, fresh_seed0); break;
+        case PUPIL_MAT_DIFFUSE: flags = shade_hit<PUPIL_MAT_DIFFUSE>(sc, tb, fp, ps, p, fresh, fresh_p, fresh_seed0); break;
+        case PUPIL_MAT_DIELECTRIC: flags = shade_hit<PUPIL_MAT_DIELECTRIC>(sc, tb, fp, ps, p, fresh, fresh_p, fresh_seed0); break;
         case PUPIL_MAT_ROUGH_DIELECTRIC:
-            flags = shade_hit<PUPIL_MAT_ROUGH_DIELECTRIC>(sc, fp, ps, p, fresh, fresh_p, fresh_seed0);
+            flags = shade_hit<PUPIL_MAT_ROUGH_DIELECTRIC>(sc, tb, fp, ps, p, fresh, fresh_p, fresh_seed0);
             break;
-        case PUPIL_MAT_CONDUCTOR: flags = shade_hit<PUPIL_MAT_CONDUCTOR>(sc, fp, ps, p, fresh, fresh_p, fresh_seed0); break;
+        case PUPIL_MAT_CONDUCTOR: flags = shade_hit<PUPIL_MAT_CONDUCTOR>(sc, tb, fp, ps, p, fresh, fresh_p, fresh_seed0); break;
         case PUPIL_MAT_ROUGH_CONDUCTOR:
-            flags = shade_hit<PUPIL_MAT_ROUGH_CONDUCTOR>(sc, fp, ps, p, fresh, fresh_p, fresh_seed0);
+            flags = shade_hit<PUPIL_MAT_ROUGH_CONDUCTOR>(sc, tb, fp, ps, p, fresh, fresh_p, fresh_seed0);
             break;
-        case PUPIL_MAT_PLASTIC: flags = shade_hit<PUPIL_MAT_PLASTIC>(sc, fp, ps, p, fresh, fresh_p, fresh_seed0); break;
-        case PUPIL_MAT_ROUGH_PLASTIC: flags = shade_hit<PUPIL_MAT_ROUGH_PLASTIC>(sc, fp, ps, p, fresh, fresh_p, fresh_seed0); break;
-        default: flags = shade_hit<0u>(sc, fp, ps, p, fresh, fresh_p, fresh_seed0); break;
+        case PUPIL_MAT_PLASTIC: flags = shade_hit<PUPIL_MAT_PLASTIC>(sc, tb, fp, ps, p, fresh, fresh_p, fresh_seed0); break;
+        case PUPIL_MAT_ROUGH_PLASTIC: flags = shade_hit<PUPIL_MAT_ROUGH_PLASTIC>(sc, tb, fp, ps, p, fresh, fresh_p, fresh_seed0); break;
+        default: flags = shade_hit<0u>(sc, tb, fp, ps, p, fresh, fresh_p, fresh_seed0); break;
         }
         if (fp.nee_count) {
             const unsigned long long m = __ballot((flags & 4u) != 0u);
@@ -78,22 +133,27 @@
 }
 
 constexpr int shade_one_waves(uint32_t mat) { return mat == PUPIL_MAT_DIFFUSE ? 5 : 4; }
-template <int LIST, uint32_t MAT>
+template <int LIST, uint32_t MAT, int TAB>
 __global__ __launch_bounds__(kShadeBlock) __attribute__((amdgpu_waves_per_eu(shade_one_waves(MAT)))) void k_shade_one(
     DeviceScene sc, FrameParams fp, PathState ps, Queues q, uint32_t tag, uint32_t range_base, uint32_t range_n,
-    uint32_t fresh_range, uint32_t fresh_seed0) {
+    uint32_t fresh_range, uint32_t fresh_seed0, uint32_t fit) {
     static_assert(LIST != kShadeBins, "single-material shading walks a list");
+    __shared__ uint4 s_tab[kTabBytes / 16u];
     const uint32_t n_list = LIST == kShadeNext || LIST == kShadeNextRange ? q.counts[kCntNext] : 0u;
     const uint32_t count = n_list + (LIST == kShadeAll || LIST == kShadeNextRange ? range_n : 0u);
+    if (blockIdx.x * blockDim.x >= count) return;
+    const BlockTables tb = stage_tables<TAB>(sc, fit, reinterpret_cast<uint32_t *>(s_tab));
     const uint32_t stride = gridDim.x * blockDim.x;
-    for (uint32_t i = blockIdx.x * blockDim.x + threadIdx.x; i < count; i += stride) {
-        const uint32_t p = i < n_list ? q.nxsh[i] : range_base + (i - n_list);
+    auto path_of = [&](uint32_t k) { return k < n_list ? q.nxsh[k] : range_base + (k - n_list); };
+    uint32_t i = blockIdx.x * blockDim.x + threadIdx.x;
+    for (; i < count; i += stride) {
+        const uint32_t p = path_of(i);
         const bool miss = __float_as_uint(ld_ps(ps.hit + p).w) == kMissIndex;
         const bool fresh = fresh_range && i >= n_list;
         const uint32_t fresh_p = p - range_base;
         uint32_t flags = 0;
-        if (miss) shade_miss(sc, fp, ps, p, fresh, fresh_p, fresh_seed0);
-        else flags = shade_hit<MAT>(sc, fp, ps, p, fresh, fresh_p, fresh_seed0);
+        if (miss) shade_miss(sc, tb, fp, ps, p, fresh, fresh_p, fresh_seed0);
+        else flags = shade_hit<MAT>(sc, tb, fp, ps, p, fresh, fresh_p, fresh_seed0);
         if (fp.nee_count) {
             const unsigned long long m = __ballot((flags & 4u) != 0u);
             if (m && __lane_id() == __ffsll((unsigned long long)__builtin_amdgcn_read_exec()) - 1)
@@ -247,24 +307,48 @@
 }
 
 
-static uint32_t shade_blocks(uint32_t num_paths) {
+static uint32_t shade_blocks(uint32_t num_paths, uint32_t max_blocks) {
     static const int forced = [] {
         const char *e = std::getenv("PUPIL_SHADE_BLOCKS");
         return e ? std::min(1 << 20, std::max(64, std::atoi(e))) : 0;
     }();
     if (forced) return (uint32_t)forced;
-    return std::max(64u, std::min(1u << 20, (num_paths + kShadeBlock - 1) / kShadeBlock));
+    const uint32_t cap = max_blocks ? max_blocks : kShadeMaxBlocks;
+    return std::max(64u, std::min(cap, (num_paths + kShadeBlock - 1) / kShadeBlock));
+}
+
+void shade_table_caps(uint32_t caps[4]) {
+    caps[0] = kTabInstances, caps[1] = kTabMaterials, caps[2] = kTabAreas, caps[3] = kTabCull;
+}
+uint32_t shade_tables_fit(const DeviceScene &sc) {
+    static const uint32_t mask = [] {
+        const char *e = std::getenv("PUPIL_SHADE_TABLES");
+        return e ? (uint32_t)std::atoi(e) & 15u : 15u;
+    }();
+    const bool areas = sc.num_areas <= kTabAreas && (!sc.area_guide || (1u << sc.guide_bits) <= kTabAreas);
+    return ((sc.num_instances <= kTabInstances ? 1u : 0u) | (sc.num_materials <= kTabMaterials ? 2u : 0u) |
+            (areas ? 4u : 0u) | (sc.cull_n <= kTabCull ? 8u : 0u)) & mask;
 }
 
 void launch_shade(const DeviceScene &sc, const FrameParams &fp, const PathState &ps, const Queues &q, uint32_t tag,
                   hipStream_t s, ShadeList list, uint32_t range_base, uint32_t range_n, uint32_t max_count,
                   bool fresh_range, uint32_t fresh_seed0) {
-    const dim3 g(shade_blocks(max_count)), b(kShadeBlock);
+    const dim3 g(shade_blocks(max_count, sc.shade_max_blocks)), b(kShadeBlock);
     const uint32_t fr = fresh_range && list != kShadeBins ? 1u : 0u;
-#define SHADE(L) \
-    hipLaunchKernelGGL(k_shade_all<L>, g, b, 0, s, sc, fp, ps, q, tag, range_base, range_n, fr, fresh_seed0)
-#define SHADE1(L, M) \
-    hipLaunchKernelGGL((k_shade_one<L, M>), g, b, 0, s, sc, fp, ps, q, tag, range_base, range_n, fr, fresh_seed0)
+    const uint32_t fit = shade_tables_fit(sc);
+#define SHADE(L)                                                                                                       \
+    if (fit == 15u)                                                                                                    \
+        hipLaunchKernelGGL((k_shade_all<L, 1>), g, b, 0, s, sc, fp, ps, q, tag, range_base, range_n, fr, fresh_seed0,  \
+                           fit);                                                                                       \
+    else                                                                                                               \
+        hipLaunchKernelGGL((k_shade_all<L, 2>), g, b, 0, s, sc, fp, ps, q, tag, range_base, range_n, fr, fresh_seed0, fit)
+#define SHADE1(L, M)                                                                                                   \
+    if (fit == 15u)                                                                                                    \
+        hipLaunchKernelGGL((k_shade_one<L, M, 1>), g, b, 0, s, sc, fp, ps, q, tag, range_base, range_n, fr,            \
+                           fresh_seed0, fit);                                                                          \
+    else                                                                                                               \
+        hipLaunchKernelGGL((k_shade_one<L, M, 2>), g, b, 0, s, sc, fp, ps, q, tag, range_base, range_n, fr,            \
+                           fresh_seed0, fit)
 #define SHADE1_ALL(L)                                                       \
     switch (sc.single_bin) {                                                \
     case PUPIL_MAT_DIFFUSE: SHADE1(L, PUPIL_MAT_DIFFUSE); break;             \
diff --git a/pupiloptixlab_amd/csrc/pt_scene.h b/pupiloptixlab_amd/csrc/pt_scene.h
--- a/pupiloptixlab_amd/csrc/pt_scene.h
+++ b/pupiloptixlab_amd/csrc/pt_scene.h
@@ -127,6 +127,7 @@
     const uint32_t *inst_first;
     const uint32_t *inst_guide;
     uint32_t inst_guide_shift;
+    uint32_t num_instances;
     const DevInstance *instances;
     const DevMaterial *materials;
     const DevEmitter *areas;
@@ -135,10 +136,12 @@
     uint32_t guide_bits;
     uint32_t num_areas;
     uint32_t has_env;
+    uint32_t num_materials;
     const DevEmitter *env;
     const uint32_t *cull_set;
     uint32_t cull_n;
     Camera camera;
+    uint32_t shade_max_blocks;
 };
 
 }
diff --git a/pupiloptixlab_amd/csrc/pt_shade.h b/pupiloptixlab_amd/csrc/pt_shade.h
--- a/pupiloptixlab_amd/csrc/pt_shade.h
+++ b/pupiloptixlab_amd/csrc/pt_shade.h
@@ -54,14 +54,76 @@
     return rng;
 }
 
+struct GlobalTables {
+    const DeviceScene &sc;
+    __device__ __forceinline__ const DevInstance &instance(uint32_t i) const { return sc.instances[i]; }
+    __device__ __forceinline__ const DevMaterial &material(uint32_t i) const { return sc.materials[i]; }
+    __device__ __forceinline__ const DevEmitter &area(uint32_t i) const { return sc.areas[i]; }
+    __device__ __forceinline__ const DevEmitter *env() const { return sc.env; }
+    __device__ __forceinline__ float area_cdf(uint32_t i) const { return sc.area_cdf[i]; }
+    __device__ __forceinline__ uint32_t area_guide(uint32_t k) const { return sc.area_guide[k]; }
+    __device__ __forceinline__ void cull_record(uint32_t k, float4 &a, float4 &b, float4 &c) const {
+        const uint32_t i = sc.cull_set[k];
+        a = sc.prims[kRecF4 * i + 0];
+        b = sc.prims[kRecF4 * i + 1];
+        c = sc.prims[kRecF4 * i + 2];
+    }
+    __device__ __forceinline__ const float *cull_to_object(uint32_t k, float4 b) const {
+        return sc.instances[__float_as_uint(b.w)].to_object;
+    }
+};
+
+constexpr uint32_t kTabInstances = 44, kTabMaterials = 40, kTabAreas = 16, kTabCull = 8;
+constexpr uint32_t kTabOffInst = 0;
+constexpr uint32_t kTabOffMat = kTabOffInst + kTabInstances * (uint32_t)sizeof(DevInstance);
+constexpr uint32_t kTabOffArea = kTabOffMat + kTabMaterials * (uint32_t)sizeof(DevMaterial);
+constexpr uint32_t kTabOffCdf = (kTabOffArea + (kTabAreas + 1u) * (uint32_t)sizeof(DevEmitter) + 15u) & ~15u;
+constexpr uint32_t kTabOffGuide = kTabOffCdf + kTabAreas * 4u;
+constexpr uint32_t kTabOffCullRec = (kTabOffGuide + (kTabAreas + 1u) * 4u + 15u) & ~15u;
+constexpr uint32_t kTabOffCullObj = kTabOffCullRec + kTabCull * 48u;
+constexpr uint32_t kTabBytes = kTabOffCullObj + kTabCull * 48u;
+static_assert(sizeof(DevInstance) % 16 == 0 && sizeof(DevMaterial) % 16 == 0 && sizeof(DevEmitter) % 4 == 0, "copy units");
+static_assert(5u * ((kTabBytes + 511u) & ~511u) <= 160u * 1024u, "five shade blocks per CU");
+
+struct BlockTables {
+    const DevInstance *instances;
+    const DevMaterial *materials;
+    const DevEmitter *areas;
+    const DevEmitter *env_;
+    const float *cdf;
+    const uint32_t *guide;
+    const float4 *cull_rec;
+    const float *cull_obj;
+    const DeviceScene &sc;
+    __device__ __forceinline__ const DevInstance &instance(uint32_t i) const { return instances[i]; }
+    __device__ __forceinline__ const DevMaterial &material(uint32_t i) const { return materials[i]; }
+    __device__ __forceinline__ const DevEmitter &area(uint32_t i) const { return areas[i]; }
+    __device__ __forceinline__ const DevEmitter *env() const { return env_; }
+    __device__ __forceinline__ float area_cdf(uint32_t i) const { return cdf[i]; }
+    __device__ __forceinline__ uint32_t area_guide(uint32_t k) const { return guide[k]; }
+    __device__ __forceinline__ void cull_record(uint32_t k, float4 &a, float4 &b, float4 &c) const {
+        if (cull_rec) {
+            a = cull_rec[3 * k + 0];
+            b = cull_rec[3 * k + 1];
+            c = cull_rec[3 * k + 2];
+        } else {
+            GlobalTables{sc}.cull_record(k, a, b, c);
+        }
+    }
+    __device__ __forceinline__ const float *cull_to_object(uint32_t k, float4 b) const {
+        return cull_rec ? cull_obj + 12 * k : instances[__float_as_uint(b.w)].to_object;
+    }
+};
+
 struct HitGeo {
     LocalGeo g;
     int emitter;
     uint32_t inst;
 };
 
-__device__ __forceinline__ HitGeo reconstruct(const DeviceScene &sc, float4 h, const float4 *ro_rec, bool fresh,
-                                             vec3 rd, vec2 stale_uv) {
+template <class TB>
+__device__ __forceinline__ HitGeo reconstruct(const DeviceScene &sc, const TB &tb, float4 h, const float4 *ro_rec,
+                                             bool fresh, vec3 rd, vec2 stale_uv) {
     HitGeo out;
     const uint32_t idx = __float_as_uint(h.w);
     uint32_t inst_id, gprim;
@@ -71,7 +133,7 @@
     if (sc.two_level) {
         gprim = idx;
         inst_id = inst_of_prim(sc, idx);
-        const DevInstance &ti = sc.instances[inst_id];
+        const DevInstance &ti = tb.instance(inst_id);
         sphere = ti.kind == PUPIL_SHAPE_SPHERE;
         rec = sc.attrs + (size_t)kAttrStride * (sphere ? 0u : ti.attr_base + (idx - ti.prim_offset));
         for (int k = 0; k < 7; k++) ra[k] = rec[k];
@@ -88,7 +150,7 @@
         sphere = (ref & kPrimSphereBit) != 0u;
         inst_id = __float_as_uint(ra[1].w);
     }
-    const DevInstance &in = sc.instances[inst_id];
+    const DevInstance &in = tb.instance(inst_id);
     out.inst = inst_id;
     LocalGeo &g = out.g;
     g.texcoord = stale_uv;
@@ -136,26 +198,35 @@
     out.emitter = in.emitter_offset >= 0 ? in.emitter_offset + (int)local : -1;
     return out;
 }
-
-__device__ __forceinline__ const DevEmitter *select_emitter(const DeviceScene &sc, float p, float &sel_prob) {
+__device__ __forceinline__ HitGeo reconstruct(const DeviceScene &sc, float4 h, const float4 *ro_rec, bool fresh,
+                                             vec3 rd, vec2 stale_uv) {
+    return reconstruct(sc, GlobalTables{sc}, h, ro_rec, fresh, rd, stale_uv);
+}
+
+template <class TB>
+__device__ __forceinline__ const DevEmitter *select_emitter(const DeviceScene &sc, const TB &tb, float p,
+                                                            float &sel_prob) {
     uint32_t lo = 0, hi = sc.num_areas;
     if (sc.area_guide) {
         const uint32_t m = 1u << sc.guide_bits;
         const uint32_t k = min((uint32_t)(p * (float)m), m - 1u);
-        lo = sc.area_guide[k];
-        hi = sc.area_guide[k + 1];
+        lo = tb.area_guide(k);
+        hi = tb.area_guide(k + 1);
     }
     while (lo < hi) {
         const uint32_t mid = (lo + hi) >> 1;
-        if (p <= sc.area_cdf[mid]) hi = mid;
+        if (p <= tb.area_cdf(mid)) hi = mid;
         else lo = mid + 1;
     }
     const DevEmitter *e = nullptr;
-    if (lo < sc.num_areas) e = &sc.areas[lo];
-    else if (sc.has_env) e = sc.env;
-    else if (sc.num_areas > 0) e = &sc.areas[sc.num_areas - 1];
+    if (lo < sc.num_areas) e = &tb.area(lo);
+    else if (sc.has_env) e = tb.env();
+    else if (sc.num_areas > 0) e = &tb.area(sc.num_areas - 1);
     sel_prob = e ? e->select_probability : 0.f;
     return e;
+}
+__device__ __forceinline__ const DevEmitter *select_emitter(const DeviceScene &sc, float p, float &sel_prob) {
+    return select_emitter(sc, GlobalTables{sc}, p, sel_prob);
 }
 
 __device__ __forceinline__ bool last_sample(const FrameParams &fp, uint32_t p, uint32_t &l, uint32_t &frame_off) {
@@ -166,18 +237,16 @@
     return q - s * fp.spp + 1u == fp.spp;
 }
 
-__device__ __forceinline__ bool terminal_ray_culled(const DeviceScene &sc, vec3 o, vec3 d) {
+template <class TB>
+__device__ __forceinline__ bool terminal_ray_culled(const DeviceScene &sc, const TB &tb, vec3 o, vec3 d) {
     const RayPre r = ray_pre(o, d);
     bool hit = false;
     for (uint32_t k = 0; k < sc.cull_n; k++) {
-        const uint32_t i = sc.cull_set[k];
-        const float4 a = sc.prims[kRecF4 * i + 0];
-        const float4 b = sc.prims[kRecF4 * i + 1];
-        const float4 c = sc.prims[kRecF4 * i + 2];
+        float4 a, b, c;
+        tb.cull_record(k, a, b, c);
         float t, b1, b2;
         if (__float_as_uint(a.w) & kPrimSphereBit)
-            hit = hit || intersect_unit_sphere(sc.instances[__float_as_uint(b.w)].to_object, r.o, d, 0.001f,
-                                               kMaxDistance, t);
+            hit = hit || intersect_unit_sphere(tb.cull_to_object(k, b), r.o, d, 0.001f, kMaxDistance, t);
         else
             hit = hit || intersect_triangle(r, v3(a.x, a.y, a.z), v3(b.x, b.y, b.z), v3(c.x, c.y, c.z), 0.001f,
                                             kMaxDistance, t, b1, b2);
@@ -185,9 +254,10 @@
     return !hit;
 }
 
-template <uint32_t MAT>
-__device__ __forceinline__ uint32_t shade_hit(const DeviceScene &sc, const FrameParams &fp, const PathState &ps,
-                                              uint32_t p, bool fresh, uint32_t fresh_p, uint32_t fresh_seed0) {
+template <uint32_t MAT, class TB>
+__device__ __forceinline__ uint32_t shade_hit(const DeviceScene &sc, const TB &tb, const FrameParams &fp,
+                                              const PathState &ps, uint32_t p, bool fresh, uint32_t fresh_p,
+                                              uint32_t fresh_seed0) {
     bool push_next = false, push_shadow = false, culled = false;
     const float4 h = ld_ps(ps.hit + p);
     const vec3 ray_d = f3(ld_ps(ps.ray_d + p));
@@ -202,9 +272,9 @@
     vec3 L_add = v3(0.f);
     const vec2 stale_uv = v2(__uint_as_float(misc.z), __uint_as_float(misc.w));
 
-    HitGeo hg = reconstruct(sc, h, ps.ray_o + p, fresh, ray_d, stale_uv);
-    const DevInstance &in = sc.instances[hg.inst];
-    const DevMaterial &mat = sc.materials[in.material];
+    HitGeo hg = reconstruct(sc, tb, h, ps.ray_o + p, fresh, ray_d, stale_uv);
+    const DevInstance &in = tb.instance(hg.inst);
+    const DevMaterial &mat = tb.material(in.material);
     if (mat.twosided && dot(-ray_d, hg.g.normal) < 0.f) hg.g.normal = -hg.g.normal;
     const LocalGeo &geo = hg.g;
     LocalBsdf bsdf = local_bsdf(mat, geo.texcoord);
@@ -214,7 +284,7 @@
     bool L_changed = fresh;
     if (bounce == 0) {
         if (hg.emitter >= 0) {
-            L_add = emitter_radiance(sc.areas[hg.emitter], geo.texcoord);
+            L_add = emitter_radiance(tb.area(hg.emitter), geo.texcoord);
             L_changed = true;
         }
         const float test = rng_next(rng);
@@ -236,7 +306,7 @@
             if (fp.test) fp.test[fo + out] = test;
         }
     } else if (hg.emitter >= 0) {
-        const DevEmitter &e = sc.areas[hg.emitter];
+        const DevEmitter &e = tb.area(hg.emitter);
         vec3 Le;
         float pdf_e;
         emitter_eval_area(e, geo, f3(ld_ps(ps.ray_o + p)), Le, pdf_e);
@@ -259,7 +329,7 @@
     const bool nee = alive;
     if (alive) {
         float sel_prob;
-        const DevEmitter *e = select_emitter(sc, rng_next(rng), sel_prob);
+        const DevEmitter *e = select_emitter(sc, tb, rng_next(rng), sel_prob);
         const float x0 = rng_next(rng);
         const float x1 = rng_next(rng);
         const vec3 wo = to_local(-ray_d, geo.normal);
@@ -298,7 +368,7 @@
             const vec3 nd = to_world(br.wi, geo.normal);
             pdf_b = br.pdf;
             delta = (br.sampled_type & kLobeDelta) ? 1u : 0u;
-            if (fp.cull_cum && bounce + 2u >= fp.max_depth && terminal_ray_culled(sc, geo.position, nd)) {
+            if (fp.cull_cum && bounce + 2u >= fp.max_depth && terminal_ray_culled(sc, tb, geo.position, nd)) {
                 culled = true;
             } else {
                 st_ps(ps.ray_d + p, f4(nd, 0.f));
@@ -319,6 +389,12 @@
     return (push_next ? 1u : 0u) | (push_shadow ? 2u : 0u) | (nee ? 4u : 0u) | (culled ? 8u : 0u);
 }
 
+template <uint32_t MAT>
+__device__ __forceinline__ uint32_t shade_hit(const DeviceScene &sc, const FrameParams &fp, const PathState &ps,
+                                              uint32_t p, bool fresh, uint32_t fresh_p, uint32_t fresh_seed0) {
+    return shade_hit<MAT>(sc, GlobalTables{sc}, fp, ps, p, fresh, fresh_p, fresh_seed0);
+}
+
 __device__ __forceinline__ void count_culled(const FrameParams &fp, uint32_t flags) {
     if (!fp.cull_cum) return;
     const unsigned long long m = __ballot((flags & 8u) != 0u);
@@ -326,8 +402,10 @@
         atomicAdd(fp.cull_cum + (blockIdx.x % kCullShards) * kCullStride, (unsigned long long)__popcll(m));
 }
 
-__device__ __forceinline__ void shade_miss(const DeviceScene &sc, const FrameParams &fp, const PathState &ps,
-                                           uint32_t p, bool fresh, uint32_t fresh_p, uint32_t fresh_seed0) {
+template <class TB>
+__device__ __forceinline__ void shade_miss(const DeviceScene &sc, const TB &tb, const FrameParams &fp,
+                                           const PathState &ps, uint32_t p, bool fresh, uint32_t fresh_p,
+                                           uint32_t fresh_seed0) {
     const uint32_t fresh_rng = fresh ? fresh_rng_of(fp, fresh_p, fresh_seed0) : 0u;
     const uint4 misc = fresh ? make_uint4(fresh_rng, 0u, 0u, 0u) : ld_ps(ps.misc + p);
     if ((misc.y & 0xFFFFFFu) == 0u) {
@@ -338,7 +416,7 @@
             vec3 Le;
             float pdf;
             const vec3 ro = fresh ? camera_origin(sc.camera) : f3(ld_ps(ps.ray_o + p));
-            env_eval(*sc.env, ro, f3(ld_ps(ps.ray_d + p)), Le, pdf);
+            env_eval(*tb.env(), ro, f3(ld_ps(ps.ray_d + p)), Le, pdf);
             L = L + Le;
         }
         const float test = rng_next(rng);
@@ -355,13 +433,17 @@
         const float4 thr4 = ld_ps(ps.thr + p);
         vec3 Le;
         float env_pdf;
-        env_eval(*sc.env, f3(ld_ps(ps.ray_o + p)), f3(ld_ps(ps.ray_d + p)), Le, env_pdf);
+        env_eval(*tb.env(), f3(ld_ps(ps.ray_o + p)), f3(ld_ps(ps.ray_d + p)), Le, env_pdf);
         const float mis = mis_weight(thr4.w, env_pdf);
         const vec3 env_rad = Le * (f3(thr4) * mis);
         float4 rad4 = ld_ps(ps.rad + p);
         st_ps(ps.rad + p, f4(f3(rad4) + env_rad, 0.f));
     }
 }
-
-}
-}
+__device__ __forceinline__ void shade_miss(const DeviceScene &sc, const FrameParams &fp, const PathState &ps,
+                                           uint32_t p, bool fresh, uint32_t fresh_p, uint32_t fresh_seed0) {
+    shade_miss(sc, GlobalTables{sc}, fp, ps, p, fresh, fresh_p, fresh_seed0);
+}
+
+}
+}
```

New measurement: 7802 Mrays/s, median of 6. +4.5%, better.
